# jirsat/wavenets

Measured on AMD Instinct MI355X. Metric: audio samples/sec (training step, 16 kHz mu-law), higher is better.
Workload: dtype f32 (fp16 hi|lo split operands, fp32 accumulate)

## Files before the change

### wavenets_amd/csrc/wn_elem.hip

```cpp
#include <algorithm>

#include "wn_kernels.h"
#include "wn_sample.h"

__global__ void wn_add_kernel(const float* a, const float* b, float* out, int64_t n) {
  for (int64_t i = (int64_t)blockIdx.x * blockDim.x + threadIdx.x; i < n;
       i += (int64_t)gridDim.x * blockDim.x)
    out[i] = a[i] + b[i];
}
int wn_launch_add(const float* a, const float* b, float* out, int64_t n, hipStream_t s) {
  if (n <= 0) return WN_OK;
  hipLaunchKernelGGL(wn_add_kernel, dim3(wn_blocks(n)), dim3(256), 0, s, a, b, out, n);
  WN_HIP_CHECK(hipGetLastError());
  return WN_OK;
}

__global__ void wn_fill_kernel(float* p, float v, int64_t n) {
  for (int64_t i = (int64_t)blockIdx.x * blockDim.x + threadIdx.x; i < n;
       i += (int64_t)gridDim.x * blockDim.x)
    p[i] = v;
}
int wn_launch_fill(float* p, float v, int64_t n, hipStream_t s) {
  if (n <= 0) return WN_OK;
  hipLaunchKernelGGL(wn_fill_kernel, dim3(wn_blocks(n)), dim3(256), 0, s, p, v, n);
  WN_HIP_CHECK(hipGetLastError());
  return WN_OK;
}

#define WN_CS_CHUNKS 128
__global__ void wn_colsum_stage1(const float* g, int T, int C, float* part) {
  __shared__ float sm[256];
  const int b = blockIdx.x, chunk = blockIdx.y;
  const int c = blockIdx.z * 64 + (threadIdx.x & 63);
  const int p = threadIdx.x >> 6;
  const int len = (T + WN_CS_CHUNKS - 1) / WN_CS_CHUNKS;
  const int t0 = chunk * len, t1 = min(T, t0 + len);
  float acc = 0.f;
  if (c < C)
    for (int t = t0 + p; t < t1; t += 4) acc += g[((int64_t)b * T + t) * C + c];
  sm[threadIdx.x] = acc;
  __syncthreads();
  if (p == 0 && c < C)
    part[((int64_t)b * WN_CS_CHUNKS + chunk) * C + c] = sm[threadIdx.x] + sm[threadIdx.x + 64] + sm[threadIdx.x + 128] + sm[threadIdx.x + 192];
}
__global__ void wn_colsum_stage2(const float* part, int C, float* out, int64_t total) {
  const int64_t i = (int64_t)blockIdx.x * blockDim.x + threadIdx.x;
  if (i >= total) return;
  const int64_t b = i / C;
  const int c = (int)(i % C);
  double acc = 0.0;
  for (int k = 0; k < WN_CS_CHUNKS; ++k) acc += (double)part[(b * WN_CS_CHUNKS + k) * C + c];
  out[i] = (float)acc;
}
int64_t wn_colsum_scratch_floats(int B, int C) { return (int64_t)B * WN_CS_CHUNKS * C; }
int wn_launch_colsum_per_batch(const float* g, int B, int T, int C, float* out, float* scratch, hipStream_t s) {
  hipLaunchKernelGGL(wn_colsum_stage1, dim3(B, WN_CS_CHUNKS, (C + 63) / 64), dim3(256), 0, s, g, T, C, scratch);
  const int64_t total = (int64_t)B * C;
  hipLaunchKernelGGL(wn_colsum_stage2, dim3((unsigned)((total + 255) / 256)), dim3(256), 0, s, scratch, C, out, total);
  WN_HIP_CHECK(hipGetLastError());
  return WN_OK;
}

__device__ __forceinline__ int wn_quantize_one(float x, int bits) {
  const int nmax = (1 << bits) - 1;
  const double step = ldexp(1.0, 1 - bits);
  double f = floor(((double)x + 1.0) / step);
  int idx = f < 0.0 ? 0 : (f > (double)nmax ? nmax : (int)f);
  while (idx > 0 && (float)(-1.0 + idx * step) > x) --idx;
  while (idx < nmax && (float)(-1.0 + (idx + 1) * step) <= x) ++idx;
  return idx;
}
__global__ void wn_quantize_kernel(const float* x, int32_t* idx, int64_t n, int bits) {
  for (int64_t i = (int64_t)blockIdx.x * blockDim.x + threadIdx.x; i < n;
       i += (int64_t)gridDim.x * blockDim.x)
    idx[i] = wn_quantize_one(x[i], bits);
}
int wn_launch_quantize(const float* x, int32_t* idx, int64_t n, int bits, hipStream_t s) {
  if (n <= 0) return WN_OK;
  if (bits < 1 || bits > 16) { wn_set_error("quantize: bits %d unsupported", bits); return WN_E_UNSUPPORTED; }
  hipLaunchKernelGGL(wn_quantize_kernel, dim3(wn_blocks(n)), dim3(256), 0, s, x, idx, n, bits);
  WN_HIP_CHECK(hipGetLastError());
  return WN_OK;
}

__global__ void wn_dequantize_kernel(const int32_t* idx, float* x, int64_t n, float inv) {
  for (int64_t i = (int64_t)blockIdx.x * blockDim.x + threadIdx.x; i < n;
       i += (int64_t)gridDim.x * blockDim.x)
    x[i] = (float)idx[i] * inv - 1.0f;
}
int wn_launch_dequantize(const int32_t* idx, float* x, int64_t n, int bits, hipStream_t s) {
  if (n <= 0) return WN_OK;
  hipLaunchKernelGGL(wn_dequantize_kernel, dim3(wn_blocks(n)), dim3(256), 0, s, idx, x, n,
                     1.0f / (float)(1 << (bits - 1)));
  WN_HIP_CHECK(hipGetLastError());
  return WN_OK;
}

__global__ void wn_mulaw_kernel(const float* x, float* y, int64_t n) {
  const float inv = 1.0f / logf(256.0f);
  for (int64_t i = (int64_t)blockIdx.x * blockDim.x + threadIdx.x; i < n;
       i += (int64_t)gridDim.x * blockDim.x) {
    const float v = x[i];
    const float sgn = v > 0.f ? 1.f : (v < 0.f ? -1.f : 0.f);
    y[i] = sgn * (logf(1.0f + 255.0f * fabsf(v)) * inv);
  }
}
int wn_launch_mulaw(const float* x, float* y, int64_t n, hipStream_t s) {
  if (n <= 0) return WN_OK;
  hipLaunchKernelGGL(wn_mulaw_kernel, dim3(wn_blocks(n)), dim3(256), 0, s, x, y, n);
  WN_HIP_CHECK(hipGetLastError());
  return WN_OK;
}

__global__ void wn_inv_mulaw_kernel(const float* y, float* x, int64_t n) {
  for (int64_t i = (int64_t)blockIdx.x * blockDim.x + threadIdx.x; i < n;
       i += (int64_t)gridDim.x * blockDim.x) {
    const float v = y[i];
    const float sgn = v > 0.f ? 1.f : (v < 0.f ? -1.f : 0.f);
    x[i] = sgn * (powf(256.0f, fabsf(v)) - 1.0f) / 255.0f;
  }
}
int wn_launch_inv_mulaw(const float* y, float* x, int64_t n, hipStream_t s) {
  if (n <= 0) return WN_OK;
  hipLaunchKernelGGL(wn_inv_mulaw_kernel, dim3(wn_blocks(n)), dim3(256), 0, s, y, x, n);
  WN_HIP_CHECK(hipGetLastError());
  return WN_OK;
}

__global__ void wn_sumsq_kernel(const float* g, const WnTensorDesc* table, float* norms2) {
  __shared__ double sm[256];
  const WnTensorDesc d = table[blockIdx.x];
  const float* p = g + d.off;
  double a0 = 0.0, a1 = 0.0, a2 = 0.0, a3 = 0.0;
  int64_t i = threadIdx.x;
  for (; i + 3 * 256 < d.len; i += 4 * 256) {
    const float v0 = p[i], v1 = p[i + 256], v2 = p[i + 512], v3 = p[i + 768];
    a0 += (double)v0 * (double)v0; a1 += (double)v1 * (double)v1;
    a2 += (double)v2 * (double)v2; a3 += (double)v3 * (double)v3;
  }
  for (; i < d.len; i += 256) a0 += (double)p[i] * (double)p[i];
  const double acc = (a0 + a1) + (a2 + a3);
  sm[threadIdx.x] = acc;
  __syncthreads();
  for (int o = 128; o > 0; o >>= 1) {
    if (threadIdx.x < o) sm[threadIdx.x] += sm[threadIdx.x + o];
    __syncthreads();
  }
  if (threadIdx.x == 0) norms2[blockIdx.x] = (float)sm[0];
}
int wn_launch_sumsq(const float* g, const WnTensorDesc* d_table, int n, float* norms2, hipStream_t s) {
  if (n <= 0) return WN_OK;
  hipLaunchKernelGGL(wn_sumsq_kernel, dim3(n), dim3(256), 0, s, g, d_table, norms2);
  WN_HIP_CHECK(hipGetLastError());
  return WN_OK;
}

#define WN_CLIP_THREADS 1024
__global__ void __launch_bounds__(WN_CLIP_THREADS)
wn_clip_kernel(float* g, const WnTensorDesc* table, float clipnorm, float* norms2) {
  __shared__ double sm[WN_CLIP_THREADS / 64];
  __shared__ float sm_scale;
  const WnTensorDesc d = table[blockIdx.x];
  float* p = g + d.off;
  const int tid = threadIdx.x;
  int64_t head = (int64_t)((16u - (unsigned)((uintptr_t)p & 15u)) & 15u) >> 2;
  if (head > d.len) head = d.len;
  const int64_t nvec = (d.len - head) >> 2;
  const int64_t tail = head + 4 * nvec;
  float4* pv = reinterpret_cast<float4*>(p + head);
  double a0 = 0.0, a1 = 0.0, a2 = 0.0, a3 = 0.0;
  int64_t i = tid;
  for (; i + WN_CLIP_THREADS < nvec; i += 2 * WN_CLIP_THREADS) {
    const float4 x = pv[i], y = pv[i + WN_CLIP_THREADS];
    a0 += (double)x.x * (double)x.x; a1 += (double)x.y * (double)x.y;
    a2 += (double)x.z * (double)x.z; a3 += (double)x.w * (double)x.w;
    a0 += (double)y.x * (double)y.x; a1 += (double)y.y * (double)y.y;
    a2 += (double)y.z * (double)y.z; a3 += (double)y.w * (double)y.w;
  }
  for (; i < nvec; i += WN_CLIP_THREADS) {
    const float4 x = pv[i];
    a0 += (double)x.x * (double)x.x; a1 += (double)x.y * (double)x.y;
    a2 += (double)x.z * (double)x.z; a3 += (double)x.w * (double)x.w;
  }
  if (tid < head) a0 += (double)p[tid] * (double)p[tid];
  if (tail + tid < d.len) a1 += (double)p[tail + tid] * (double)p[tail + tid];
  double acc = (a0 + a1) + (a2 + a3);
  for (int o = 32; o > 0; o >>= 1) acc += __shfl_down(acc, o, 64);
  if ((tid & 63) == 0) sm[tid >> 6] = acc;
  __syncthreads();
  if (tid == 0) {
    double n2 = 0.0;
    for (int w = 0; w < WN_CLIP_THREADS / 64; ++w) n2 += sm[w];
    const float n2f = (float)n2;
    norms2[blockIdx.x] = n2f;
    sm_scale = clipnorm / fmaxf(sqrtf(n2f), clipnorm);
  }
  __syncthreads();
  const float scale = sm_scale;
  if (scale == 1.0f) return;
  for (i = tid; i < nvec; i += WN_CLIP_THREADS) {
    float4 x = pv[i];
    x.x *= scale; x.y *= scale; x.z *= scale; x.w *= scale;
    pv[i] = x;
  }
  if (tid < head) p[tid] *= scale;
  if (tail + tid < d.len) p[tail + tid] *= scale;
}
int wn_launch_clip(float* g, const WnTensorDesc* d_table, int n, float clipnorm, float* norms2, hipStream_t s) {
  if (n <= 0) return WN_OK;
  hipLaunchKernelGGL(wn_clip_kernel, dim3(n), dim3(WN_CLIP_THREADS), 0, s, g, d_table, clipnorm, norms2);
  WN_HIP_CHECK(hipGetLastError());
  return WN_OK;
}

__global__ void wn_adam_kernel(float* p, const float* g, float* m, float* v, const WnTensorDesc* table,
                               const float* norms2, float clipnorm, float alpha, float beta1,
                               float beta2, float eps, const float* skip_flag) {
  if (skip_flag && *skip_flag != 0.f) return;
  const WnTensorDesc d = table[blockIdx.y];
  float scale = 1.0f;
  if (clipnorm > 0.f) {
    const float nrm = sqrtf(norms2[blockIdx.y]);
    scale = clipnorm / fmaxf(nrm, clipnorm);
  }
  for (int64_t i = (int64_t)blockIdx.x * blockDim.x + threadIdx.x; i < d.len;
       i += (int64_t)gridDim.x * blockDim.x) {
    const int64_t k = d.off + i;
    const float gi = g[k] * scale;
    const float mi = m[k] + (gi - m[k]) * (1.0f - beta1);
    const float vi = v[k] + (gi * gi - v[k]) * (1.0f - beta2);
    m[k] = mi;
    v[k] = vi;
    p[k] = p[k] - alpha * mi / (sqrtf(vi) + eps);
  }
}
int wn_launch_adam(float* p, const float* g, float* m, float* v, const WnTensorDesc* d_table, int n,
                   const float* norms2, float clipnorm, float alpha, float beta1, float beta2,
                   float eps, const float* skip_flag, hipStream_t s) {
  if (n <= 0) return WN_OK;
  hipLaunchKernelGGL(wn_adam_kernel, dim3(32, n), dim3(256), 0, s, p, g, m, v, d_table, norms2,
                     clipnorm, alpha, beta1, beta2, eps, skip_flag);
  WN_HIP_CHECK(hipGetLastError());
  return WN_OK;
}

__global__ void wn_adam_ema_kernel(float* p, const float* g, float* m, float* v, float* a, const WnTensorDesc* table,
                                   const float* norms2, float clipnorm, float alpha, float beta1,
                                   float beta2, float eps, float momentum, int first, int overwrite,
                                   const float* skip_flag) {
  if (skip_flag && *skip_flag != 0.f) return;
  const WnTensorDesc d = table[blockIdx.y];
  float scale = 1.0f;
  if (clipnorm > 0.f) {
    const float nrm = sqrtf(norms2[blockIdx.y]);
    scale = clipnorm / fmaxf(nrm, clipnorm);
  }
  for (int64_t i = (int64_t)blockIdx.x * blockDim.x + threadIdx.x; i < d.len;
       i += (int64_t)gridDim.x * blockDim.x) {
    const int64_t k = d.off + i;
    const float gi = g[k] * scale;
    const float mi = m[k] + (gi - m[k]) * (1.0f - beta1);
    const float vi = v[k] + (gi * gi - v[k]) * (1.0f - beta2);
    m[k] = mi;
    v[k] = vi;
    const float pi = p[k] - alpha * mi / (sqrtf(vi) + eps);
    const float ai = first ? pi : a[k] + (pi - a[k]) * (1.0f - momentum);
    a[k] = ai;
    p[k] = overwrite ? ai : pi;
  }
}
int wn_launch_adam_ema(float* p, const float* g, float* m, float* v, float* a, const WnTensorDesc* d_table, int n,
                       const float* norms2, float clipnorm, float alpha, float beta1, float beta2,
                       float eps, float momentum, int first, int overwrite, const float* skip_flag, hipStream_t s) {
  if (n <= 0) return WN_OK;
  hipLaunchKernelGGL(wn_adam_ema_kernel, dim3(32, n), dim3(256), 0, s, p, g, m, v, a, d_table, norms2,
                     clipnorm, alpha, beta1, beta2, eps, momentum, first, overwrite, skip_flag);
  WN_HIP_CHECK(hipGetLastError());
  return WN_OK;
}

__global__ void wn_gate_kernel(const float* u, int64_t rows, int D, float* ag, float* z, int ldz) {
  const int64_t total = rows * D;
  for (int64_t i = (int64_t)blockIdx.x * blockDim.x + threadIdx.x; i < total;
       i += (int64_t)gridDim.x * blockDim.x) {
    const int64_t r = i / D;
    const int c = (int)(i % D);
    const float a = wn_tanh_fast(u[r * 2 * D + c]);
    const float g = wn_sigmoid_fast(u[r * 2 * D + D + c]);
    if (ag) ag[r * D + c] = g;
    if (z) z[r * ldz + c] = a * g;
  }
}
int wn_launch_gate(const float* u, int64_t rows, int D, float* ag, float* z, int ldz, hipStream_t s) {
  if (rows <= 0) return WN_OK;
  hipLaunchKernelGGL(wn_gate_kernel, dim3(wn_blocks(rows * D)), dim3(256), 0, s, u, rows, D, ag, z, ldz);
  WN_HIP_CHECK(hipGetLastError());
  return WN_OK;
}

__global__ void wn_batch_reduce_kernel(const float* slab, int splits, int N, float* out, int64_t total) {
  const int64_t i = (int64_t)blockIdx.x * blockDim.x + threadIdx.x;
  if (i >= total) return;
  const int64_t b = i / N;
  const int n = (int)(i % N);
  float acc = 0.f;
  for (int s = 0; s < splits; ++s) acc += slab[(b * splits + s) * N + n];
  out[i] = acc;
}
int wn_launch_batch_reduce(const float* slab, int B, int splits, int N, float* out, hipStream_t s) {
  const int64_t total = (int64_t)B * N;
  if (total <= 0) return WN_OK;
  hipLaunchKernelGGL(wn_batch_reduce_kernel, dim3((unsigned)((total + 255) / 256)), dim3(256), 0, s,
                     slab, splits, N, out, total);
  WN_HIP_CHECK(hipGetLastError());
  return WN_OK;
}

__global__ void wn_axpy_table_kernel(float* y, const float* x, const WnTensorDesc* table, float coef) {
  const WnTensorDesc d = table[blockIdx.y];
  for (int64_t i = (int64_t)blockIdx.x * blockDim.x + threadIdx.x; i < d.len;
       i += (int64_t)gridDim.x * blockDim.x)
    y[d.off + i] += coef * x[d.off + i];
}
int wn_launch_axpy_table(float* y, const float* x, const WnTensorDesc* d_table, int n, float coef,
                         hipStream_t s) {
  if (n <= 0) return WN_OK;
  hipLaunchKernelGGL(wn_axpy_table_kernel, dim3(16, n), dim3(256), 0, s, y, x, d_table, coef);
  WN_HIP_CHECK(hipGetLastError());
  return WN_OK;
}

__global__ void wn_dact_mul_kernel(const float* g, const float* y, float* out, int64_t n, int act) {
  for (int64_t i = (int64_t)blockIdx.x * blockDim.x + threadIdx.x; i < n;
       i += (int64_t)gridDim.x * blockDim.x)
    out[i] = g[i] * wn_dact_from_y(y[i], act);
}
int wn_launch_dact_mul(const float* g, const float* y, float* out, int64_t n, int act, hipStream_t s) {
  if (n <= 0) return WN_OK;
  hipLaunchKernelGGL(wn_dact_mul_kernel, dim3(wn_blocks(n)), dim3(256), 0, s, g, y, out, n, act);
  WN_HIP_CHECK(hipGetLastError());
  return WN_OK;
}

__device__ __forceinline__ uint32_t wn_hash32(uint32_t x) {
  x ^= x >> 16; x *= 0x7feb352dU; x ^= x >> 15; x *= 0x846ca68bU; x ^= x >> 16;
  return x;
}
__device__ __forceinline__ bool wn_drop_keep(int64_t idx, uint32_t key, float rate) {
  const uint32_t lo = (uint32_t)idx, hi = (uint32_t)((uint64_t)idx >> 32);
  const uint32_t hsh = wn_hash32(lo ^ wn_hash32(hi + key));
  return (float)(hsh >> 8) * (1.0f / 16777216.0f) >= rate;
}
__global__ void wn_dropout_kernel(const float* x, const float* g_res, float* out, int64_t n, float rate, float scale,
                                  uint32_t key, float* absmax_out) {
  float m = 0.f;
  for (int64_t i = (int64_t)blockIdx.x * blockDim.x + threadIdx.x; i < n; i += (int64_t)gridDim.x * blockDim.x) {
    float v = wn_drop_keep(i, key, rate) ? x[i] * scale : 0.f;
    if (g_res) v += g_res[i];
    out[i] = v;
    m = fmaxf(m, fabsf(v));
  }
  if (absmax_out) {
    m = wn_wave_max(m);
    if ((threadIdx.x & 63) == 0) wn_absmax_publish(absmax_out, m);
  }
}
uint32_t wn_dropout_key(uint64_t seed, int block, uint64_t step) {
  uint32_t k = (uint32_t)seed * 0x9E3779B9U + (uint32_t)(seed >> 32);
  k ^= (uint32_t)block * 0x85EBCA6BU + 0x1234567U;
  k ^= (uint32_t)step * 0xC2B2AE35U + (uint32_t)(step >> 32) * 0x27D4EB2FU;
  return k;
}
int wn_launch_dropout(const float* x, const float* g_res, float* out, int64_t n, float rate, uint32_t key,
                      float* absmax_out, hipStream_t s) {
  if (n <= 0) return WN_OK;
  hipLaunchKernelGGL(wn_dropout_kernel, dim3(wn_blocks(n)), dim3(256), 0, s, x, g_res, out, n, rate, 1.0f / (1.0f - rate),
                     key, absmax_out);
  WN_HIP_CHECK(hipGetLastError());
  return WN_OK;
}

__global__ void wn_cond_scatter_kernel(const float* tmp, const float* params, int64_t b_off0, int64_t b_stride, int B,
                                       int N, int D2, float* cb) {
  const int64_t total = (int64_t)N * B * D2;
  for (int64_t i = (int64_t)blockIdx.x * blockDim.x + threadIdx.x; i < total; i += (int64_t)gridDim.x * blockDim.x) {
    const int n = (int)(i % D2);
    const int u = (int)((i / D2) % B);
    const int b = (int)(i / ((int64_t)D2 * B));
    cb[i] = tmp[((int64_t)u * N + b) * D2 + n] + params[b_off0 + (int64_t)b * b_stride + n];
  }
}
__global__ void wn_cond_gather_kernel(const float* slab, int64_t P, int spb, int64_t bd_off0, int64_t bd_stride, int B,
                                      int N, int D2, float* dcb) {
  const int64_t total = (int64_t)B * N * D2;
  for (int64_t i = (int64_t)blockIdx.x * blockDim.x + threadIdx.x; i < total; i += (int64_t)gridDim.x * blockDim.x) {
    const int n = (int)(i % D2);
    const int b = (int)((i / D2) % N);
    const int u = (int)(i / ((int64_t)D2 * N));
    float acc = 0.f;
    for (int sp = 0; sp < spb; ++sp) acc += slab[(int64_t)(u * spb + sp) * P + bd_off0 + (int64_t)b * bd_stride + n];
    dcb[i] = acc;
  }
}
__global__ void wn_cond_wgrad_kernel(const float* m, const float* dcb, int B, int Cc, int N, int D2, float* grads,
                                     int64_t w_off0, int64_t w_stride, int64_t b_off0, int64_t b_stride) {
  const int64_t total = (int64_t)N * (Cc + 1) * D2;
  for (int64_t i = (int64_t)blockIdx.x * blockDim.x + threadIdx.x; i < total; i += (int64_t)gridDim.x * blockDim.x) {
    const int n = (int)(i % D2);
    const int c = (int)((i / D2) % (Cc + 1));
    const int b = (int)(i / ((int64_t)D2 * (Cc + 1)));
    float acc = 0.f;
    for (int u = 0; u < B; ++u) {
      const float g = dcb[((int64_t)u * N + b) * D2 + n];
      acc += c < Cc ? m[(int64_t)u * Cc + c] * g : g;
    }
    if (c < Cc) grads[w_off0 + (int64_t)b * w_stride + (int64_t)c * D2 + n] = acc;
    else grads[b_off0 + (int64_t)b * b_stride + n] = acc;
  }
}
int wn_launch_cond_scatter(const float* tmp, const float* params, int64_t b_off0, int64_t b_stride, int B, int N, int D2,
                           float* cb, hipStream_t s) {
  const int64_t total = (int64_t)N * B * D2;
  hipLaunchKernelGGL(wn_cond_scatter_kernel, dim3((unsigned)std::min<int64_t>((total + 255) / 256, 1024)), dim3(256), 0, s, tmp,
                     params, b_off0, b_stride, B, N, D2, cb);
  WN_HIP_CHECK(hipGetLastError());
  return WN_OK;
}
int wn_launch_cond_gather(const float* slab, int64_t P, int spb, int64_t bd_off0, int64_t bd_stride, int B, int N, int D2,
                          float* dcb, hipStream_t s) {
  const int64_t total = (int64_t)B * N * D2;
  hipLaunchKernelGGL(wn_cond_gather_kernel, dim3((unsigned)std::min<int64_t>((total + 255) / 256, 1024)), dim3(256), 0, s, slab, P,
                     spb, bd_off0, bd_stride, B, N, D2, dcb);
  WN_HIP_CHECK(hipGetLastError());
  return WN_OK;
}
int wn_launch_cond_wgrad(const float* m, const float* dcb, int B, int Cc, int N, int D2, float* grads, int64_t w_off0,
                         int64_t w_stride, int64_t b_off0, int64_t b_stride, hipStream_t s) {
  const int64_t total = (int64_t)N * (Cc + 1) * D2;
  hipLaunchKernelGGL(wn_cond_wgrad_kernel, dim3((unsigned)std::min<int64_t>((total + 255) / 256, 1024)), dim3(256), 0, s, m, dcb, B,
                     Cc, N, D2, grads, w_off0, w_stride, b_off0, b_stride);
  WN_HIP_CHECK(hipGetLastError());
  return WN_OK;
}

__global__ __launch_bounds__(256) void wn_inconv_fwd_kernel(const float* x, const float* w, const float* bias, int B, int T,
                                                            int R, int KS, float* y, float* absmax_out) {
  const int q = R / 4;
  const int64_t total = (int64_t)B * T * q;
  float wmax = 0.f;
  for (int64_t i = (int64_t)blockIdx.x * blockDim.x + threadIdx.x; i < total; i += (int64_t)gridDim.x * blockDim.x) {
    const int c = (int)(i % q) * 4;
    const int64_t row = i / q;
    const int t = (int)(row % T);
    float a0 = 0.f, a1 = 0.f, a2 = 0.f, a3 = 0.f;
    for (int tap = 0; tap < KS; ++tap) {
      const int ts = t - (KS - 1 - tap);
      const float xv = ts >= 0 ? x[row - (KS - 1 - tap)] : 0.f;
      const f32x4 wv = *reinterpret_cast<const f32x4*>(w + (int64_t)tap * R + c);
      a0 = fmaf(wv.x, xv, a0); a1 = fmaf(wv.y, xv, a1); a2 = fmaf(wv.z, xv, a2); a3 = fmaf(wv.w, xv, a3);
    }
    const f32x4 bv = *reinterpret_cast<const f32x4*>(bias + c);
    const f32x4 o = f32x4{a0 + bv.x, a1 + bv.y, a2 + bv.z, a3 + bv.w};
    *reinterpret_cast<f32x4*>(y + row * R + c) = o;
    wmax = fmaxf(wmax, fmaxf(fmaxf(fabsf(o.x), fabsf(o.y)), fmaxf(fabsf(o.z), fabsf(o.w))));
  }
  if (absmax_out) {
    __shared__ float wm[4];
    if (!(wmax < 3.0e38f)) wmax = 3.0e38f;
    wmax = wn_wave_max(wmax);
    if ((threadIdx.x & 63) == 0) wm[threadIdx.x >> 6] = wmax;
    __syncthreads();
    if (threadIdx.x == 0) wn_absmax_publish_any(absmax_out, fmaxf(fmaxf(wm[0], wm[1]), fmaxf(wm[2], wm[3])));
  }
}
int wn_launch_inconv_fwd(const float* x, const float* w, const float* bias, int B, int T, int R, int KS, float* y,
                         float* absmax_out, hipStream_t s) {
  const int64_t total = (int64_t)B * T * (R / 4);
  if (total <= 0) return WN_OK;
  hipLaunchKernelGGL(wn_inconv_fwd_kernel, dim3((unsigned)std::min<int64_t>((total + 255) / 256, 1024)), dim3(256), 0, s, x, w, bias,
                     B, T, R, KS, y, absmax_out);
  WN_HIP_CHECK(hipGetLastError());
  return WN_OK;
}

__global__ __launch_bounds__(256) void wn_sgemm_small32_kernel(const float* A, int64_t sai, int64_t sak, const float* B, int64_t sbk,
                                                               int64_t sbj, float* C, int ldc, int M, int N, int K,
                                                               int64_t za, int64_t zb, int64_t zc, const float* bias, int act,
                                                               int zk) {
  constexpr int KC = 128;
  __shared__ float As[KC][32 + 1], Bs[KC][32 + 1];
  A += (int64_t)blockIdx.z * za; B += (int64_t)blockIdx.z * zb; C += (int64_t)blockIdx.z * zc;
  if (zk > 0) K = max(0, min(K - (int)blockIdx.z * zk, zk));
  const int i0 = blockIdx.y * 32, j0 = blockIdx.x * 32;
  const int tx = threadIdx.x & 31, ty = threadIdx.x >> 5;
  float acc[4] = {0.f, 0.f, 0.f, 0.f};
  for (int k0 = 0; k0 < K; k0 += KC) {
    float ra[16], rb[16];
#pragma unroll
    for (int q = 0; q < 16; ++q) {
      const int e = threadIdx.x + 256 * q;
      const int ka = sak == 1 ? e % KC : e / 32, ia = sak == 1 ? e / KC : e % 32;
      ra[q] = (i0 + ia < M && k0 + ka < K) ? A[(int64_t)(i0 + ia) * sai + (int64_t)(k0 + ka) * sak] : 0.f;
      const int kb = sbk == 1 ? e % KC : e / 32, jb = sbk == 1 ? e / KC : e % 32;
      rb[q] = (j0 + jb < N && k0 + kb < K) ? B[(int64_t)(k0 + kb) * sbk + (int64_t)(j0 + jb) * sbj] : 0.f;
    }
    if (k0 > 0) __syncthreads();
#pragma unroll
    for (int q = 0; q < 16; ++q) {
      const int e = threadIdx.x + 256 * q;
      const int ka = sak == 1 ? e % KC : e / 32, ia = sak == 1 ? e / KC : e % 32;
      As[ka][ia] = ra[q];
      const int kb = sbk == 1 ? e % KC : e / 32, jb = sbk == 1 ? e / KC : e % 32;
      Bs[kb][jb] = rb[q];
    }
    __syncthreads();
#pragma unroll 8
    for (int k = 0; k < KC; ++k) {
      const float bv = Bs[k][tx];
#pragma unroll
      for (int a = 0; a < 4; ++a) acc[a] = fmaf(As[k][ty + 8 * a], bv, acc[a]);
    }
  }
#pragma unroll
  for (int a = 0; a < 4; ++a) {
    const int i = i0 + ty + 8 * a, j = j0 + tx;
    if (i < M && j < N) {
      float v = acc[a];
      if (bias) v = wn_act(v + bias[j], act);
      C[(int64_t)i * ldc + j] = v;
    }
  }
}
int wn_launch_sgemm_small(const float* A, int64_t sai, int64_t sak, const float* B, int64_t sbk, int64_t sbj, float* C, int ldc,
                          int M, int N, int K, hipStream_t s) {
  if (M <= 0 || N <= 0) return WN_OK;
  hipLaunchKernelGGL(wn_sgemm_small32_kernel, dim3((N + 31) / 32, (M + 31) / 32), dim3(256), 0, s, A, sai, sak, B, sbk, sbj, C,
                     ldc, M, N, K, (int64_t)0, (int64_t)0, (int64_t)0, (const float*)nullptr, 0, 0);
  WN_HIP_CHECK(hipGetLastError());
  return WN_OK;
}

int wn_launch_sgemm_small_batched(const float* A, int64_t sai, int64_t sak, int64_t za, const float* B, int64_t sbk, int64_t sbj,
                                  int64_t zb, float* C, int ldc, int64_t zc, int M, int N, int K, int nz, const float* bias,
                                  int act, hipStream_t s, int zk) {
  if (M <= 0 || N <= 0 || nz <= 0) return WN_OK;
  if (nz > 65535) { wn_set_error("sgemm_small_batched: too many products"); return WN_E_UNSUPPORTED; }
  hipLaunchKernelGGL(wn_sgemm_small32_kernel, dim3((N + 31) / 32, (M + 31) / 32, nz), dim3(256), 0, s, A, sai, sak, B, sbk, sbj, C,
                     ldc, M, N, K, za, zb, zc, bias, act, zk);
  WN_HIP_CHECK(hipGetLastError());
  return WN_OK;
}

__global__ void wn_skip_gather_kernel(const float* params, int64_t ws_off0, int64_t ws_stride, const float* bsum, int N, int D,
                                      int S, float* wsall) {
  for (int64_t i = (int64_t)blockIdx.x * blockDim.x + threadIdx.x; i < (int64_t)(N * D + 1) * S; i += (int64_t)gridDim.x * blockDim.x) {
    const int k = (int)(i / S), sidx = (int)(i % S);
    wsall[i] = k < N * D ? params[ws_off0 + (int64_t)(k / D) * ws_stride + (int64_t)(k % D) * S + sidx] : bsum[sidx];
  }
}
__global__ void wn_vec_add_kernel(const float* a, const float* b, int n, float* out) {
  const int i = blockIdx.x * blockDim.x + threadIdx.x;
  if (i < n) out[i] = a[i] + b[i];
}
int wn_launch_skip_fold(const float* params, int64_t ws_off0, int64_t ws_stride, int64_t wf0_off, int64_t bf0_off,
                        const float* bsum, int N, int D, int S, int F0, float* V, float* bfold, float* wsall, hipStream_t s) {
  const int64_t total = (int64_t)(N * D + 1) * S;
  hipLaunchKernelGGL(wn_skip_gather_kernel, dim3((unsigned)std::min<int64_t>((total + 255) / 256, 2048)), dim3(256), 0, s, params,
                     ws_off0, ws_stride, bsum, N, D, S, wsall);
  WN_HIP_CHECK(hipGetLastError());
  int rc = wn_launch_sgemm_small(wsall, S, 1, params + wf0_off, F0, 1, V, F0, N * D + 1, F0, S, s);
  if (rc) return rc;
  hipLaunchKernelGGL(wn_vec_add_kernel, dim3((F0 + 255) / 256), dim3(256), 0, s, V + (int64_t)N * D * F0, params + bf0_off, F0, bfold);
  WN_HIP_CHECK(hipGetLastError());
  return WN_OK;
}

__global__ void wn_skip_scatter_kernel(const float* Y, const float* colsum, int64_t ws_off0, int64_t ws_stride, int64_t bs_off0,
                                       int64_t bs_stride, int64_t bf0_off, int N, int D, int S, int F0, float* grads) {
  const int64_t n_ws = (int64_t)N * D * S, n_bs = (int64_t)N * S;
  const int64_t total = n_ws + n_bs + F0;
  for (int64_t i = (int64_t)blockIdx.x * blockDim.x + threadIdx.x; i < total; i += (int64_t)gridDim.x * blockDim.x) {
    if (i < n_ws) {
      const int k = (int)(i / S), sidx = (int)(i % S);
      grads[ws_off0 + (int64_t)(k / D) * ws_stride + (int64_t)(k % D) * S + sidx] = Y[i];
    } else if (i < n_ws + n_bs) {
      const int64_t j = i - n_ws;
      grads[bs_off0 + (j / S) * bs_stride + (j % S)] = Y[n_ws + (j % S)];
    } else {
      grads[bf0_off + (i - n_ws - n_bs)] = colsum[i - n_ws - n_bs];
    }
  }
}
int wn_launch_skip_scatter(const float* Y, const float* colsum, int64_t ws_off0, int64_t ws_stride, int64_t bs_off0,
                           int64_t bs_stride, int64_t bf0_off, int N, int D, int S, int F0, float* grads, hipStream_t s) {
  const int64_t total = (int64_t)N * D * S + (int64_t)N * S + F0;
  hipLaunchKernelGGL(wn_skip_scatter_kernel, dim3((unsigned)std::min<int64_t>((total + 255) / 256, 4096)), dim3(256), 0, s, Y, colsum,
                     ws_off0, ws_stride, bs_off0, bs_stride, bf0_off, N, D, S, F0, grads);
  WN_HIP_CHECK(hipGetLastError());
  return WN_OK;
}

__global__ void wn_guard_flag_kernel(const float* absmax, float limit, int enabled, float* out) {
  const float m = absmax ? *absmax : 0.f;
  out[0] = (enabled && !(m < limit)) ? 1.0f : 0.0f;
}
__global__ void wn_guard_accumulate_kernel(const float* src, float* dst) {
  const unsigned a = __float_as_uint(src[0]) & 0x7fffffffu, b = __float_as_uint(dst[0]) & 0x7fffffffu;
  dst[0] = __uint_as_float(a > b ? a : b);
}
int wn_launch_guard_accumulate(const float* src, float* dst, hipStream_t s) {
  hipLaunchKernelGGL(wn_guard_accumulate_kernel, dim3(1), dim3(1), 0, s, src, dst);
  WN_HIP_CHECK(hipGetLastError());
  return WN_OK;
}
int wn_launch_guard_flag(const float* absmax, float limit, int enabled, float* out, hipStream_t s) {
  hipLaunchKernelGGL(wn_guard_flag_kernel, dim3(1), dim3(1), 0, s, absmax, limit, enabled, out);
  WN_HIP_CHECK(hipGetLastError());
  return WN_OK;
}

template <int KS>
__global__ __launch_bounds__(256) void wn_inconv_wgrad_kernel(const float* x, const float* g, int T, int R, int spb,
                                                              float* slab, int64_t P, int64_t w_off, int64_t b_off) {
  __shared__ float red[256 * (KS + 1) * 4];
  const int split = blockIdx.x, ub = split / spb, sp = split % spb;
  int len = (T + spb - 1) / spb;
  const int r0 = sp * len, r1 = min(T, r0 + len);
// ... 49 lines not shown
```

### wavenets_amd/csrc/wn_forward.hip

```cpp
#include "wn_plan_internal.h"

namespace {

__global__ void wn_ring_capture_kernel(const float* src, int B, int T, int C, int nslots, float* ring) {
  const int64_t n = (int64_t)nslots * B * C;
  for (int64_t i = (int64_t)blockIdx.x * blockDim.x + threadIdx.x; i < n; i += (int64_t)gridDim.x * blockDim.x) {
    const int c = (int)(i % C);
    const int b = (int)((i / C) % B);
    const int k = (int)(i / ((int64_t)C * B));
    const int t = T - nslots + k;
    if (t >= 0) ring[((int64_t)(t % nslots) * B + b) * C + c] = src[((int64_t)b * T + t) * C + c];
  }
}

__global__ void wn_shift_split_kernel(const float* x_full, int B, int T, float* inputs, float* y_true) {
  const int64_t n = (int64_t)B * T;
  for (int64_t i = (int64_t)blockIdx.x * blockDim.x + threadIdx.x; i < n; i += (int64_t)gridDim.x * blockDim.x) {
    const int64_t b = i / T, t = i % T;
    inputs[i] = x_full[b * (T + 1) + t];
    y_true[i] = x_full[b * (T + 1) + t + 1];
  }
}

}

namespace wnp {

BlockPtrs block_ptrs(const wn_plan* p, int b, const float* params, const float* fragbase, int B, int T) {
  BlockPtrs k;
  memset(&k, 0, sizeof(k));
  const BlockInfo& bi = p->blocks[b];
  k.B = B; k.T = T; k.KS = p->KS; k.R = p->R; k.D = p->D; k.S = p->S; k.Cin = p->R; k.depth = p->LPB;
  k.act = p->c.activation; k.residual = p->c.use_residual;
  for (int i = 0; i < p->LPB; ++i) {
    const ConvInfo& c = bi.dil[i];
    k.dil[i] = c.dil;
    k.Wd[i] = params + p->tensors[c.kernel_t].off;
    k.bd[i] = params + p->tensors[c.bias_t].off;
    k.Fd[i] = fragbase + c.fragF; k.Fd_stride[i] = c.fragF_stride;
    k.Bd[i] = fragbase + c.fragB; k.Bd_stride[i] = c.fragB_stride;
  }
  k.br = params + p->tensors[bi.conv1.bias_t].off;
  k.Fr = fragbase + bi.conv1.fragF; k.Br_ = fragbase + bi.conv1.fragB;
  if (bi.has_skip) { k.bs = params + p->tensors[bi.conv_skip.bias_t].off; k.Bs = fragbase + bi.conv_skip.fragB; }
  k.Cc = 0; k.cond = nullptr; k.cb = nullptr;
  k.fused = p->fused_ok;
  if (p->fused16_ok && p->LPB == 1) { k.F16d = fragbase + bi.dil.back().frag16; k.F16r = fragbase + bi.conv1.frag16; }
  if (bi.f16gate >= 0) { k.F16g = fragbase + bi.f16gate; k.F16r = fragbase + bi.conv1.frag16; }
  if (bi.f16nat >= 0) k.F16n = fragbase + bi.f16nat;
  if (bi.g16u >= 0 && p->LPB == 1) k.G16u = fragbase + bi.g16u;
  if (bi.g16uf >= 0) k.G16uf = fragbase + bi.g16uf;
  if (p->LPB == 1 && bi.dil[0].frag16B >= 0) k.G16x = fragbase + bi.dil[0].frag16B;
  return k;
}

void deep16_ptrs(const wn_plan* p, int b, const float* fragbase, BlockPtrs& k) {
  if (!deep16(p)) return;
  const BlockInfo& bi = p->blocks[b];
  k.F16d = fragbase + bi.dil.back().frag16; k.F16r = fragbase + bi.conv1.frag16;
  for (int i = 0; i < p->LPB; ++i) {
    const ConvInfo& c = bi.dil[i];
    if (bi.d16F[i] >= 0) { k.F16i[i] = fragbase + bi.d16F[i]; k.JTi[i] = std::max(2, ceil32(c.cout)); }
    if (bi.d16B[i] >= 0) { k.G16i[i] = fragbase + bi.d16B[i]; k.JTb[i] = std::max(2, ceil32(c.cin)); }
  }
  if (bi.g16u >= 0) { k.G16u = fragbase + bi.g16u; k.JTu = std::max(2, ceil32(p->D)); }
}

int ring_capture(const float* src, int B, int T, int C, int nslots, float* ring, hipStream_t s) {
  const int64_t n = (int64_t)nslots * B * C;
  hipLaunchKernelGGL(wn_ring_capture_kernel, dim3((unsigned)std::min<int64_t>((n + 255) / 256, 4096)), dim3(256), 0, s,
                     src, B, T, C, nslots, ring);
  WN_HIP_CHECK(hipGetLastError());
  return WN_OK;
}

int forward_core(wn_plan* p, const float* params, const float* x, bool prep, const float* cond, int B,
                 int T, bool training, float* ws, const WsLayout& L, hipStream_t s, const GenRings* rings, LossFuse* lf) {
  int rc = ensure_device_tables(p);
  if (rc) return rc;
  const int64_t rows = (int64_t)B * T;
  float* fragbase = ws + L.frag;
  if (prep) {
    rc = wn_launch_prep_table(p->d_prep, (int)p->prep.size(), params, fragbase, s);
    if (rc) return rc;
  }
  wn_exec& exs = wnp::ex(p);
  const bool fold = fold_ok(p);
  const bool fork_prep = prep && fold && p->c.use_skip && wn_debug_get(9) == 0;
  bool prep_forked = false;
  auto fold_prep = [&](hipStream_t sp) -> int {
    const bool fp_prof = prep && fold && exs.foldprep_used + 2 <= (int)exs.foldprep_ev.size();
    if (fp_prof) (void)hipEventRecord(exs.foldprep_ev[exs.foldprep_used], sp);
    if (prep && p->c.use_skip) {
      const ConvInfo& c0 = p->blocks[0].has_skip ? p->blocks[0].conv_skip : p->blocks[0].conv1;
      WnVecSumArgs v;
      v.base = params; v.off0 = p->tensors[c0.bias_t].off;
      v.stride = p->N > 1 ? (p->tensors[(p->blocks[1].has_skip ? p->blocks[1].conv_skip : p->blocks[1].conv1).bias_t].off - v.off0) : 0;
      v.count = p->N; v.len = p->Sh; v.out = ws + L.bias_sum;
      const int r = wn_launch_vecsum(v, sp);
      if (r) return r;
    }
    if (fold && prep) {
      const BlockInfo& b0 = p->blocks[0];
      const int64_t wst = p->N > 1 ? p->tensors[p->blocks[1].conv_skip.kernel_t].off - p->tensors[b0.conv_skip.kernel_t].off : 0;
      int r = wn_launch_skip_fold(params, p->tensors[b0.conv_skip.kernel_t].off, wst, p->tensors[p->finals[0].kernel_t].off,
                                  p->tensors[p->finals[0].bias_t].off, ws + L.bias_sum, p->N, p->D, p->S, p->fold_F0, ws + L.vfold,
                                  ws + L.bfold, ws + L.wsall, sp);
      if (r) return r;
      r = wn_launch_prep_table(p->d_prep2, (int)p->prep2.size(), ws, fragbase, sp, 64);
      if (r) return r;
    }
    if (fp_prof) { (void)hipEventRecord(exs.foldprep_ev[exs.foldprep_used + 1], sp); exs.foldprep_used += 2; }
    return WN_OK;
  };
  if (!fork_prep) {
    rc = fold_prep(s);
    if (rc) return rc;
  }
  const float* m = cond;
  if (p->c.cond_inputs > 0) {
    if (!cond) { wn_set_error("Conditioning must be provided."); return WN_E_INVALID; }
    int mc = p->c.cond_inputs;
    for (size_t j = 0; j < p->mapping.size(); ++j) {
      const ConvInfo& c = p->mapping[j];
      if (cond_small(p))
        rc = wn_launch_sgemm_small_batched(m, mc, 1, 0, params + p->tensors[c.kernel_t].off, c.cout, 1, 0, ws + L.M[j], c.cout, 0,
                                           B, c.cout, mc, 1, params + p->tensors[c.bias_t].off, p->c.mapping_activation, s);
      else
      rc = Gemm(1, B, c.cout, ceil32(c.cout)).seg(m, mc, mc, 0, fragbase + c.fragF)
               .bias(params + p->tensors[c.bias_t].off).act(p->c.mapping_activation).run(ws + L.M[j], c.cout, s);
      if (rc) return rc;
      m = ws + L.M[j]; mc = c.cout;
    }
    if (p->frag_condF >= 0) {
      const int D2 = 2 * p->D;
      const ConvInfo& c0 = p->blocks[0].conv_cond;
      const int64_t bst = p->N > 1 ? p->tensors[p->blocks[1].conv_cond.bias_t].off - p->tensors[c0.bias_t].off : 0;
      if (cond_small(p)) {
        const int64_t wst = p->N > 1 ? p->tensors[p->blocks[1].conv_cond.kernel_t].off - p->tensors[c0.kernel_t].off : 0;
        rc = wn_launch_sgemm_small_batched(m, p->Cc, 1, 0, params + p->tensors[c0.kernel_t].off, D2, 1, wst, ws + L.cbt, p->N * D2, D2,
                                           B, D2, p->Cc, p->N, nullptr, 0, s);
      } else
      rc = Gemm(1, B, p->N * D2, ceil32(p->N * D2)).seg(m, p->Cc, p->Cc, 0, fragbase + p->frag_condF).run(ws + L.cbt, p->N * D2, s);
      if (rc) return rc;
      rc = wn_launch_cond_scatter(ws + L.cbt, params, p->tensors[c0.bias_t].off, bst, B, p->N, D2, ws + L.cb, s);
      if (rc) return rc;
    } else {
    for (int b = 0; b < p->N; ++b) {
      const ConvInfo& c = p->blocks[b].conv_cond;
      rc = Gemm(1, B, 2 * p->D, ceil32(2 * p->D)).seg(m, p->Cc, p->Cc, 0, fragbase + c.fragF)
               .bias(params + p->tensors[c.bias_t].off).run(ws + L.cb + (int64_t)b * B * 2 * p->D, 2 * p->D, s);
      if (rc) return rc;
    }
    }
  }
  float* const fam = ws + L.fwd_absmax;
  WN_HIP_CHECK(hipMemsetAsync(fam, 0, sizeof(float), s));
  {
    if (p->R % 4 == 0 && wn_debug_get(1) != 1) {
      rc = wn_launch_inconv_fwd(x, params + p->tensors[p->causal.kernel_t].off, params + p->tensors[p->causal.bias_t].off, B, T,
                                p->R, p->KS, ws + L.H[0], fam, s);
    } else {
      Gemm g(B, T, p->R, ceil32(p->R));
      for (int t = 0; t < p->KS; ++t)
        g.seg(x, 1, 1, (p->KS - 1 - t), fragbase + p->causal.fragF + t * p->causal.fragF_stride);
      rc = g.bias(params + p->tensors[p->causal.bias_t].off).run(ws + L.H[0], p->R, s);
    }
    if (rc) return rc;
    if (rings) {
      rc = ring_capture(x, B, T, 1, p->KS, rings->xin, s);
      if (!rc) rc = ring_capture(ws + L.H[0], B, T, p->R, rings->nslots[0], rings->h[0], s);
      if (rc) return rc;
    }
  }
  if (p->Dp != p->D) {
    rc = wn_launch_fill(ws + L.Z, 0.f, rows * p->N * p->Dp, s);
    if (rc) return rc;
  }
  const bool prof_chain = wnp::ex(p).prof_on && !rings && p->LPB == 1 && p->c.cond_inputs == 0 && p->R == p->D &&
                          !(training && wnp::ex(p).drop_rate > 0.f) && block_ptrs(p, 0, params, fragbase, B, T).fused;
  const bool stack_prof = !rings && wnp::ex(p).stack_used + 2 <= (int)wnp::ex(p).stack_ev.size();
  if (stack_prof) (void)hipEventRecord(wnp::ex(p).stack_ev[wnp::ex(p).stack_used], s);
  if (fork_prep) {
    if (!exs.side) {
      WN_HIP_CHECK(hipStreamCreateWithFlags(&exs.side, hipStreamNonBlocking));
      WN_HIP_CHECK(hipEventCreateWithFlags(&exs.ev_fork, hipEventDisableTiming));
      WN_HIP_CHECK(hipEventCreateWithFlags(&exs.ev_join, hipEventDisableTiming));
    }
    if (!exs.ev_ffork) {
      WN_HIP_CHECK(hipEventCreateWithFlags(&exs.ev_ffork, hipEventDisableTiming));
      WN_HIP_CHECK(hipEventCreateWithFlags(&exs.ev_fjoin, hipEventDisableTiming));
    }
    WN_HIP_CHECK(hipEventRecord(exs.ev_ffork, s));
    WN_HIP_CHECK(hipStreamWaitEvent(exs.side, exs.ev_ffork, 0));
    rc = fold_prep(exs.side);
    if (rc) return rc;
    WN_HIP_CHECK(hipEventRecord(exs.ev_fjoin, exs.side));
    prep_forked = true;
  }
  for (int b = 0; b < p->N; ++b) {
    BlockPtrs k = block_ptrs(p, b, params, fragbase, B, T);
    if (training && !rings) deep16_ptrs(p, b, fragbase, k);
    if (p->c.cond_inputs > 0) k.cb = ws + L.cb + (int64_t)b * B * 2 * p->D;
    BlockBufs f;
    memset(&f, 0, sizeof(f));
    const int hi = training ? b : (b & 1), ho = training ? b + 1 : ((b + 1) & 1);
    f.x = ws + L.H[hi];
    if (training && wnp::ex(p).drop_rate > 0.f) {
      rc = wn_launch_dropout(ws + L.H[hi], nullptr, ws + L.XD[b], rows * p->R, wnp::ex(p).drop_rate,
                             wn_dropout_key(wnp::ex(p).drop_seed, b, wnp::ex(p).drop_step), nullptr, s);
      if (rc) return rc;
      f.x = ws + L.XD[b];
      f.res = ws + L.H[hi];
    }
    for (int i = 0; i + 1 < p->LPB; ++i) f.P[i] = ws + L.P[b][i];
    f.U = ws + L.U;
    f.AG = training ? ws + L.AG[b] : nullptr;
    f.Z = ws + L.Z + (int64_t)b * rows * p->Dp; f.ldz = p->Dp;
    f.O = nullptr;
    f.x_out = ws + L.H[ho];
    f.fwd_absmax = fam;
    const bool prof = wnp::ex(p).prof_on && wnp::ex(p).prof_used + 2 <= (int)wnp::ex(p).prof_ev.size();
    const bool ev0 = prof && (!prof_chain || b == 0), ev1 = prof && (!prof_chain || b == p->N - 1);
    if (ev0) (void)hipEventRecord(wnp::ex(p).prof_ev[wnp::ex(p).prof_used], s);
    rc = block_forward(k, f, s);
    if (rc) return rc;
    if (ev1) {
      (void)hipEventRecord(wnp::ex(p).prof_ev[wnp::ex(p).prof_used + 1], s);
      wnp::ex(p).prof_cnt[wnp::ex(p).prof_used / 2] = prof_chain ? p->N : 1;
      wnp::ex(p).prof_used += 2;
    }
    if (rings && b + 1 < p->N) {
      rc = ring_capture(f.x_out, B, T, p->R, rings->nslots[b + 1], rings->h[b + 1], s);
      if (rc) return rc;
    }
    if (rings)
      for (int i = 0; i + 1 < p->LPB; ++i) {
        rc = ring_capture(f.P[i], B, T, p->D, rings->nslots_p[b][i], rings->hp[b][i], s);
        if (rc) return rc;
      }
  }
  if (prep_forked) WN_HIP_CHECK(hipStreamWaitEvent(s, exs.ev_fjoin, 0));
  const float* hin;
  size_t first_final = 0;
  if (fold) {
    const ConvInfo& c0 = p->finals[0];
    if (p->Dp == p->D && wn_gemm_planes16s_supported(c0.cout, p->D, p->N, p->Dp, c0.cout) &&
        (int64_t)rows * p->Dp * 4 < ((int64_t)1 << 32) && (int64_t)rows * c0.cout * 4 < ((int64_t)1 << 32)) {
      WnGemmPlanesArgs ga;
      memset(&ga, 0, sizeof(ga));
      ga.z = ws + L.Z; ga.plane_stride = rows * p->Dp; ga.ld = p->Dp; ga.plane_k = p->D; ga.nplanes = p->N;
      ga.w16 = fragbase + p->frag16_foldF; ga.bias = ws + L.bfold; ga.act = p->c.activation;
      ga.y = ws + L.HA[0]; ga.ldy = c0.cout; ga.N = c0.cout; ga.B = B; ga.T = T; ga.absmax_out = fam;
      rc = wn_launch_gemm_planes16s(ga, s);
    } else
    rc = Gemm(B, T, c0.cout, ceil32(c0.cout)).seg_planes(ws + L.Z, p->Dp, rows * p->Dp, p->N * p->Dp, nullptr)
             .w16(fragbase + p->frag16_foldF).bias(ws + L.bfold).act(p->c.activation).absmax_fwd(fam)
             .run(ws + L.HA[0], c0.cout, s);
    if (rc) return rc;
    hin = ws + L.HA[0];
    first_final = 1;
  } else if (p->c.use_skip) {
    rc = Gemm(B, T, p->Sh, ceil32(p->Sh)).seg_planes(ws + L.Z, p->Dp, rows * p->Dp, p->N * p->Dp, fragbase + p->frag_skipF)
             .w16(p->frag16_skipF >= 0 ? fragbase + p->frag16_skipF : nullptr)
             .bias(ws + L.bias_sum).absmax_fwd(fam).run(ws + L.skipsum, p->Sh, s);
    if (rc) return rc;
    hin = ws + L.skipsum;
  } else {
    hin = ws + L.H[training ? p->N : (p->N & 1)];
  }
  if (stack_prof) { (void)hipEventRecord(wnp::ex(p).stack_ev[wnp::ex(p).stack_used + 1], s); wnp::ex(p).stack_used += 2; }
  int hc = fold ? p->finals[0].cout : p->Hin;
  for (size_t i = first_final; i < p->finals.size(); ++i) {
    const ConvInfo& c = p->finals[i];
    const bool last = (i + 1 == p->finals.size());
    float* dst = last ? ws + L.logits : ws + L.HA[i];
    if (last && lf && loss_fusable(p, rows) && wn_gemm_planes16s_supported(c.cout, hc, 1, hc, c.cout) &&
        (int64_t)rows * hc * 4 < ((int64_t)1 << 32)) {
      WnGemmPlanesArgs ga;
      memset(&ga, 0, sizeof(ga));
      ga.z = hin; ga.plane_stride = 0; ga.ld = hc; ga.plane_k = hc; ga.nplanes = 1;
      ga.w16 = fragbase + c.frag16; ga.bias = params + p->tensors[c.bias_t].off; ga.act = WN_ACT_LINEAR;
      ga.y = lf->g_logits; ga.ldy = c.cout; ga.N = c.cout; ga.B = B; ga.T = T; ga.absmax_out = lf->absmax_out;
      ga.cat_loss = 1; ga.target = lf->target; ga.gscale = lf->gscale; ga.loss_rows = lf->loss_rows;
      ga.sample_out = lf->sample_out; ga.inv_lv = lf->inv_lv; ga.seed = lf->seed; ga.offset = lf->offset;
      rc = wn_launch_gemm_planes16s(ga, s);
      if (rc) return rc;
      lf->done = true;
      break;
    }
    if (c.frag16 >= 0 && wn_debug_get(1) != 1 && wn_gemm_planes16s_supported(c.cout, hc, 1, hc, c.cout) &&
        (int64_t)rows * hc * 4 < ((int64_t)1 << 32)) {
      WnGemmPlanesArgs ga;
      memset(&ga, 0, sizeof(ga));
      ga.z = hin; ga.plane_stride = 0; ga.ld = hc; ga.plane_k = hc; ga.nplanes = 1;
      ga.w16 = fragbase + c.frag16; ga.bias = params + p->tensors[c.bias_t].off; ga.act = last ? WN_ACT_LINEAR : p->c.activation;
      ga.y = dst; ga.ldy = c.cout; ga.N = c.cout; ga.B = B; ga.T = T; ga.absmax_out = last ? nullptr : fam;
      rc = wn_launch_gemm_planes16s(ga, s);
      if (rc) return rc;
      hin = dst; hc = c.cout;
      continue;
    }
    rc = Gemm(B, T, c.cout, ceil32(c.cout)).seg(hin, hc, hc, 0, fragbase + c.fragF)
             .w16(c.frag16 >= 0 ? fragbase + c.frag16 : nullptr)
             .bias(params + p->tensors[c.bias_t].off).act(last ? WN_ACT_LINEAR : p->c.activation)
             .absmax_fwd(last ? nullptr : fam).run(dst, c.cout, s);
    if (rc) return rc;
    hin = dst; hc = c.cout;
  }
  return WN_OK;
}

int shift_split(const float* x_full, int B, int T, float* inputs, float* y_true, hipStream_t s) {
  const int64_t rows = (int64_t)B * T;
  hipLaunchKernelGGL(wn_shift_split_kernel, dim3((unsigned)std::min<int64_t>((rows + 255) / 256, 4096)), dim3(256), 0, s,
                     x_full, B, T, inputs, y_true);
  WN_HIP_CHECK(hipGetLastError());
  return WN_OK;
}

bool loss_fusable(const wn_plan* p, int64_t rows) {
  if (p->c.head != WN_HEAD_CATEGORICAL || p->Cout != 256 || wn_debug_get(1) == 1 || p->finals.empty()) return false;
  const ConvInfo& c = p->finals.back();
  return c.frag16 >= 0 && c.cout == 256 && rows > 0;
}

int loss_stage(wn_plan* p, int B, int T, int global_batch, bool want_grad, float* ws, const WsLayout& L,
               float* loss_out, float* absmax_out, hipStream_t s, bool fused_done) {
  const int64_t rows = (int64_t)B * T;
  const float gscale = 1.0f / (float)global_batch;
  int rc;
  if (fused_done) return wn_launch_sum(ws + L.loss_rows, rows, gscale, loss_out, ws + L.sum_scratch, s);
  float* g_logits = want_grad ? ws + L.GF.back() : nullptr;
  if (p->c.head == WN_HEAD_CATEGORICAL) {
    rc = wn_launch_quantize(ws + L.yt, reinterpret_cast<int32_t*>(ws + L.target), rows, p->c.bits, s);
    if (rc) return rc;
    float* so = nullptr;
    if (want_grad && wnp::ex(p).step_sample && !wnp::ex(p).step_sample_det && p->Cout <= 256) { so = wnp::ex(p).step_sample; wnp::ex(p).step_sample = nullptr; }
    rc = wn_launch_cat_loss(ws + L.logits, reinterpret_cast<const int32_t*>(ws + L.target), rows, p->Cout,
                            gscale, ws + L.loss_rows, g_logits, absmax_out, s, so, p->c.bits, wnp::ex(p).step_sample_seed,
                            wnp::ex(p).step_sample_off);
  } else {
    rc = wn_launch_mix_loss(ws + L.logits, ws + L.yt, rows, p->c.num_mixtures, p->c.bits,
                            p->c.head == WN_HEAD_LOGISTIC ? 1 : 2, gscale, ws + L.loss_rows, g_logits, absmax_out, s);
  }
  if (rc) return rc;
  return wn_launch_sum(ws + L.loss_rows, rows, gscale, loss_out, ws + L.sum_scratch, s);
}

}

using namespace wnp;

extern "C" int wn_forward(wn_plan* p, const float* params, const float* x, const float* cond, int32_t B,
                          int32_t T, float* out, float* logits_out, float* workspace, int64_t ws_floats,
                          void* stream) {
  if (!p || !params || !x || !workspace || B < 1 || T < 1) { wn_set_error("forward: bad arguments"); return WN_E_INVALID; }
  hipStream_t s = (hipStream_t)stream;
  const WsLayout L = make_layout(p, B, T, false);
  if (ws_floats < L.total) { wn_set_error("forward: workspace too small (%lld < %lld floats)", (long long)ws_floats, (long long)L.total); return WN_E_INVALID; }
  int rc = forward_core(p, params, x, true, cond, B, T, false, workspace, L, s);
  if (rc) return rc;
  const int64_t rows = (int64_t)B * T;
  if (logits_out) WN_HIP_CHECK(hipMemcpyAsync(logits_out, workspace + L.logits, rows * p->Cout * sizeof(float), hipMemcpyDeviceToDevice, s));
  if (out) {
    if (p->c.head == WN_HEAD_CATEGORICAL) return wn_launch_softmax(workspace + L.logits, out, rows, p->Cout, s);
    WN_HIP_CHECK(hipMemcpyAsync(out, workspace + L.logits, rows * p->Cout * sizeof(float), hipMemcpyDeviceToDevice, s));
  }
  return WN_OK;
}

extern "C" int wn_forward_training(wn_plan* p, const float* params, const float* x, const float* cond, int32_t B,
                                   int32_t T, float* out, float* logits_out, float* workspace, int64_t ws_floats,
                                   void* stream) {
  if (!p || !params || !x || !workspace || B < 1 || T < 1) { wn_set_error("forward_training: bad arguments"); return WN_E_INVALID; }
  hipStream_t s = (hipStream_t)stream;
  const WsLayout L = make_layout(p, B, T, true);
  if (ws_floats < L.total) { wn_set_error("forward_training: workspace too small (%lld < %lld floats)", (long long)ws_floats, (long long)L.total); return WN_E_INVALID; }
  int rc = forward_core(p, params, x, true, cond, B, T, true, workspace, L, s);
  if (rc) return rc;
  const int64_t rows = (int64_t)B * T;
  if (logits_out) WN_HIP_CHECK(hipMemcpyAsync(logits_out, workspace + L.logits, rows * p->Cout * sizeof(float), hipMemcpyDeviceToDevice, s));
  if (out) {
    if (p->c.head == WN_HEAD_CATEGORICAL) return wn_launch_softmax(workspace + L.logits, out, rows, p->Cout, s);
    WN_HIP_CHECK(hipMemcpyAsync(out, workspace + L.logits, rows * p->Cout * sizeof(float), hipMemcpyDeviceToDevice, s));
  }
  return WN_OK;
}

extern "C" int wn_eval_loss(wn_plan* p, const float* params, const float* x_full, const float* cond,
                            int32_t B, int32_t T, int32_t global_batch, float* loss_out, float* pred_out,
                            float* workspace, int64_t ws_floats, void* stream) {
  if (!p || !params || !x_full || !workspace || !loss_out || B < 1 || T < 1) { wn_set_error("eval_loss: bad arguments"); return WN_E_INVALID; }
  hipStream_t s = (hipStream_t)stream;
  const WsLayout L = make_layout(p, B, T, false);
  if (ws_floats < L.total) { wn_set_error("eval_loss: workspace too small"); return WN_E_INVALID; }
  const int64_t rows = (int64_t)B * T;
  float* inputs = workspace + L.probs;
  { const int rcs = shift_split(x_full, B, T, inputs, workspace + L.yt, s); if (rcs) return rcs; }
  int rc = forward_core(p, params, inputs, true, cond, B, T, false, workspace, L, s);
  if (rc) return rc;
  rc = loss_stage(p, B, T, global_batch > 0 ? global_batch : B, false, workspace, L, loss_out, nullptr, s);
  if (rc) return rc;
  rc = wn_launch_guard_flag(workspace + L.fwd_absmax, WN_RANGE_LIMIT, wn_debug_get(1) != 1, loss_out + 2, s);
  if (rc) return rc;
  if (pred_out) {
    if (p->c.head == WN_HEAD_CATEGORICAL) return wn_launch_softmax(workspace + L.logits, pred_out, rows, p->Cout, s);
    WN_HIP_CHECK(hipMemcpyAsync(pred_out, workspace + L.logits, rows * p->Cout * sizeof(float), hipMemcpyDeviceToDevice, s));
  }
  return WN_OK;
}
```

### wavenets_amd/csrc/wn_gemm.hip

```cpp
#include "wn_split16.h"

using namespace wn_split16;

__device__ __forceinline__ void wn_prep16_body(const WnPrepDesc& d, const float* params, float* ws,
                                               int64_t start, int64_t stride) {
  const int JI = (d.I + 31) / 32;
  const int nks = (d.KK + 15) / 16;
  const int64_t total = (int64_t)nks * JI * 64 * 8;
  const float* src = params + d.src_off;
  __half* dst = reinterpret_cast<__half*>(ws + d.dst_off);
  for (int64_t idx = start; idx < total; idx += stride) {
    const int jj = idx & 7;
    const int lane = (idx >> 3) & 63;
    const int64_t blk = idx >> 9;
    const int j = blk % JI;
    const int ks = blk / JI;
    const int i = 32 * j + (lane & 31);
    const int kk = 16 * ks + 8 * (jj >> 2) + 4 * (lane >> 5) + (jj & 3);
    float v = 0.f;
    if (i < d.I && kk < d.KK) v = d.transpose ? src[(int64_t)kk * d.ld + i] : src[(int64_t)i * d.ld + kk];
    const __half hi = __float2half_rn(v);
    const __half lo = __float2half_rn(v - __half2float(hi));
    const int64_t base = (((int64_t)(ks + d.q_off) * d.JT + (j + d.j_off)) * 2) * 512 + lane * 8 + jj;
    dst[base] = hi;
    dst[base + 512] = lo;
  }
}

__device__ __forceinline__ void wn_prep_body(const WnPrepDesc& d, const float* params, float* ws,
                                             int64_t start, int64_t stride) {
  if (d.kind == 1) { wn_prep16_body(d, params, ws, start, stride); return; }
  const int JI = (d.I + 31) / 32;
  const int nq = (d.KK + 7) / 8;
  const int64_t total = (int64_t)nq * JI * 256;
  const float* src = params + d.src_off;
  float* dst = ws + d.dst_off;
  for (int64_t idx = start; idx < total; idx += stride) {
    int e = idx & 3;
    int lane = (idx >> 2) & 63;
    int64_t blk = idx >> 8;
    int j = blk % JI;
    int q = blk / JI;
    int i = 32 * j + (lane & 31);
    int kk = 8 * q + 4 * (lane >> 5) + e;
    float v = 0.f;
    if (i < d.I && kk < d.KK) v = d.transpose ? src[(int64_t)kk * d.ld + i] : src[(int64_t)i * d.ld + kk];
    dst[(((int64_t)(q + d.q_off) * d.JT + (j + d.j_off)) * 64 + lane) * 4 + e] = v;
  }
}

__global__ void wn_prep_table_kernel(const WnPrepDesc* table, const float* params, float* ws) {
  WnPrepDesc d = table[blockIdx.y];
  wn_prep_body(d, params, ws, (int64_t)blockIdx.x * blockDim.x + threadIdx.x,
               (int64_t)gridDim.x * blockDim.x);
}

__global__ void wn_prep_one_kernel(WnPrepDesc d, const float* params, float* ws) {
  wn_prep_body(d, params, ws, (int64_t)blockIdx.x * blockDim.x + threadIdx.x,
               (int64_t)gridDim.x * blockDim.x);
}

int wn_launch_prep_table(const WnPrepDesc* d_table, int n, const float* params, float* ws,
                         hipStream_t s, int gx) {
  if (n <= 0) return WN_OK;
  dim3 grid(gx > 0 ? gx : 16, n);
  hipLaunchKernelGGL(wn_prep_table_kernel, grid, dim3(256), 0, s, d_table, params, ws);
  WN_HIP_CHECK(hipGetLastError());
  return WN_OK;
}

int wn_launch_prep_one(WnPrepDesc d, const float* params, float* ws, hipStream_t s) {
  hipLaunchKernelGGL(wn_prep_one_kernel, dim3(16), dim3(256), 0, s, d, params, ws);
  WN_HIP_CHECK(hipGetLastError());
  return WN_OK;
}

__global__ void wn_vecsum_kernel(WnVecSumArgs a) {
  int i = blockIdx.x * blockDim.x + threadIdx.x;
  if (i >= a.len) return;
  float acc = 0.f;
  for (int j = 0; j < a.count; ++j) acc += a.base[a.off0 + (int64_t)j * a.stride + i];
  a.out[i] = acc;
}

int wn_launch_vecsum(WnVecSumArgs a, hipStream_t s) {
  hipLaunchKernelGGL(wn_vecsum_kernel, dim3((a.len + 255) / 256), dim3(256), 0, s, a);
  WN_HIP_CHECK(hipGetLastError());
  return WN_OK;
}

template <int JT>
__global__ __launch_bounds__(256, (JT >= 8 ? 2 : (JT >= 4 ? 3 : 4))) void wn_gemm_rows_kernel(WnGemmArgs a) {
  const int lane = threadIdx.x & 63;
  const int wave = threadIdx.x >> 6;
  const int tiles_per_b = (a.T + 31) >> 5;
  const int64_t tile = (int64_t)blockIdx.x * 4 + wave;
  if (tile >= (int64_t)a.B * tiles_per_b) return;
  const int b = (int)(tile / tiles_per_b);
  const int t0 = (int)(tile % tiles_per_b) * 32;
  const int tl = lane & 31, h = lane >> 5;
  const int t = t0 + tl;
  const int jb = blockIdx.y * JT;

  f32x16 acc[JT];
#pragma unroll
  for (int j = 0; j < JT; ++j)
#pragma unroll
    for (int r = 0; r < 16; ++r) acc[j][r] = 0.f;

#pragma unroll
  for (int s = 0; s < WN_MAXSEG; ++s) {
    if (s >= a.nseg) break;
    const float* sx = a.seg[s].x;
    const float* sfrag = a.seg[s].frag;
    const int sldx = a.seg[s].ldx, sK = a.seg[s].K, sshift = a.seg[s].shift, svec = a.seg[s].vec;
    const int splk = a.seg[s].plane_k;
    const int64_t splst = a.seg[s].plane_stride;
    const int ts = t - sshift;
    const bool valid = (t < a.T) && (ts >= 0) && (ts < a.T);
    const float* xrow = sx + ((int64_t)b * a.T + (valid ? ts : 0)) * sldx;
    const int nq = (sK + 7) >> 3;
    const f32x4* fr = reinterpret_cast<const f32x4*>(sfrag) + (int64_t)jb * 64 + lane;

    auto load_x = [&](int q) -> f32x4 {
      const int k = 8 * q + 4 * h;
      f32x4 xv = {0.f, 0.f, 0.f, 0.f};
      if (valid) {
        const float* xp = splk > 0 ? xrow + (int64_t)(k / splk) * splst + (k % splk) : xrow + k;
        if (svec && k + 3 < sK) {
          xv = *reinterpret_cast<const f32x4*>(xp);
        } else {
          if (k + 0 < sK) xv.x = xp[0];
          if (k + 1 < sK) xv.y = xp[1];
          if (k + 2 < sK) xv.z = xp[2];
          if (k + 3 < sK) xv.w = xp[3];
        }
      }
      return xv;
    };
    auto load_a = [&](int q, f32x4 (&av)[JT]) {
      wn_static_for<JT>([&](auto jc) {
        constexpr int j = decltype(jc)::value;
        if (jb + j < a.JTtot) av[j] = fr[((int64_t)q * a.JTtot + j) * 64];
      });
    };
    auto compute = [&](const f32x4& xv, const f32x4 (&av)[JT]) {
      wn_static_for<JT>([&](auto jc) {
        constexpr int j = decltype(jc)::value;
        if (jb + j < a.JTtot) {
          acc[j] = wn_mfma(av[j].x, xv.x, acc[j]);
          acc[j] = wn_mfma(av[j].y, xv.y, acc[j]);
          acc[j] = wn_mfma(av[j].z, xv.z, acc[j]);
          acc[j] = wn_mfma(av[j].w, xv.w, acc[j]);
        }
      });
    };
    constexpr int PF = 8;
    if (JT == 1 && svec && splk == 0 && (sK & 7) == 0 && (nq % PF) == 0 && jb < a.JTtot) {
      const f32x4* xp = reinterpret_cast<const f32x4*>(xrow + 4 * h);
      const f32x4* ap = fr;
      const int64_t astep = (int64_t)a.JTtot * 64;
      f32x4 xr[PF], ar[PF];
#pragma unroll
      for (int i = 0; i < PF; ++i) { xr[i] = xp[2 * i]; ar[i] = ap[i * astep]; }
      __builtin_amdgcn_sched_barrier(0);
      for (int q0 = 0; q0 < nq; q0 += PF) {
#pragma unroll
        for (int i = 0; i < PF; ++i) {
          f32x4 xv = xr[i];
          if (!valid) xv = f32x4{0.f, 0.f, 0.f, 0.f};
          const f32x4 av = ar[i];
          acc[0] = wn_mfma(av.x, xv.x, acc[0]);
          acc[0] = wn_mfma(av.y, xv.y, acc[0]);
          acc[0] = wn_mfma(av.z, xv.z, acc[0]);
          acc[0] = wn_mfma(av.w, xv.w, acc[0]);
          const int qn = min(q0 + i + PF, nq - 1);
          xr[i] = xp[2 * qn];
          ar[i] = ap[qn * astep];
          __builtin_amdgcn_sched_barrier(0);
        }
      }
    } else {
    f32x4 x0, x1, a0[JT], a1[JT];
    x0 = load_x(0);
    load_a(0, a0);
    int q = 0;
    for (; q + 2 <= nq; q += 2) {
      x1 = load_x(q + 1);
      load_a(q + 1, a1);
      compute(x0, a0);
      if (q + 2 < nq) {
        x0 = load_x(q + 2);
        load_a(q + 2, a0);
      }
      compute(x1, a1);
    }
    if (q < nq) compute(x0, a0);
    }
  }

  if (t >= a.T) return;
  const int64_t row = (int64_t)b * a.T + t;
  wn_static_for<JT * 4>([&](auto jc) {
    constexpr int j = decltype(jc)::value / 4;
    constexpr int rq = decltype(jc)::value % 4;
    {
      const int n0 = 32 * (jb + j) + 8 * rq + 4 * h;
      if (n0 >= a.N) return;
      float v[4];
      v[0] = acc[j][4 * rq + 0]; v[1] = acc[j][4 * rq + 1];
      v[2] = acc[j][4 * rq + 2]; v[3] = acc[j][4 * rq + 3];
      const bool full = a.vec_out && (n0 + 3 < a.N);
      if (full) {
        if (a.bias) {
          const f32x4 bv = *reinterpret_cast<const f32x4*>(a.bias + n0);
          v[0] += bv.x; v[1] += bv.y; v[2] += bv.z; v[3] += bv.w;
        }
        if (a.rowbias) {
          const float* rb = a.rowbias + (int64_t)b * a.ld_rowbias + n0;
// ... 258 lines not shown
      compute_chunk(av0, bv0);
      if (tt + 16 < r1) {
        if (tt + 32 < r1) load_chunk(tt + 32, av0, bv0);
        compute_chunk(av1, bv1);
      }
    }
  }

#pragma unroll
  for (int i = 0; i < WG_TM; ++i)
#pragma unroll
    for (int j = 0; j < WG_TN; ++j) {
      const int n = n0 + 32 * j + tl;
#pragma unroll
      for (int r = 0; r < 16; ++r) {
        const int k = k0 + 32 * i + wn_drow(r, h);
        if (k < a.K && n < a.N) a.out[(int64_t)k * a.out_ld + n] = acc[i][j][r] * inv_gsc;
      }
    }
  if (a.bias) {
#pragma unroll
    for (int j = 0; j < WG_TN; ++j) {
      const float tot = bsum[j] + __shfl_xor(bsum[j], 32);
      const int n = n0 + 32 * j + tl;
      if (h == 0 && n < a.N) a.bias[n] = tot;
    }
  }
}

__global__ __launch_bounds__(256, 2) void wn_wgrad_kernel(WnWgradArgs a, int nkb, int nnb) {
  const int wave = threadIdx.x >> 6;
  const int nsplit = a.B * a.splits_per_b;
  const int split = blockIdx.x * 4 + wave;
  if (split >= nsplit) return;
  const int kb = blockIdx.y / nnb, nb = blockIdx.y % nnb;
  const int sp = split % a.splits_per_b;
  int len = (a.T + a.splits_per_b - 1) / a.splits_per_b;
  len = (len + 1) & ~1;
  WnWgUnit u;
  u.x = a.x; u.ldx = a.ldx; u.K = a.K; u.shift = a.shift; u.g = a.g; u.ldg = a.ldg; u.N = a.N;
  u.T = a.T; u.b = split / a.splits_per_b; u.r0 = sp * len; u.r1 = min(a.T, u.r0 + len);
  u.k0 = kb * 32 * WG_TM; u.n0 = nb * 32 * WG_TN;
  u.out = a.slab + (int64_t)split * a.K * a.N; u.out_ld = a.N;
  u.bias = (a.slab_bias && kb == 0) ? a.slab_bias + (int64_t)split * a.N : nullptr;
  wn_wgrad_body(u);
}

template <bool F16>
__global__ __launch_bounds__(256, 2) void wn_wgrad_batched_kernel(const WnWgJob* jobs, float* ws, float* slab,
                                                                  int64_t P, int B, int T, int splits_per_b) {
  const int wave = threadIdx.x >> 6;
  const int nsplit = B * splits_per_b;
  const int split = blockIdx.x * 4 + wave;
  if (split >= nsplit) return;
  const WnWgJob j = jobs[blockIdx.y];
  const int sp = split % splits_per_b;
  int len = (T + splits_per_b - 1) / splits_per_b;
  len = (len + 1) & ~1;
  WnWgUnit u;
  u.x = ws + j.x_off; u.ldx = j.ldx; u.K = j.K; u.shift = j.shift; u.g = ws + j.g_off; u.ldg = j.ldg; u.N = j.N;
  u.T = T; u.b = split / splits_per_b; u.r0 = sp * len; u.r1 = min(T, u.r0 + len);
  u.k0 = j.k0; u.n0 = j.n0;
  float* row = slab + (int64_t)split * P;
  u.out = row + j.out_off; u.out_ld = j.N;
  u.bias = j.bias_off >= 0 ? row + j.bias_off : nullptr;
  if constexpr (F16) {
    float gsc = 1.0f, inv = 1.0f;
    if (j.gmax_off >= 0) pow2_scale(ws[j.gmax_off], gsc, inv);
    wn_wgrad_body16(u, gsc, inv);
  } else {
    wn_wgrad_body(u);
  }
}

int wn_launch_wgrad_batched(const WnWgJob* d_jobs, int njobs, float* ws, float* slab, int64_t P, int B, int T,
                            int splits_per_b, hipStream_t s, bool exact_fp32) {
  if (njobs <= 0) return WN_OK;
  const int nsplit = B * splits_per_b;
  if (exact_fp32 || wn_debug_get(1) == 1 || wn_debug_get(3) == 1)
    hipLaunchKernelGGL(wn_wgrad_batched_kernel<false>, dim3((nsplit + 3) / 4, njobs), dim3(256), 0, s, d_jobs, ws, slab, P,
                       B, T, splits_per_b);
  else
    hipLaunchKernelGGL(wn_wgrad_batched_kernel<true>, dim3((nsplit + 3) / 4, njobs), dim3(256), 0, s, d_jobs, ws, slab, P,
                       B, T, splits_per_b);
  WN_HIP_CHECK(hipGetLastError());
  return WN_OK;
}

__global__ void wn_reduce_table_kernel(const float* slab, int nsplit, int64_t P, float* out,
                                       const WnTensorDesc* table) {
  const WnTensorDesc d = table[blockIdx.y];
  for (int64_t i = (int64_t)blockIdx.x * blockDim.x + threadIdx.x; i < d.len;
       i += (int64_t)gridDim.x * blockDim.x) {
    float acc = 0.f;
    const float* col = slab + d.off + i;
    int s = 0;
    for (; s + 8 <= nsplit; s += 8) {
      float v[8];
#pragma unroll
      for (int e = 0; e < 8; ++e) v[e] = col[(int64_t)(s + e) * P];
#pragma unroll
      for (int e = 0; e < 8; ++e) acc += v[e];
    }
    for (; s < nsplit; ++s) acc += col[(int64_t)s * P];
    out[d.off + i] = acc;
  }
}

struct WnBlkFirst { int v[257]; };
__global__ __launch_bounds__(256) void wn_reduce_flat_kernel(const float* slab, int nsplit, int64_t P, float* out,
                                                             const WnTensorDesc* table, WnBlkFirst bf, int n) {
  int lo = 0, hi = n;
  while (hi - lo > 1) {
    const int mid = (lo + hi) >> 1;
    if (bf.v[mid] <= (int)blockIdx.x) lo = mid; else hi = mid;
  }
  const WnTensorDesc d = table[lo];
  const int64_t i = (int64_t)((int)blockIdx.x - bf.v[lo]) * 256 + threadIdx.x;
  if (i >= d.len) return;
  float acc = 0.f;
  const float* col = slab + d.off + i;
  int s = 0;
  for (; s + 16 <= nsplit; s += 16) {
    float v[16];
#pragma unroll
    for (int e = 0; e < 16; ++e) v[e] = col[(int64_t)(s + e) * P];
#pragma unroll
    for (int e = 0; e < 16; ++e) acc += v[e];
  }
  for (; s < nsplit; ++s) acc += col[(int64_t)s * P];
  out[d.off + i] = acc;
}

int wn_launch_reduce_table(const float* slab, int nsplit, int64_t P, float* out, const WnTensorDesc* d_table,
                           int n, hipStream_t s, const WnTensorDesc* h_table) {
  if (n <= 0) return WN_OK;
  if (h_table && n <= 256) {
    WnBlkFirst bf;
    int64_t nblk = 0;
    for (int t = 0; t < n; ++t) { bf.v[t] = (int)nblk; nblk += (h_table[t].len + 255) / 256; }
    for (int t = n; t <= 256; ++t) bf.v[t] = (int)nblk;
    if (nblk <= 0) return WN_OK;
    if (nblk < (int64_t)1 << 30) {
      hipLaunchKernelGGL(wn_reduce_flat_kernel, dim3((unsigned)nblk), dim3(256), 0, s, slab, nsplit, P, out, d_table, bf, n);
      WN_HIP_CHECK(hipGetLastError());
      return WN_OK;
    }
  }
  hipLaunchKernelGGL(wn_reduce_table_kernel, dim3(64, n), dim3(256), 0, s, slab, nsplit, P, out, d_table);
  WN_HIP_CHECK(hipGetLastError());
  return WN_OK;
}

int wn_wgrad_tile_k() { return 32 * WG_TM; }
int wn_wgrad_tile_n() { return 32 * WG_TN; }

int wn_wgrad_choose_splits(int B, int T, int K, int N) {
  const int jobs = ((K + 32 * WG_TM - 1) / (32 * WG_TM)) * ((N + 32 * WG_TN - 1) / (32 * WG_TN));
  int want = (1024 + jobs - 1) / jobs;
  int per_b = (want + B - 1) / B;
  const int max_per_b = (T + 255) / 256;
  if (per_b > max_per_b) per_b = max_per_b;
  if (per_b < 1) per_b = 1;
  return per_b;
}

int wn_launch_wgrad(const WnWgradArgs& a, hipStream_t s) {
  if (a.K <= 0 || a.N <= 0 || a.B <= 0 || a.T <= 0) return WN_OK;
  const int nkb = (a.K + 32 * WG_TM - 1) / (32 * WG_TM);
  const int nnb = (a.N + 32 * WG_TN - 1) / (32 * WG_TN);
  const int nsplit = a.B * a.splits_per_b;
  dim3 grid((nsplit + 3) / 4, nkb * nnb);
  hipLaunchKernelGGL(wn_wgrad_kernel, grid, dim3(256), 0, s, a, nkb, nnb);
  WN_HIP_CHECK(hipGetLastError());
  return WN_OK;
}

#define WN_RED_GROUP 16
__global__ void wn_reduce_stageA_kernel(float* slab, int nsplit, int64_t total) {
  const int g = blockIdx.y;
  const int s0 = g * WN_RED_GROUP;
  const int s1 = min(nsplit, s0 + WN_RED_GROUP);
  for (int64_t i = (int64_t)blockIdx.x * blockDim.x + threadIdx.x; i < total;
       i += (int64_t)gridDim.x * blockDim.x) {
    float acc = 0.f;
    for (int s = s0; s < s1; ++s) acc += slab[(int64_t)s * total + i];
    slab[(int64_t)s0 * total + i] = acc;
  }
}

__global__ void wn_reduce_kernel(WnReduceArgs a, int stride) {
  const int64_t total = (int64_t)a.K * a.N;
  for (int64_t i = (int64_t)blockIdx.x * blockDim.x + threadIdx.x; i < total;
       i += (int64_t)gridDim.x * blockDim.x) {
    float acc = 0.f;
    for (int s = 0; s < a.nsplit; s += stride) acc += a.slab[(int64_t)s * total + i];
    const int k = (int)(i / a.N), n = (int)(i % a.N);
    float* dst = a.out + (int64_t)(k / a.seg_len) * a.seg_stride + (int64_t)(k % a.seg_len) * a.N + n;
    for (int r = 0; r < a.replicate; ++r) {
      float* d = dst + (int64_t)r * a.rep_stride;
      *d = a.accumulate ? (*d + acc) : acc;
    }
  }
}

int wn_launch_reduce(const WnReduceArgs& a, hipStream_t s) {
  const int64_t total = (int64_t)a.K * a.N;
  if (total <= 0) return WN_OK;
  int blocks = (int)((total + 255) / 256);
  if (blocks > 2048) blocks = 2048;
  int stride = 1;
  if (a.nsplit > 2 * WN_RED_GROUP) {
    const int groups = (a.nsplit + WN_RED_GROUP - 1) / WN_RED_GROUP;
    hipLaunchKernelGGL(wn_reduce_stageA_kernel, dim3(blocks, groups), dim3(256), 0, s,
                       const_cast<float*>(a.slab), a.nsplit, total);
    stride = WN_RED_GROUP;
  }
  hipLaunchKernelGGL(wn_reduce_kernel, dim3(blocks), dim3(256), 0, s, a, stride);
  WN_HIP_CHECK(hipGetLastError());
  return WN_OK;
}
```

### wavenets_amd/csrc/wn_kernels.h

```cpp
#pragma once
#include "wn_common.h"

struct WnTensorDesc { int64_t off; int64_t len; };

struct WnPrepDesc {
  int64_t src_off;
  int64_t dst_off;
  int32_t I;
  int32_t KK;
  int32_t ld;
  int32_t transpose;
  int32_t q_off;
  int32_t j_off;
  int32_t JT;
  int32_t kind;
};
int wn_launch_prep_table(const WnPrepDesc* d_table, int n, const float* params, float* ws,
                         hipStream_t s, int gx = 16);
int wn_launch_prep_one(WnPrepDesc d, const float* params, float* ws, hipStream_t s);
struct WnVecSumArgs { const float* base; int64_t off0; int64_t stride; int32_t count; int32_t len; float* out; };
int wn_launch_vecsum(WnVecSumArgs a, hipStream_t s);

#define WN_MAXSEG 4
struct WnSeg {
  const float* x;
  const float* frag;
  int32_t ldx;
  int32_t K;
  int32_t shift;
  int32_t vec;
  int32_t plane_k;
  int64_t plane_stride;
};
struct WnGemmArgs {
  WnSeg seg[WN_MAXSEG];
  int32_t nseg;
  int32_t B, T;
  int32_t N;
  int32_t JTtot;
  const float* bias;
  const float* rowbias;
  int32_t ld_rowbias;
  const float* addc;
  int32_t ld_addc;
  int32_t act;
  int32_t epi;
  const float* aux;
  int32_t ld_aux;
  const float* aux2;
  int32_t ld_aux2;
  float* y;
  int32_t ldy;
  int32_t vec_out;
  float* y2;
  int32_t ld_y2;
  int32_t absmax_any;
};
int wn_launch_gemm_rows(const WnGemmArgs& a, hipStream_t s);
int wn_gemm_rows16_ok(const WnGemmArgs& a);
int wn_launch_gemm_rows16(const WnGemmArgs& a, const float* w16, const float* absmax_in0,
                          const float* absmax_in1, float* absmax_out, hipStream_t s);

struct WnGemmPlanesArgs {
  const float* z;
  int64_t plane_stride;
  int32_t ld, plane_k, nplanes;
  const float* w16;
  const float* bias;
  int32_t act;
  float* y; int32_t ldy;
  int32_t N;
  int32_t B, T;
  float* absmax_out;
  int32_t bwd;
  const float* absmax_in;
  const float* aux; int32_t ld_aux;
  int32_t nshift; int32_t shift[4];
  int32_t cat_loss;
  const int32_t* target;
  float gscale;
  float* loss_rows;
  float* sample_out;
  float inv_lv;
  uint64_t seed, offset;
};
int wn_gemm_planes16s_supported(int N, int plane_k, int nplanes, int ld, int ldy);
int wn_gemm_taps16s_supported(int N, int plane_k, int ntaps, int ld, int ldy);
int wn_launch_gemm_planes16s(const WnGemmPlanesArgs& a, hipStream_t s);

struct WnWgradArgs {
  const float* x; int32_t ldx; int32_t K; int32_t shift;
  const float* g; int32_t ldg; int32_t N;
  int32_t B, T;
  int32_t splits_per_b;
  float* slab;
  float* slab_bias;
};
int wn_wgrad_choose_splits(int B, int T, int K, int N);
int wn_launch_wgrad(const WnWgradArgs& a, hipStream_t s);
struct WnWgJob {
  int64_t x_off, g_off, out_off, bias_off;
  int64_t gmax_off;
  int32_t ldx, ldg, K, N, shift, k0, n0, pad_;
};
struct WnWgLayer {
  int64_t x_off, du_off, z_off, go_off;
  int64_t dwd_off, dbd_off, dwr_off, dbr_off;
  int64_t gmax_u_off, gmax_h_off;
  int32_t dilation, ldz;
};
int wn_wgrad_layer_supported(int R, int D, int KS);
int wn_launch_wgrad_layers(const WnWgLayer* d_layers, int nlayers, int R, float* ws, float* slab, int64_t P, int B,
                           int T, int splits_per_b, hipStream_t s, int inner = 0);
struct WnWgPair {
  int64_t x_off, g_off;
  int64_t w_off, b_off;
  int64_t gmax_off;
  int32_t shift;
  union { int32_t pad_; int32_t nseg; };
  union { int64_t g2_off; int64_t seg_stride; };
  int64_t w2_off, b2_off, gmax2_off;
};
int wn_wgrad_pair_kind(int K, int N);
int wn_launch_wgrad_pairs(int kind, const WnWgPair* d_jobs, int njobs, float* ws, float* slab, int64_t P, int B, int T,
                          int splits_per_b, hipStream_t s);
int wn_wgrad_tr_kind(int K, int N, int taps);
int wn_launch_wgrad_tr(int kind, const WnWgPair* d_jobs, int njobs, float* ws, float* slab, int64_t P, int B, int T,
                       int splits_per_b, hipStream_t s, float* slab2 = nullptr, int64_t P2 = 0);
struct WnBwdPairArgs {
  const float* gu_in;
  const float* gx_res;
  const float* gf;
  const float* ag;
  const float* z; int32_t ldz;
  float* gx_out;
  float* gu_out;
  const float* wx16;
  const float* wu16;
  const float* am_gu_in; const float* am_gf;
  float* am_gx; float* am_gu;
  int32_t B, T, dil;
};
int wn_bwd_pair_supported(int R, int D, int KS, int F0);
int wn_launch_bwd_pair(const WnBwdPairArgs& a, hipStream_t s);
int wn_bwd_s128_supported(int R, int D, int KS, int F0);
int wn_launch_bwd_s128(const WnBwdPairArgs& a, hipStream_t s);
int wn_wgrad_skip_supported(int D, int S, int KZ);
int wn_launch_wgrad_skip(const float* z, int ldz, const float* g, int ldg, int64_t rows, int KZ, int S, int D,
                         int nsplit, float* slab, int64_t P, int64_t w_off0, int64_t w_stride, int64_t b_off0,
                         int64_t b_stride, int nblocks, const float* gmax, hipStream_t s);
int wn_wgrad_tile_k();
int wn_wgrad_tile_n();
int wn_launch_wgrad_batched(const WnWgJob* d_jobs, int njobs, float* ws, float* slab, int64_t P, int B, int T,
                            int splits_per_b, hipStream_t s, bool exact_fp32 = false);
int wn_launch_reduce_table(const float* slab, int nsplit, int64_t P, float* out, const WnTensorDesc* d_table,
                           int n, hipStream_t s, const WnTensorDesc* h_table = nullptr);
struct WnReduceArgs {
  const float* slab; int32_t nsplit; int32_t K; int32_t N;
  float* out; int32_t seg_len; int64_t seg_stride; int32_t accumulate;
  int32_t replicate; int64_t rep_stride;
};
int wn_launch_reduce(const WnReduceArgs& a, hipStream_t s);

struct WnLayerFwdArgs {
  const float* x;
  const float* frag_d;
  const float* frag_r;
  const float* bias_d;
  const float* bias_r;
  const float* cb;
  float* x_out;
  float* o_out;
  float* z_out; int32_t ldz;
  float* ag_out;
  const float* res;
  const float* xt[3];
  int32_t B, T, R, D, KS, dilation, residual;
  float* absmax_out;
};
int wn_layer_fwd_supported(int R, int D, int KS);
int wn_layer_fwd_f16_supported(int R, int D, int KS);
int wn_launch_layer_fwd_f16(const WnLayerFwdArgs& a, hipStream_t s);
size_t wn_frag16_floats(int I, int KK);
int wn_layer_fwd_s128_supported(int R, int D, int KS);
int wn_launch_layer_fwd_s128(const WnLayerFwdArgs& a, hipStream_t s);
int wn_launch_layer_fwd(const WnLayerFwdArgs& a, hipStream_t s);
int wn_gen_block128_supported(int R, int D, int KS);
int wn_launch_gen_block128(const WnLayerFwdArgs& a, hipStream_t s);

struct WnGenBlock {
  int64_t ring_off;
  int64_t w16d_off;
  int64_t w16r_off;
  int64_t bias_d_off;
  int64_t bias_r_off;
  int64_t cb_off;
  int32_t nslots, dilation;
};
struct WnGenStepArgs {
  const float* params;
  float* ws;
  const WnGenBlock* blocks;
  const float* xin;
  const float* causal_w;
  const float* causal_b;
  int64_t zrow_off;
  int64_t hrow_off;
  int64_t skip_w16_off;
  int64_t skip_bias_off;
  int64_t skiprow_off;
  int32_t skip_tiles, skip_ld;
  int32_t skip_act, pad1_;
  int64_t u0_off;
  int64_t tau;
  int32_t B, nblocks, residual;
  int32_t ntiles;
  unsigned long long* ts;
  int64_t bias_r_off0, bias_r_stride;
  WnGenBlock blk0[3];
  float* guard;
};
struct WnGen128Args {
  const float* params;
  float* ws;
  const WnGenBlock* blocks;
  int64_t zrow_off;
  int64_t hrow_off;
  int64_t tau;
  int32_t B, nblocks, residual;
  float* guard;
  int64_t skip_w16_off, skip_bias_off, skiprow_off;
  int32_t skip_act;
  const float* xin; const float* causal_w; const float* causal_b;
  int32_t ntiles; uint32_t epoch; int64_t relay_off; unsigned* tmo;
  unsigned long long* ts;
  int32_t mute_block;
};
int wn_launch_gen_chain128(const WnGen128Args& a, hipStream_t s);
int wn_launch_gen_relay128(const WnGen128Args& a, hipStream_t s);
int64_t wn_gen_relay128_floats(int B, int nblocks);
struct WnEmit { float* out; int length; int step; float* xin_slot; };
#define WN_EMIT_NONE (WnEmit{nullptr, 0, 0, nullptr})
struct WnSampleCtl {
  float T, inv_T;
  int32_t top_k;
  float top_p;
  __host__ __device__ bool on() const { return T != 1.0f || top_k > 0 || top_p > 0.f; }
};
#define WN_SAMPLE_CTL_OFF (WnSampleCtl{1.0f, 1.0f, 0, 0.f})
#define WN_GEN_HEAD_MAX 4
struct WnGenHeadArgs {
  const float* params;
  float* ws;
  int64_t in_off;
  int64_t out_off;
  int64_t w16_off[WN_GEN_HEAD_MAX];
  int64_t bias_off[WN_GEN_HEAD_MAX];
  int32_t K[WN_GEN_HEAD_MAX], N[WN_GEN_HEAD_MAX], act[WN_GEN_HEAD_MAX];
  int32_t in_ld, nlayers, B;
  int64_t f32_w_off, f32_bias_off;
  int32_t f32_K, f32_N;
  int32_t tail, mix_M, mix_kind;
  float inv_lv;
  uint64_t seed, offset;
  float* samp;
  WnEmit em;
  float* guard;
  WnSampleCtl ctl;
};
int wn_launch_gen_head(const WnGenHeadArgs& a, hipStream_t s);
int wn_gen_blocks_supported(int R, int D, int KS);
int wn_gen_chain_max_blocks();
int64_t wn_gen_u0_floats(int B, int nblocks, int D);
int wn_gen_skip_fusable(int S);
int wn_launch_gen_blocks(const WnGenStepArgs& a, int R, int KS, int what, hipStream_t s);
int wn_launch_gen_head_pre(const WnGenHeadArgs& a, const WnGenStepArgs& g, int R, int KS, hipStream_t s);

int wn_launch_add(const float* a, const float* b, float* out, int64_t n, hipStream_t s);
int wn_launch_fill(float* p, float v, int64_t n, hipStream_t s);
int wn_launch_dact_mul(const float* g, const float* y, float* out, int64_t n, int act, hipStream_t s);
uint32_t wn_dropout_key(uint64_t seed, int block, uint64_t step);
int wn_launch_dropout(const float* x, const float* g_res, float* out, int64_t n, float rate, uint32_t key,
                      float* absmax_out, hipStream_t s);
int wn_launch_gate(const float* u, int64_t rows, int D, float* ag, float* z, int ldz, hipStream_t s);
int wn_launch_cond_scatter(const float* tmp, const float* params, int64_t b_off0, int64_t b_stride, int B, int N, int D2,
                           float* cb, hipStream_t s);
int wn_launch_cond_gather(const float* slab, int64_t P, int spb, int64_t bd_off0, int64_t bd_stride, int B, int N, int D2,
                          float* dcb, hipStream_t s);
int wn_launch_cond_wgrad(const float* m, const float* dcb, int B, int Cc, int N, int D2, float* grads, int64_t w_off0,
                         int64_t w_stride, int64_t b_off0, int64_t b_stride, hipStream_t s);
int wn_launch_skip_fold(const float* params, int64_t ws_off0, int64_t ws_stride, int64_t wf0_off, int64_t bf0_off,
                        const float* bsum, int N, int D, int S, int F0, float* V, float* bfold, float* wsall, hipStream_t s);
int wn_launch_sgemm_small(const float* A, int64_t sai, int64_t sak, const float* B, int64_t sbk, int64_t sbj, float* C, int ldc,
                          int M, int N, int K, hipStream_t s);
int wn_launch_sgemm_small_batched(const float* A, int64_t sai, int64_t sak, int64_t za, const float* B, int64_t sbk, int64_t sbj,
                                  int64_t zb, float* C, int ldc, int64_t zc, int M, int N, int K, int nz, const float* bias,
                                  int act, hipStream_t s, int zk = 0);
int wn_launch_skip_scatter(const float* Y, const float* colsum, int64_t ws_off0, int64_t ws_stride, int64_t bs_off0,
                           int64_t bs_stride, int64_t bf0_off, int N, int D, int S, int F0, float* grads, hipStream_t s);
int wn_inconv_wgrad_supported(int R, int KS);
int wn_launch_inconv_wgrad(const float* x, const float* g, int B, int T, int R, int KS, int splits_per_b, float* slab,
                           int64_t P, int64_t w_off, int64_t b_off, hipStream_t s);
int wn_launch_inconv_fwd(const float* x, const float* w, const float* bias, int B, int T, int R, int KS, float* y,
                         float* absmax_out, hipStream_t s);
int wn_launch_guard_flag(const float* absmax, float limit, int enabled, float* out, hipStream_t s);
int wn_launch_guard_accumulate(const float* src, float* dst, hipStream_t s);
int wn_launch_batch_reduce(const float* slab, int B, int splits, int N, float* out, hipStream_t s);
int64_t wn_colsum_scratch_floats(int B, int C);
int wn_launch_colsum_per_batch(const float* g, int B, int T, int C, float* out, float* scratch, hipStream_t s);
int wn_launch_quantize(const float* x, int32_t* idx, int64_t n, int bits, hipStream_t s);
int wn_launch_dequantize(const int32_t* idx, float* x, int64_t n, int bits, hipStream_t s);
int wn_launch_mulaw(const float* x, float* y, int64_t n, hipStream_t s);
int wn_launch_inv_mulaw(const float* y, float* x, int64_t n, hipStream_t s);

int wn_launch_softmax(const float* logits, float* probs, int64_t rows, int C, hipStream_t s);
int wn_launch_cat_loss(const float* logits, const int32_t* target, int64_t rows, int C,
                       float gscale, float* loss_rows, float* g_logits, float* absmax_out, hipStream_t s,
                       float* sample_out = nullptr, int bits = 8, uint64_t seed = 0, uint64_t offset = 0);
int wn_launch_cat_loss_probs(const float* probs, const int32_t* target, int64_t rows, int C,
                             float* loss_rows, hipStream_t s);
int wn_launch_mix_loss(const float* pred, const float* y, int64_t rows, int M, int bits, int kind,
                       float gscale, float* loss_rows, float* g_pred, float* absmax_out, hipStream_t s);
int wn_launch_sum(const float* v, int64_t n, float scale, float* out, float* scratch, hipStream_t s);
int wn_launch_sqdiff_sum(const float* a, const float* b, int64_t n, float scale, float* out, float* scratch, hipStream_t s);

int wn_launch_sample_det(const float* pred, int64_t rows, int C, int M, int bits, float* out, hipStream_t s,
                         WnEmit em = WN_EMIT_NONE);
int wn_launch_sample_rand(const float* pred, int64_t rows, int C, int M, int bits, int kind, uint64_t seed, uint64_t offset,
                          float* out, hipStream_t s, WnSampleCtl ctl = WN_SAMPLE_CTL_OFF, WnEmit em = WN_EMIT_NONE);
int wn_sample_from_logits_supported(int C);
int wn_launch_sample_rand_cat_logits(const float* logits, int64_t rows, int C, int bits, uint64_t seed, uint64_t offset,
                                     float* out, hipStream_t s, WnSampleCtl ctl = WN_SAMPLE_CTL_OFF, WnEmit em = WN_EMIT_NONE);
int wn_sample_top_k_max_classes();

int wn_launch_sumsq(const float* g, const WnTensorDesc* d_table, int n, float* norms2, hipStream_t s);
int wn_launch_clip(float* g, const WnTensorDesc* d_table, int n, float clipnorm, float* norms2, hipStream_t s);
int wn_launch_axpy_table(float* y, const float* x, const WnTensorDesc* d_table, int n, float coef,
                         hipStream_t s);
int wn_launch_adam(float* p, const float* g, float* m, float* v, const WnTensorDesc* d_table, int n,
                   const float* norms2, float clipnorm, float alpha, float beta1, float beta2,
                   float eps, const float* skip_flag, hipStream_t s);
int wn_launch_adam_ema(float* p, const float* g, float* m, float* v, float* a, const WnTensorDesc* d_table, int n,
                       const float* norms2, float clipnorm, float alpha, float beta1, float beta2,
                       float eps, float momentum, int first, int overwrite, const float* skip_flag, hipStream_t s);
```

### wavenets_amd/csrc/wn_loss.hip

```cpp
#include <algorithm>

#include "wn_kernels.h"
#include "wn_sample.h"

__global__ __launch_bounds__(256) void wn_softmax_kernel(const float* logits, float* probs,
                                                         int64_t rows, int C) {
  const int lane = threadIdx.x & 63;
  const int64_t row = (int64_t)blockIdx.x * 4 + (threadIdx.x >> 6);
  if (row >= rows) return;
  WnSoftmaxLoop(logits + row * C, C, lane).each([&](int j, float q) { probs[row * C + j] = q; });
}
int wn_launch_softmax(const float* logits, float* probs, int64_t rows, int C, hipStream_t s) {
  if (rows <= 0) return WN_OK;
  hipLaunchKernelGGL(wn_softmax_kernel, dim3((unsigned)((rows + 3) / 4)), dim3(256), 0, s, logits,
                     probs, rows, C);
  WN_HIP_CHECK(hipGetLastError());
  return WN_OK;
}

__global__ __launch_bounds__(256) void wn_cat_loss256_kernel(const float* logits, const int32_t* target,
                                                             int64_t rows, int C, float gscale,
                                                             float* loss_rows, float* g_logits, float* absmax_out,
                                                             float* sample_out, float inv_lv, uint64_t seed, uint64_t offset) {
  __shared__ float qs[4][256];
// ... 52 lines not shown
  if (sample_out && C > 256) { wn_set_error("cat_loss: the in-kernel sample draw needs <= 256 classes"); return WN_E_UNSUPPORTED; }
  const float inv_lv = sample_out ? 1.0f / (float)(1 << (bits - 1)) : 0.f;
  if (C <= 256) {
    const int64_t wgs = std::min<int64_t>((rows + 3) / 4, 256 * 8);
    hipLaunchKernelGGL(wn_cat_loss256_kernel, dim3((unsigned)wgs), dim3(256), 0, s, logits, target, rows, C, gscale,
                       loss_rows, g_logits, absmax_out, sample_out, inv_lv, seed, offset);
  } else {
    hipLaunchKernelGGL(wn_cat_loss_kernel, dim3((unsigned)((rows + 3) / 4)), dim3(256), 0, s, logits,
                       target, rows, C, gscale, loss_rows, g_logits, absmax_out);
  }
  WN_HIP_CHECK(hipGetLastError());
  return WN_OK;
}

__global__ __launch_bounds__(256) void wn_cat_loss_probs_kernel(const float* probs,
                                                                const int32_t* target, int64_t rows,
                                                                int C, float* loss_rows) {
  const int lane = threadIdx.x & 63;
  const int64_t row = (int64_t)blockIdx.x * 4 + (threadIdx.x >> 6);
  if (row >= rows) return;
  const float* q = probs + row * C;
  float S = 0.f;
  for (int j = lane; j < C; j += 64) S += wn_ce_clip(q[j]);
  S = wn_wave_sum(S);
  const float pt = wn_ce_clip(q[wn_ce_target(target[row], C)]);
  if (lane == 0) loss_rows[row] = wn_ce_loss(pt, S);
}
int wn_launch_cat_loss_probs(const float* probs, const int32_t* target, int64_t rows, int C,
                             float* loss_rows, hipStream_t s) {
  if (rows <= 0) return WN_OK;
  hipLaunchKernelGGL(wn_cat_loss_probs_kernel, dim3((unsigned)((rows + 3) / 4)), dim3(256), 0, s,
                     probs, target, rows, C, loss_rows);
  WN_HIP_CHECK(hipGetLastError());
  return WN_OK;
}

#define WN_MAXMIX 32
__device__ __forceinline__ double wn_sigmoid_d(double x) { return 1.0 / (1.0 + exp(-x)); }
__device__ __forceinline__ double wn_dsigmoid_d(double x) { return wn_sigmoid_d(x) * wn_sigmoid_d(-x); }
__device__ __forceinline__ bool wn_logistic_bin(double a, double b, double& hi, double& lo) {
  const bool up = a + b > 0.0;
  hi = up ? -b : a;
  lo = up ? -a : b;
  return up;
}
__global__ void wn_mix_loss_kernel(const float* pred, const float* y, int64_t rows, int M, int bits,
                                   int kind, float gscale, float* loss_rows, float* g_pred, float* absmax_out) {
  const int64_t row = (int64_t)blockIdx.x * blockDim.x + threadIdx.x;
  if (row >= rows) return;
  const float* p = pred + row * 3 * M;
  const double yy = (double)y[row];
  double w[WN_MAXMIX], comp[WN_MAXMIX];
  double wm = -INFINITY;
  for (int k = 0; k < M; ++k) wm = fmax(wm, (double)p[k]);
  double wz = 0.0;
  for (int k = 0; k < M; ++k) { w[k] = exp((double)p[k] - wm); wz += w[k]; }
  const double winv = 1.0 / wz;
  const double halfbit = 0.5 / (double)(1 << bits);
  const double sqrt2pi = sqrt(2.0 * 3.14159265359);
  double lik = 0.0;
  for (int k = 0; k < M; ++k) {
    w[k] *= winv;
    const double mu = (double)p[M + k];
    const double ls = fmax((double)p[2 * M + k], -7.0);
    if (kind == 1) {
      const double inv = exp(-ls);
      double hi, lo;
      wn_logistic_bin((yy - mu + halfbit) * inv, (yy - mu - halfbit) * inv, hi, lo);
      comp[k] = wn_sigmoid_d(hi) - wn_sigmoid_d(lo);
    } else {
      const double sc = exp(ls);
      const double xx = fmin((yy - mu) / sc, 1e8);
      comp[k] = exp(-0.5 * xx * xx) / (sc * sqrt2pi);
    }
    lik += w[k] * comp[k];
  }
  loss_rows[row] = (float)(-log(lik));
  if (!g_pred) return;
  float* g = g_pred + row * 3 * M;
  const double dl = -(double)gscale / lik;
  for (int k = 0; k < M; ++k) {
    const double mu = (double)p[M + k];
    const double lsr = (double)p[2 * M + k];
    const double ls = fmax(lsr, -7.0);
    const double lsmask = lsr >= -7.0 ? 1.0 : 0.0;
    g[k] = (float)(dl * (w[k] * comp[k] - w[k] * lik));
    if (kind == 1) {
      const double inv = exp(-ls);
      double hi, lo;
      const bool up = wn_logistic_bin((yy - mu + halfbit) * inv, (yy - mu - halfbit) * inv, hi, lo);
      const double dhi = wn_dsigmoid_d(hi), dlo = wn_dsigmoid_d(lo);
      g[M + k] = (float)(dl * (-w[k] * inv * (up ? dlo - dhi : dhi - dlo)));
      g[2 * M + k] = (float)(dl * lsmask * (-w[k] * (hi * dhi - lo * dlo)));
    } else {
      const double sc = exp(ls);
      const double xr = (yy - mu) / sc;
      const double xx = fmin(xr, 1e8);
      const double xmask = xr <= 1e8 ? 1.0 : 0.0;
      const double pdf = comp[k];
      g[M + k] = (float)(dl * w[k] * pdf * xx / sc * xmask);
      g[2 * M + k] = (float)(dl * lsmask * w[k] * pdf * (xx * xx * xmask - 1.0));
    }
  }
  if (absmax_out) {
    float gmax = 0.f;
    for (int k = 0; k < 3 * M; ++k) gmax = fmaxf(gmax, fabsf(g[k]));
    wn_absmax_publish(absmax_out, gmax);
  }
}
int wn_launch_mix_loss(const float* pred, const float* y, int64_t rows, int M, int bits, int kind,
                       float gscale, float* loss_rows, float* g_pred, float* absmax_out, hipStream_t s) {
  if (rows <= 0) return WN_OK;
  if (M < 1 || M > WN_MAXMIX) { wn_set_error("mix_loss: num_mixtures %d unsupported (max %d)", M, WN_MAXMIX); return WN_E_UNSUPPORTED; }
  hipLaunchKernelGGL(wn_mix_loss_kernel, dim3((unsigned)((rows + 255) / 256)), dim3(256), 0, s, pred,
                     y, rows, M, bits, kind, gscale, loss_rows, g_pred, absmax_out);
  WN_HIP_CHECK(hipGetLastError());
  return WN_OK;
}

__global__ void wn_sum_stage1(const float* v, int64_t n, double* scratch) {
  __shared__ double sm[256];
  double acc = 0.0;
  for (int64_t i = (int64_t)blockIdx.x * blockDim.x + threadIdx.x; i < n;
       i += (int64_t)gridDim.x * blockDim.x)
    acc += (double)v[i];
  sm[threadIdx.x] = acc;
  __syncthreads();
  for (int o = 128; o > 0; o >>= 1) {
    if (threadIdx.x < o) sm[threadIdx.x] += sm[threadIdx.x + o];
    __syncthreads();
  }
  if (threadIdx.x == 0) scratch[blockIdx.x] = sm[0];
}
__global__ void wn_sum_stage2(const double* scratch, int nb, float scale, float* out) {
  __shared__ double sm[256];
  double acc = 0.0;
  for (int i = threadIdx.x; i < nb; i += blockDim.x) acc += scratch[i];
  sm[threadIdx.x] = acc;
  __syncthreads();
  for (int o = 128; o > 0; o >>= 1) {
    if (threadIdx.x < o) sm[threadIdx.x] += sm[threadIdx.x + o];
    __syncthreads();
  }
  if (threadIdx.x == 0) out[0] = (float)(sm[0] * (double)scale);
}
int wn_launch_sum(const float* v, int64_t n, float scale, float* out, float* scratch, hipStream_t s) {
  int nb = wn_blocks(n, 256, 1024);
  hipLaunchKernelGGL(wn_sum_stage1, dim3(nb), dim3(256), 0, s, v, n, reinterpret_cast<double*>(scratch));
  hipLaunchKernelGGL(wn_sum_stage2, dim3(1), dim3(256), 0, s, reinterpret_cast<const double*>(scratch), nb, scale, out);
  WN_HIP_CHECK(hipGetLastError());
  return WN_OK;
}

__global__ void wn_sqdiff_stage1(const float* a, const float* b, int64_t n, double* scratch) {
  __shared__ double sm[256];
  double acc = 0.0;
  for (int64_t i = (int64_t)blockIdx.x * blockDim.x + threadIdx.x; i < n;
       i += (int64_t)gridDim.x * blockDim.x) {
    const float d = a[i] - b[i];
    acc += (double)(d * d);
  }
  sm[threadIdx.x] = acc;
  __syncthreads();
  for (int o = 128; o > 0; o >>= 1) {
    if (threadIdx.x < o) sm[threadIdx.x] += sm[threadIdx.x + o];
    __syncthreads();
  }
  if (threadIdx.x == 0) scratch[blockIdx.x] = sm[0];
}
int wn_launch_sqdiff_sum(const float* a, const float* b, int64_t n, float scale, float* out, float* scratch, hipStream_t s) {
  int nb = wn_blocks(n, 256, 1024);
  hipLaunchKernelGGL(wn_sqdiff_stage1, dim3(nb), dim3(256), 0, s, a, b, n, reinterpret_cast<double*>(scratch));
  hipLaunchKernelGGL(wn_sum_stage2, dim3(1), dim3(256), 0, s, reinterpret_cast<const double*>(scratch), nb, scale, out);
  WN_HIP_CHECK(hipGetLastError());
  return WN_OK;
}
```

### wavenets_amd/csrc/wn_plan_internal.h

```cpp
#pragma once
#include <math.h>
#include <stdlib.h>
#include <string.h>

#include <algorithm>
#include <mutex>
#include <vector>

#include "../../include/wn_hip.h"
#include "wn_kernels.h"

namespace wnp {

inline int64_t align64(int64_t v) { return (v + 63) & ~(int64_t)63; }
inline int ceil32(int v) { return (v + 31) / 32; }
inline int ceil8(int v) { return (v + 7) / 8 * 8; }

struct TensorInfo {
  int64_t off, len;
  int ndim;
  int64_t shape[3];
  int is_kernel;
};

struct ConvInfo {
  int kernel_t = -1, bias_t = -1;
  int taps = 1, cin = 0, cout = 0, dil = 1;
  int64_t fragF = -1;
  int64_t fragB = -1;
  int64_t fragF_stride = 0, fragB_stride = 0;
  int64_t frag16 = -1;
  int64_t frag16B = -1;
};

struct BlockInfo {
  std::vector<ConvInfo> dil;
  ConvInfo conv1, conv_skip, conv_cond;
  bool has_skip = false, has_cond = false;
  int64_t g16u = -1;
  int64_t f16gate = -1;
  int64_t f16nat = -1;
  int64_t g16uf = -1;
  int64_t d16F[16], d16B[16];
  BlockInfo() { for (int i = 0; i < 16; ++i) d16F[i] = d16B[i] = -1; }
};

struct AbsmaxSlots {
  int nf, N, LPB;
  int gf(int i) const { return i; }
  int gskip() const { return nf; }
  int gu(int b) const { return nf + 1 + b; }
  int gh(int b) const { return nf + 1 + N + b; }
  int gp(int b, int i) const { return nf + 1 + N + (N + 1) + b * (LPB - 1) + i; }
  int count() const { return gp(N, 0); }
};

enum WgFamily { WG_LAYER, WG_LAYER_INNER, WG_TR_PAIRS, WG_GENERIC, WG_GENERIC_FP32 };
enum BwdFamily { BWD_BLOCKS, BWD_PAIR, BWD_S128 };
struct TrainPaths {
  WgFamily wg = WG_GENERIC;
  BwdFamily bwd = BWD_BLOCKS;
  int mtr = 0;
  bool mfused = false;
  bool skipk = false, fold = false, deep16 = false, head_pairs = false;
  bool drop = false, head_split = false, in_split = false, rows32 = true;
  bool layerk() const { return wg == WG_LAYER || wg == WG_LAYER_INNER; }
  bool pairk() const { return wg == WG_TR_PAIRS; }
  bool headpairs() const { return head_pairs && head_split; }
  bool bwd_pairs() const { return bwd != BWD_BLOCKS && !drop && (bwd != BWD_S128 || rows32); }
  bool operator==(const TrainPaths& o) const {
    return wg == o.wg && bwd == o.bwd && mtr == o.mtr && mfused == o.mfused && skipk == o.skipk && fold == o.fold &&
           deep16 == o.deep16 && head_pairs == o.head_pairs && drop == o.drop && head_split == o.head_split &&
           in_split == o.in_split && rows32 == o.rows32;
  }
};

template <class T> struct DevTable {
  T* d = nullptr;
  void release() { if (d) (void)hipFree(d); d = nullptr; }
  int upload(const std::vector<T>& v, size_t min_count = 0) {
    release();
    const size_t n = std::max(v.size(), min_count);
    if (n == 0) return WN_OK;
    WN_HIP_CHECK(hipMalloc((void**)&d, n * sizeof(T)));
    if (!v.empty()) WN_HIP_CHECK(hipMemcpy(d, v.data(), v.size() * sizeof(T), hipMemcpyHostToDevice));
    return WN_OK;
  }
};

struct WgSpan {
  enum Op : uint8_t { INCONV, JOBS, PAIRS, TR, LAYERS, SKIP } op;
  enum Slab : uint8_t { BATCH, HEAD, MFOLD } slab;
  int kind;
  int first, count;
};

struct WgSchedule {
  bool valid = false;
  int B = 0, T = 0, bsplits = 0;
  TrainPaths paths;
  DevTable<WnWgJob> jobs;
  DevTable<WnWgLayer> layers, inner;
  DevTable<WnWgPair> pairs;
  DevTable<WnTensorDesc> cov;
  std::vector<WnTensorDesc> h_cov;
  std::vector<WgSpan> spans;
  int n_side = 0;
  bool overlap = false;
  int cov_head = 0;
  void release() { valid = false; jobs.release(); layers.release(); inner.release(); pairs.release(); cov.release(); }
};

}

struct wn_exec {
  const struct wn_plan* plan = nullptr;
  float drop_rate = 0.f;
  uint64_t drop_seed = 0, drop_step = 0;
  float* step_sample = nullptr; int step_sample_det = 0; uint64_t step_sample_seed = 0, step_sample_off = 0;
  wnp::WgSchedule wg;
  hipStream_t side = nullptr;
  hipEvent_t ev_fork = nullptr, ev_join = nullptr;
  hipEvent_t ev_ffork = nullptr, ev_fjoin = nullptr;
  WnGenBlock* d_gen = nullptr;
  WnGenBlock gen_blk0[3]{};
  int64_t gen_bias_stride = 0;
  int train_phases = 3;
  int gen_B = 0;
  bool gen_chain128 = false;
  std::vector<hipEvent_t> prof_ev;
  std::vector<int> prof_cnt;
  hipEvent_t phase_ev[5] = {nullptr, nullptr, nullptr, nullptr, nullptr};
  bool phase_on = false;
  int prof_used = 0;
  bool prof_on = false;
  std::vector<hipEvent_t> stack_ev;
  std::vector<hipEvent_t> foldprep_ev;
  int foldprep_used = 0;
  int stack_used = 0;
};

struct wn_plan {
  wn_config c;
  int KS, R, D, S, N, LPB, Cout, Sh, Hin, Cc, Dp;
  std::vector<int> dilations;
  std::vector<wnp::TensorInfo> tensors;
  int64_t nparams = 0;
  wnp::ConvInfo causal;
  std::vector<wnp::BlockInfo> blocks;
  std::vector<wnp::ConvInfo> finals, mapping;
  int64_t frag_skipF = -1;
  int64_t frag_condF = -1, frag_condB = -1;
  int64_t frag16_skipF = -1;
  int64_t frag_floats = 0;
  int fold_F0 = 0;
  int64_t frag16_foldF = -1;
  std::vector<WnPrepDesc> prep2;
  WnPrepDesc* d_prep2 = nullptr;
  WnTensorDesc* d_cov_fold = nullptr;
  WnTensorDesc h_cov_fold = {0, 0};
  std::vector<WnPrepDesc> prep;
  std::vector<WnTensorDesc> tdesc, kdesc;
  WnPrepDesc* d_prep = nullptr;
  WnTensorDesc* d_tdesc = nullptr;
  WnTensorDesc* d_kdesc = nullptr;
  bool fused_ok = false, fused16_ok = false;
  bool deep16_ok = false;
  std::mutex tables_mu;
  bool tables_ready = false;
  struct wn_exec* own = nullptr;
};

namespace wnp {
wn_exec& ex(const wn_plan* p);
void exec_release(wn_exec* e);


struct Carver {
  int64_t pos = 0;
  int64_t take(int64_t n) { int64_t o = pos; pos = align64(pos + (n > 0 ? n : 0)); return o; }
};

struct WsLayout {
  int64_t frag, bias_sum;
  std::vector<int64_t> H;
  std::vector<std::vector<int64_t>> P;
  int64_t Z;
  std::vector<int64_t> AG;
  std::vector<std::vector<int64_t>> GP;
  int64_t U;
  int64_t O;
  int64_t skipsum;
  std::vector<int64_t> HA;
  int64_t logits, probs;
  int64_t target, loss_rows, yt;
  int64_t g_skipsum;
  int64_t slab, slab_floats;
  std::vector<int64_t> GU, GH, GO, GF;
  int64_t bslab; int bsplits;
  int64_t hslab; int hsplits; int64_t head_base, head_span;
  int64_t islab; int isplits;
  int64_t vfold, bfold, wsall, mslab, mtot, ytmp;
  std::vector<int64_t> XD;
  int64_t gxd;
  int64_t absmax; int n_absmax;
  int64_t fwd_absmax;
  int64_t sum_scratch;
  std::vector<int64_t> M;
  int64_t cb;
  int64_t dcb, g_m0, g_m1;
  int64_t cbt;
  int64_t total;
};

inline bool al16(const void* p) { return (((uintptr_t)p) & 15) == 0; }

struct Gemm {
  WnGemmArgs a;
  const float* w16_ = nullptr;
  const float* am0_ = nullptr;
  const float* am1_ = nullptr;
  float* amo_ = nullptr;
  Gemm& w16(const float* img) { w16_ = img; return *this; }
  Gemm& absmax(const float* in0, const float* in1, float* out) { am0_ = in0; am1_ = in1; amo_ = out; return *this; }
  Gemm& absmax_fwd(float* out) { amo_ = out; a.absmax_any = out ? 1 : 0; return *this; }
  Gemm(int B, int T, int N, int JTtot) {
    memset(&a, 0, sizeof(a));
    a.B = B; a.T = T; a.N = N; a.JTtot = JTtot; a.act = WN_ACT_LINEAR; a.epi = WN_EPI_PLAIN;
  }
  Gemm& seg(const float* x, int ldx, int K, int shift, const float* frag) {
    WnSeg& s = a.seg[a.nseg++];
    s.x = x; s.ldx = ldx; s.K = K; s.shift = shift; s.frag = frag;
    s.vec = (ldx % 4 == 0 && K % 4 == 0 && al16(x)) ? 1 : 0;
    s.plane_k = 0; s.plane_stride = 0;
    return *this;
  }
  Gemm& seg_planes(const float* x, int plane_k, int64_t plane_stride, int K, const float* frag) {
    seg(x, plane_k, K, 0, frag);
    WnSeg& s = a.seg[a.nseg - 1];
    s.plane_k = plane_k; s.plane_stride = plane_stride;
    s.vec = (plane_k % 4 == 0 && plane_stride % 4 == 0 && al16(x)) ? 1 : 0;
    return *this;
  }
  Gemm& bias(const float* b) { a.bias = b; return *this; }
  Gemm& rowbias(const float* b, int ld) { a.rowbias = b; a.ld_rowbias = ld; return *this; }
  Gemm& addc(const float* c, int ld) { a.addc = c; a.ld_addc = ld; return *this; }
  Gemm& act(int act) { a.act = act; return *this; }
  Gemm& dact(const float* ysaved, int ld, int act) { a.epi = WN_EPI_DACT; a.aux = ysaved; a.ld_aux = ld; a.act = act; return *this; }
  Gemm& gate_bwd(const float* g, int ldg, const float* z, int ldz) {
    a.epi = WN_EPI_GATE_BWD; a.aux = g; a.ld_aux = ldg; a.aux2 = z; a.ld_aux2 = ldz;
    return *this;
  }
  Gemm& gate_fwd(float* sig, int ld) { a.epi = WN_EPI_GATE_FWD; a.y2 = sig; a.ld_y2 = ld; return *this; }
  int run(float* y, int ldy, hipStream_t s) {
    a.y = y; a.ldy = ldy;
    bool v = (a.N % 4 == 0) && (ldy % 4 == 0) && al16(y);
    if (a.bias) v = v && al16(a.bias);
    if (a.addc) v = v && (a.ld_addc % 4 == 0) && al16(a.addc);
    if (a.aux) v = v && (a.ld_aux % 4 == 0) && al16(a.aux);
    if (a.aux2) v = v && (a.ld_aux2 % 4 == 0) && al16(a.aux2);
    if (a.y2) v = v && (a.ld_y2 % 4 == 0) && al16(a.y2);
    a.vec_out = v ? 1 : 0;
    if (w16_ && wn_debug_get(1) != 1 && wn_gemm_rows16_ok(a)) return wn_launch_gemm_rows16(a, w16_, am0_, am1_, amo_, s);
    if (a.epi == WN_EPI_GATE_FWD) { wn_set_error("gate-forward contraction needs the split-precision kernel (alignment / shape)"); return WN_E_UNSUPPORTED; }
    for (int i = 0; i < a.nseg; ++i)
      if (!a.seg[i].frag) { wn_set_error("contraction without an fp32 weight image needs the split-precision kernel"); return WN_E_UNSUPPORTED; }
    return wn_launch_gemm_rows(a, s);
  }
};

struct BlockPtrs {
  int B, T, KS, R, D, S, Cin, depth, act, residual;
  int dil[16];
  const float* Wd[16]; const float* bd[16];
  const float* br; const float* bs; const float* bc;
  const float* Fd[16]; const float* Bd[16]; int64_t Fd_stride[16], Bd_stride[16];
  const float* Fr; const float* Br_;
  const float* Fs; const float* Bs;
  const float* Fc; const float* Bc;
  int Cc;
  const float* cond;
  const float* cb;
  bool fused;
  const float* F16d; const float* F16r;
  const float* G16u; const float* G16x;
  const float* G16uf;
  const float* F16g;
  const float* F16n;
  const float* F16i[16]; const float* G16i[16];
  int JTi[16], JTb[16], JTu;
};

struct BlockBufs {
  const float* x;
  float* P[16];
  float* U;
  float* AG;
  float* Z; int ldz;
  float* O;
  float* x_out;
  const float* xt[3];
  const float* res;
  bool pre_done;
  float* fwd_absmax;
};

struct BlockGrads {
  const float* g_xout;
  const float* g_skip;
  float* g_o_tmp;
  float* g_u;
  float* g_p;
  float* g_pi[16];
  float* g_x;
  float* g_cond;
  float* dWd[16]; float* dbd[16];
  float* dWr; float* dbr; float* dWs; float* dbs; float* dWc; float* dbc;
  float* dcb;
  float* slab;
  bool defer;
  const float* am_gxout; const float* am_gskip;
  float* am_gu; float* am_gx;
  float* am_gp[16];
  const float* g_fold; int fold_F0; const float* am_gfold;
  float drop_rate; uint32_t drop_key; float* g_xd;
};

struct GenRings {
  float* xin;
  std::vector<float*> h;
  std::vector<int> nslots;
  std::vector<std::vector<float*>> hp;
  std::vector<std::vector<int>> nslots_p;
};

inline bool m16(int v) { return v > 0 && v % 16 == 0; }
inline bool m32(int v) { return v >= 64 && v % 32 == 0; }

int ensure_device_tables(wn_plan* p);
WsLayout make_layout(const wn_plan* p, int B, int T, bool training);
bool deep16(const wn_plan* p);
bool cond_small(const wn_plan* p);
bool fold_ok(const wn_plan* p);
bool head_pairs_ok(const wn_plan* p);
TrainPaths train_paths(const wn_plan* p);
TrainPaths train_paths(const wn_plan* p, const wn_exec& e, const WsLayout& L, int64_t rows);
int64_t slab_need(int B, int T, int K, int N);
int wgrad(const float* x, int ldx, int K, int shift, const float* g, int ldg, int N, int B, int T,
          float* dW, float* db, float* per_batch, float* slab, hipStream_t s);
int block_forward(const BlockPtrs& k, const BlockBufs& f, hipStream_t s);
int block_backward(const BlockPtrs& k, const BlockBufs& f, const BlockGrads& g, hipStream_t s);
struct LossFuse {
  const int32_t* target; float gscale; float* loss_rows; float* g_logits; float* absmax_out;
  float* sample_out; float inv_lv; uint64_t seed, offset;
  bool done;
};
bool loss_fusable(const wn_plan* p, int64_t rows);
BlockPtrs block_ptrs(const wn_plan* p, int b, const float* params, const float* fragbase, int B, int T);
void deep16_ptrs(const wn_plan* p, int b, const float* fragbase, BlockPtrs& k);
int forward_core(wn_plan* p, const float* params, const float* x, bool prep, const float* cond, int B,
                 int T, bool training, float* ws, const WsLayout& L, hipStream_t s, const GenRings* rings = nullptr,
                 LossFuse* lf = nullptr);
int shift_split(const float* x_full, int B, int T, float* inputs, float* y_true, hipStream_t s);
int loss_stage(wn_plan* p, int B, int T, int global_batch, bool want_grad, float* ws, const WsLayout& L,
               float* loss_out, float* absmax_out, hipStream_t s, bool fused_done = false);

}

int wn_sampling_check(const char* who, const wn_sampling* sp, int head, int classes, WnSampleCtl* ctl);
```

### wavenets_amd/csrc/wn_train.hip

```cpp
#include "wn_plan_internal.h"

namespace {
using namespace wnp;

void add_jobs(std::vector<WnWgJob>& jobs, int64_t x_off, int ldx, int K, int shift, int64_t g_off, int ldg, int N,
              int64_t out_off, int64_t bias_off, int64_t gmax_off) {
  const int tk = wn_wgrad_tile_k(), tn = wn_wgrad_tile_n();
  for (int k0 = 0; k0 < K; k0 += tk)
    for (int n0 = 0; n0 < N; n0 += tn) {
      WnWgJob j;
      memset(&j, 0, sizeof(j));
      j.x_off = x_off; j.g_off = g_off; j.out_off = out_off; j.bias_off = (k0 == 0) ? bias_off : -1;
      j.gmax_off = gmax_off;
      j.ldx = ldx; j.ldg = ldg; j.K = K; j.N = N; j.shift = shift; j.k0 = k0; j.n0 = n0;
      jobs.push_back(j);
    }
}

int ensure_schedule(const wn_plan* p, wn_exec& e, const WsLayout& L, int B, int T, const TrainPaths& tp) {
  WgSchedule& g = e.wg;
  if (g.valid && g.B == B && g.T == T && g.bsplits == L.bsplits && g.paths == tp) return WN_OK;
  const bool layerk = tp.layerk(), pairk = tp.pairk(), fold = tp.fold;
  std::vector<WnWgLayer> wgl, wgli;
  std::vector<WnWgPair> pairs[3];
// ... 1 lines not shown
  std::vector<WnWgJob> jobs;
  std::vector<WnTensorDesc> cov;
  auto cover = [&](int t) { WnTensorDesc d; d.off = p->tensors[t].off; d.len = p->tensors[t].len; cov.push_back(d); };
  const AbsmaxSlots slot{(int)p->finals.size(), p->N, p->LPB};
  const int64_t am_skip = L.absmax + slot.gskip();
  auto am_GU = [&](int b) { return L.absmax + slot.gu(b); };
  auto am_GH = [&](int b) { return L.absmax + slot.gh(b); };
  auto am_GP = [&](int b, int i) { return tp.deep16 ? L.absmax + slot.gp(b, i) : (int64_t)-1; };
  if (!tp.in_split)
    for (int t = 0; t < p->KS; ++t)
      add_jobs(jobs, L.probs, 1, 1, p->KS - 1 - t, L.GH[0], p->R, p->R,
               p->tensors[p->causal.kernel_t].off + (int64_t)t * p->R,
               t == p->KS - 1 ? p->tensors[p->causal.bias_t].off : -1, am_GH(0));
  cover(p->causal.kernel_t); cover(p->causal.bias_t);
  for (int b = 0; b < p->N; ++b) {
    const BlockInfo& bi = p->blocks[b];
    const ConvInfo& c = bi.dil.back();
    const int64_t zoff = L.Z + (int64_t)b * B * T * p->Dp;
    if (layerk) {
      const int64_t xin0 = tp.drop ? L.XD[b] : L.H[b];
      for (int i = 0; i + 1 < p->LPB; ++i) {
        const ConvInfo& ci = bi.dil[i];
        WnWgLayer w;
        memset(&w, 0, sizeof(w));
        w.x_off = i == 0 ? xin0 : L.P[b][i - 1];
        w.du_off = L.GP[b][i];
        w.dwd_off = p->tensors[ci.kernel_t].off; w.dbd_off = p->tensors[ci.bias_t].off;
        w.dwr_off = w.dbr_off = -1; w.z_off = w.go_off = 0;
        w.gmax_u_off = am_GP(b, i); w.gmax_h_off = -1;
        w.dilation = ci.dil; w.ldz = p->Dp;
        wgli.push_back(w);
        cover(ci.kernel_t); cover(ci.bias_t);
      }
      WnWgLayer w;
      w.x_off = p->LPB > 1 ? L.P[b][p->LPB - 2] : xin0;
      w.du_off = L.GU[b]; w.z_off = zoff; w.ldz = p->Dp;
      w.go_off = p->S == 0 ? L.GO[b] : L.GH[b + 1];
      w.dwd_off = p->tensors[c.kernel_t].off; w.dbd_off = p->tensors[c.bias_t].off;
      w.dwr_off = p->tensors[bi.conv1.kernel_t].off; w.dbr_off = p->tensors[bi.conv1.bias_t].off;
      w.gmax_u_off = am_GU(b); w.gmax_h_off = p->S == 0 ? am_skip : am_GH(b + 1);
      w.dilation = c.dil;
      wgl.push_back(w);
    } else if (pairk) {
      const int64_t xoff = tp.drop ? L.XD[b] : L.H[b];
      {
        WnWgPair w;
        memset(&w, 0, sizeof(w));
        w.x_off = xoff; w.g_off = L.GU[b]; w.shift = c.dil;
        w.w_off = p->tensors[c.kernel_t].off;
        w.b_off = p->tensors[c.bias_t].off;
        w.gmax_off = am_GU(b);
        pairs[1].push_back(w);
      }
      WnWgPair w;
      memset(&w, 0, sizeof(w));
      w.x_off = zoff; w.g_off = p->S == 0 ? L.GO[b] : L.GH[b + 1]; w.shift = 0;
      w.w_off = p->tensors[bi.conv1.kernel_t].off; w.b_off = p->tensors[bi.conv1.bias_t].off;
      w.gmax_off = p->S == 0 ? am_skip : am_GH(b + 1);
      w.g2_off = w.w2_off = w.b2_off = w.gmax2_off = -1;
      if (tp.mfused) {
        w.g2_off = L.GF[0]; w.w2_off = (int64_t)b * p->D * p->fold_F0;
        w.b2_off = b == 0 ? (int64_t)p->N * p->D * p->fold_F0 : -1;
        w.gmax2_off = L.absmax + slot.gf(0);
      }
      pairs[2].push_back(w);
    } else {
    for (int i = 0; i < p->LPB; ++i) {
      const ConvInfo& ci = bi.dil[i];
      const bool lastc = i == p->LPB - 1;
      const int64_t xo = i == 0 ? (tp.drop ? L.XD[b] : L.H[b]) : L.P[b][i - 1];
      const int kc = i == 0 ? p->R : p->D, nc = lastc ? 2 * p->D : p->D;
      for (int t = 0; t < p->KS; ++t)
        add_jobs(jobs, xo, kc, kc, (p->KS - 1 - t) * ci.dil, lastc ? L.GU[b] : L.GP[b][i], nc, nc,
                 p->tensors[ci.kernel_t].off + (int64_t)t * kc * nc,
                 t == p->KS - 1 ? p->tensors[ci.bias_t].off : -1, lastc ? am_GU(b) : am_GP(b, i));
      if (!lastc) { cover(ci.kernel_t); cover(ci.bias_t); }
    }
    add_jobs(jobs, zoff, p->Dp, p->D, 0, p->S == 0 ? L.GO[b] : L.GH[b + 1], p->R, p->R,
             p->tensors[bi.conv1.kernel_t].off, p->tensors[bi.conv1.bias_t].off, p->S == 0 ? am_skip : am_GH(b + 1));
    }
    cover(bi.dil.back().kernel_t); cover(bi.dil.back().bias_t);
    cover(bi.conv1.kernel_t); cover(bi.conv1.bias_t);
    if (bi.has_skip && p->c.use_skip && !fold) {
      if (!tp.skipk)
        add_jobs(jobs, zoff, p->Dp, p->D, 0, L.g_skipsum, p->S, p->S,
                 p->tensors[bi.conv_skip.kernel_t].off, p->tensors[bi.conv_skip.bias_t].off, am_skip);
      cover(bi.conv_skip.kernel_t); cover(bi.conv_skip.bias_t);
    }
  }
  if (tp.mtr != 0) {
    const int per = 256 / p->D;
    for (int b0 = 0; b0 < p->N; b0 += per) {
      WnWgPair w;
      memset(&w, 0, sizeof(w));
      w.x_off = L.Z + (int64_t)b0 * B * T * p->Dp;
      w.seg_stride = (int64_t)B * T * p->Dp;
      w.nseg = std::min(per, p->N - b0);
      w.g_off = L.GF[0]; w.shift = 0;
      w.w_off = (int64_t)b0 * p->D * p->fold_F0;
      w.b_off = b0 == 0 ? (int64_t)p->N * p->D * p->fold_F0 : -1;
      w.gmax_off = L.absmax + slot.gf(0);
      w.w2_off = w.b2_off = w.gmax2_off = -1;
      pairs[0].push_back(w);
    }
  }
  const int head_first = (int)jobs.size(), cov_head = (int)cov.size();
  for (size_t i = fold ? 1 : 0; i < p->finals.size(); ++i) {
    const ConvInfo& c = p->finals[i];
    const int64_t xin = (i == 0) ? (p->c.use_skip ? L.skipsum : L.H[p->N]) : L.HA[i - 1];
    if (tp.headpairs() && wn_wgrad_pair_kind(c.cin, c.cout) != 0) {
      WnWgPair w;
      memset(&w, 0, sizeof(w));
      w.x_off = xin; w.g_off = L.GF[i]; w.shift = 0;
      w.w_off = p->tensors[c.kernel_t].off; w.b_off = p->tensors[c.bias_t].off;
      w.gmax_off = L.absmax + slot.gf((int)i);
      const int kind = wn_wgrad_pair_kind(c.cin, c.cout);
      hpairs[kind].push_back(w);
      if (kind == 5) {
        w.g_off += 128; w.w_off += 128; w.b_off += 128;
        hpairs[kind].push_back(w);
      }
    } else {
      add_jobs(jobs, xin, c.cin, c.cin, 0, L.GF[i], c.cout, c.cout, p->tensors[c.kernel_t].off,
               p->tensors[c.bias_t].off, L.absmax + slot.gf((int)i));
    }
    cover(c.kernel_t); cover(c.bias_t);
  }
  std::vector<WnWgPair> all;
  int pfirst[3], hfirst[6] = {0, 0, 0, 0, 0, 0};
  for (int kd = 0; kd <= 2; ++kd) { pfirst[kd] = (int)all.size(); all.insert(all.end(), pairs[kd].begin(), pairs[kd].end()); }
  for (int kd = 1; kd <= 5; ++kd) { hfirst[kd] = (int)all.size(); all.insert(all.end(), hpairs[kd].begin(), hpairs[kd].end()); }
  std::vector<WgSpan> spans;
  auto span = [&](WgSpan::Op op, WgSpan::Slab slab, int kind, int first, size_t count) {
    if (count > 0) spans.push_back(WgSpan{op, slab, kind, first, (int)count});
  };
  const int njobs = (int)jobs.size();
  const bool head_own = tp.head_split && (head_first < njobs || tp.headpairs());
  span(WgSpan::INCONV, WgSpan::BATCH, 0, 0, tp.in_split);
  span(WgSpan::JOBS, WgSpan::BATCH, tp.wg == WG_GENERIC_FP32, 0, head_own ? head_first : njobs);
  if (head_own) span(WgSpan::JOBS, WgSpan::HEAD, 0, head_first, njobs - head_first);
  for (int kd = 1; kd <= 5; ++kd) {
    const int trk = kd == 1 ? 3 : (kd == 3 ? 4 : (kd == 5 ? 5 : (kd == 2 ? 2 : 0)));
    if (trk != 0 && tp.pairk()) span(WgSpan::TR, WgSpan::HEAD, trk, hfirst[kd], hpairs[kd].size());
    else span(WgSpan::PAIRS, WgSpan::HEAD, kd, hfirst[kd], hpairs[kd].size());
  }
  const int n_side = (int)spans.size();
  span(WgSpan::TR, WgSpan::BATCH, 1, pfirst[1], pairs[1].size());
  span(WgSpan::TR, WgSpan::BATCH, tp.mfused ? 6 : 2, pfirst[2], pairs[2].size());
  span(WgSpan::LAYERS, WgSpan::BATCH, 0, 0, wgl.size());
  span(WgSpan::LAYERS, WgSpan::BATCH, 1, 0, wgli.size());
  if (tp.mtr != 0) span(WgSpan::TR, WgSpan::MFOLD, tp.mtr, pfirst[0], pairs[0].size());
  else if (tp.fold) span(WgSpan::SKIP, WgSpan::MFOLD, 0, 0, !tp.mfused);
  else span(WgSpan::SKIP, WgSpan::BATCH, 0, 0, tp.skipk);
  g.valid = false;
  int rc = g.jobs.upload(jobs, 1);
  if (!rc) rc = g.cov.upload(cov);
  if (!rc) rc = g.layers.upload(wgl);
  if (!rc) rc = g.inner.upload(wgli);
  if (!rc) rc = g.pairs.upload(all);
  if (rc) return rc;
  g.h_cov.swap(cov); g.spans.swap(spans);
  g.n_side = n_side; g.overlap = layerk || pairk; g.cov_head = head_own ? cov_head : (int)g.h_cov.size();
  g.B = B; g.T = T; g.bsplits = L.bsplits; g.paths = tp;
  g.valid = true;
  return WN_OK;
}

struct TrainCall {
  wn_exec& e;
  wn_plan* p; const float* params; const float* x_full; const float* cond;
  int B, T, global_batch, n_replicas;
  float* grads; float* loss_out; float* pred_out; float* ws; hipStream_t s;
  WsLayout L;
  int64_t rows;
  float* inputs;
  const float* fragbase; float* slab;
  float* am; AbsmaxSlots slot;
  int nf; float* am_gskip;
  const float* mlast = nullptr;
  TrainPaths tp;
  bool cond_batched = false;
  int64_t pm = 0;
  float* am_GF(int i) const { return am + slot.gf(i); }
  float* am_GU(int b) const { return am + slot.gu(b); }
  float* am_GH(int b) const { return am + slot.gh(b); }
  float* am_GP(int b, int i) const { return am + slot.gp(b, i); }
  struct Strided { int64_t off, stride; };
  Strided strided(int t0, int t1) const { return {p->tensors[t0].off, p->N > 1 ? p->tensors[t1].off - p->tensors[t0].off : 0}; }
  Strided skip_w{0, 0}, skip_b{0, 0};

  int forward_and_loss() {
    int rc;
    { const int rcs = shift_split(x_full, B, T, inputs, ws + L.yt, s); if (rcs) return rcs; }
    if (e.phase_on) (void)hipEventRecord(e.phase_ev[0], s);
    WN_HIP_CHECK(hipMemsetAsync(am, 0, L.n_absmax * sizeof(float), s));
    LossFuse lf;
    memset(&lf, 0, sizeof(lf));
    const bool fuse = !pred_out && loss_fusable(p, rows);
    if (fuse) {
      rc = wn_launch_quantize(ws + L.yt, reinterpret_cast<int32_t*>(ws + L.target), rows, p->c.bits, s);
      if (rc) return rc;
      lf.target = reinterpret_cast<const int32_t*>(ws + L.target);
      lf.gscale = 1.0f / (float)global_batch;
      lf.loss_rows = ws + L.loss_rows; lf.g_logits = ws + L.GF.back(); lf.absmax_out = am_GF(nf - 1);
      if (e.step_sample && !e.step_sample_det) {
        lf.sample_out = e.step_sample; lf.inv_lv = 1.0f / (float)(1 << (p->c.bits - 1));
        lf.seed = e.step_sample_seed; lf.offset = e.step_sample_off;
      }
    }
    rc = forward_core(p, params, inputs, true, cond, B, T, true, ws, L, s, nullptr, fuse ? &lf : nullptr);
    if (rc) return rc;
    if (lf.done && lf.sample_out) e.step_sample = nullptr;
    if (e.phase_on) (void)hipEventRecord(e.phase_ev[1], s);
    rc = loss_stage(p, B, T, global_batch, true, ws, L, loss_out, am_GF(nf - 1), s, lf.done);
    if (rc) return rc;
    if (pred_out) {
      if (p->c.head == WN_HEAD_CATEGORICAL) rc = wn_launch_softmax(ws + L.logits, pred_out, rows, p->Cout, s);
      else rc = hipMemcpyAsync(pred_out, ws + L.logits, rows * p->Cout * sizeof(float), hipMemcpyDeviceToDevice, s) == hipSuccess ? WN_OK : WN_E_HIP;
      if (rc) return rc;
    }
    if (e.step_sample) {
      float* so = e.step_sample;
      e.step_sample = nullptr;
      if (p->c.head == WN_HEAD_CATEGORICAL) {
        if (e.step_sample_det) {
          wn_set_error("step sample: deterministic categorical draws go through wn_sample_waveform");
          return WN_E_UNSUPPORTED;
        }
        rc = wn_launch_sample_rand_cat_logits(ws + L.logits, rows, p->Cout, p->c.bits, e.step_sample_seed, e.step_sample_off, so, s);
      } else {
        if (e.step_sample_det) rc = wn_launch_sample_det(ws + L.logits, rows, p->Cout, p->c.num_mixtures, p->c.bits, so, s);
        else rc = wn_launch_sample_rand(ws + L.logits, rows, p->Cout, p->c.num_mixtures, p->c.bits, p->c.head, e.step_sample_seed, e.step_sample_off, so, s);
      }
      if (rc) return rc;
    }
    if (p->c.l2_reg_factor > 0.f) {
      float* norms = ws + L.loss_rows;
      rc = wn_launch_sumsq(params, p->d_kdesc, (int)p->kdesc.size(), norms, s);
      if (rc) return rc;
      rc = wn_launch_sum(norms, (int64_t)p->kdesc.size(), p->c.l2_reg_factor / (float)n_replicas, loss_out + 1, ws + L.sum_scratch, s);
      if (rc) return rc;
    } else {
      rc = wn_launch_fill(loss_out + 1, 0.f, 1, s);
      if (rc) return rc;
    }
    rc = wn_launch_guard_flag(ws + L.fwd_absmax, WN_RANGE_LIMIT * (e.drop_rate > 0.f ? 1.f - e.drop_rate : 1.f),
                              wn_debug_get(1) != 1, loss_out + 2, s);
    if (rc) return rc;
    if (e.phase_on) (void)hipEventRecord(e.phase_ev[2], s);
    return WN_OK;
  }

  int cond_block_bwd(const BlockInfo& bi) {
    const ConvInfo& c = bi.conv_cond;
    int r = wgrad(mlast, p->Cc, p->Cc, 0, ws + L.dcb, 2 * p->D, 2 * p->D, 1, B, grads + p->tensors[c.kernel_t].off,
                  grads + p->tensors[c.bias_t].off, nullptr, slab, s);
    if (r) return r;
    return Gemm(1, B, p->Cc, ceil32(p->Cc)).seg(ws + L.dcb, 2 * p->D, 2 * p->D, 0, fragbase + c.fragB)
        .addc(ws + L.g_m0, p->Cc).run(ws + L.g_m0, p->Cc, s);
  }

  int head_backward() {
    int rc;
    float* head_out = p->c.use_skip ? ws + L.g_skipsum : ws + L.GH[p->N];
    for (int i = (int)p->finals.size() - 1; i >= (tp.fold ? 1 : 0); --i) {
      const ConvInfo& c = p->finals[i];
      float* dst = (i == 0) ? head_out : ws + L.GF[i - 1];
      if (c.frag16B >= 0 && wn_debug_get(1) != 1 && wn_gemm_planes16s_supported(c.cin, c.cout, 1, c.cout, c.cin) &&
          (int64_t)rows * c.cout * 4 < ((int64_t)1 << 32)) {
        WnGemmPlanesArgs ga;
        memset(&ga, 0, sizeof(ga));
        ga.z = ws + L.GF[i]; ga.ld = c.cout; ga.plane_k = c.cout; ga.nplanes = 1;
        ga.w16 = fragbase + c.frag16B; ga.act = p->c.activation;
        ga.y = dst; ga.ldy = c.cin; ga.N = c.cin; ga.B = B; ga.T = T;
        ga.bwd = 1; ga.absmax_in = am_GF(i);
        ga.absmax_out = i > 0 ? am_GF(i - 1) : (p->c.use_skip ? am_gskip : am_GH(p->N));
        if (i > 0) { ga.aux = ws + L.HA[i - 1]; ga.ld_aux = c.cin; }
        rc = wn_launch_gemm_planes16s(ga, s);
        if (rc) return rc;
        continue;
      }
      Gemm gm(B, T, c.cin, ceil32(c.cin));
      gm.seg(ws + L.GF[i], c.cout, c.cout, 0, fragbase + c.fragB);
      if (i > 0) gm.dact(ws + L.HA[i - 1], c.cin, p->c.activation);
      if (c.frag16B >= 0)
        gm.w16(fragbase + c.frag16B).absmax(am_GF(i), nullptr, i > 0 ? am_GF(i - 1) : (p->c.use_skip ? am_gskip : am_GH(p->N)));
      rc = gm.run(dst, c.cin, s);
      if (rc) return rc;
    }
    return WN_OK;
  }

  int chain_backward() {
    int rc;
    const float* g_skip = (p->c.use_skip && !tp.fold) ? ws + L.g_skipsum : nullptr;
    if (p->c.use_skip) {
      rc = wn_launch_fill(ws + L.GH[p->N], 0.f, rows * p->R, s);
      if (rc) return rc;
    }
    const bool pairk = tp.bwd_pairs();
    for (int b = p->N - 1; b >= 0; --b) {
      BlockPtrs k = block_ptrs(p, b, params, fragbase, B, T);
      deep16_ptrs(p, b, fragbase, k);
      const BlockInfo& bi = p->blocks[b];
      if (pairk && b < p->N - 1) {
        const BlockPtrs k1 = block_ptrs(p, b + 1, params, fragbase, B, T);
        WnBwdPairArgs a;
        memset(&a, 0, sizeof(a));
        a.gu_in = ws + L.GU[b + 1]; a.gx_res = ws + L.GH[b + 2]; a.gf = ws + L.GF[0];
        a.ag = ws + L.AG[b]; a.z = ws + L.Z + (int64_t)b * rows * p->Dp; a.ldz = p->Dp;
        a.gx_out = ws + L.GH[b + 1]; a.gu_out = ws + L.GU[b];
        a.wx16 = k1.G16x; a.wu16 = k.G16uf;
        a.am_gu_in = am_GU(b + 1); a.am_gf = am_GF(0); a.am_gx = am_GH(b + 1); a.am_gu = am_GU(b);
        a.B = B; a.T = T; a.dil = k1.dil[0];
        if (!a.wx16 || !a.wu16) { wn_set_error("bwd_pair: weight images missing"); return WN_E_UNSUPPORTED; }
        rc = tp.bwd == BWD_S128 ? wn_launch_bwd_s128(a, s) : wn_launch_bwd_pair(a, s);
        if (rc) return rc;
        if (b == 0) {
          Gemm gm(B, T, p->R, ceil32(p->R));
          for (int t = 0; t < p->KS; ++t)
            gm.seg(ws + L.GU[0], 2 * p->D, 2 * p->D, -(p->KS - 1 - t) * k.dil[0], k.Bd[0] + t * k.Bd_stride[0]);
          if (p->c.use_residual) gm.addc(ws + L.GH[1], p->R);
          gm.w16(k.G16x).absmax(am_GU(0), nullptr, am_GH(0));
          rc = gm.run(ws + L.GH[0], p->R, s);
          if (rc) return rc;
        }
        continue;
      }
      BlockBufs f;
      memset(&f, 0, sizeof(f));
      f.x = tp.drop ? ws + L.XD[b] : ws + L.H[b];
      for (int i = 0; i + 1 < p->LPB; ++i) f.P[i] = ws + L.P[b][i];
      f.AG = ws + L.AG[b];
      f.Z = ws + L.Z + (int64_t)b * rows * p->Dp; f.ldz = p->Dp;
      BlockGrads bg;
      memset(&bg, 0, sizeof(bg));
      bg.defer = true;
      for (int i = 0; i + 1 < p->LPB; ++i) bg.g_pi[i] = ws + L.GP[b][i];
      if (tp.deep16)
        for (int i = 0; i + 1 < p->LPB; ++i) bg.am_gp[i] = am_GP(b, i);
      if (tp.drop) {
        bg.drop_rate = e.drop_rate; bg.drop_key = wn_dropout_key(e.drop_seed, b, e.drop_step); bg.g_xd = ws + L.gxd;
      }
      bg.g_xout = (p->c.use_skip && b == p->N - 1 && p->S == 0) ? nullptr : ws + L.GH[b + 1];
      bg.g_skip = g_skip;
      bg.g_o_tmp = p->S == 0 ? ws + L.GO[b] : nullptr;
      bg.g_u = ws + L.GU[b];
      bg.g_x = pairk ? nullptr : ws + L.GH[b];
      bg.dcb = (bi.has_cond && !cond_batched) ? ws + L.dcb : nullptr;
      bg.slab = slab;
      bg.am_gxout = bg.g_xout ? am_GH(b + 1) : nullptr;
      bg.am_gskip = g_skip ? am_gskip : nullptr;
      bg.am_gu = am_GU(b); bg.am_gx = am_GH(b);
      if (tp.fold) { bg.g_fold = ws + L.GF[0]; bg.fold_F0 = p->fold_F0; bg.am_gfold = am_GF(0); }
      rc = block_backward(k, f, bg, s);
      if (rc) return rc;
      if (p->S == 0 && bg.g_xout == nullptr && g_skip) {
        WN_HIP_CHECK(hipMemcpyAsync(ws + L.GO[b], g_skip, rows * p->R * sizeof(float), hipMemcpyDeviceToDevice, s));
      }
      if (bi.has_cond && !cond_batched) {
        rc = cond_block_bwd(bi);
        if (rc) return rc;
      }
    }
    return WN_OK;
  }

  int fold_weight_gradients() {
    const int F0 = p->fold_F0;
    int rc = wn_launch_reduce_table(ws + L.mslab, B * L.bsplits, pm, ws + L.mtot, p->d_cov_fold, 1, s, &p->h_cov_fold);
    if (rc) return rc;
    const ConvInfo& c0 = p->finals[0];
    const int nd1 = p->N * p->D + 1;
    const float* wf0 = params + p->tensors[c0.kernel_t].off;
    rc = wn_launch_sgemm_small(ws + L.mtot, F0, 1, wf0, 1, F0, ws + L.ytmp, p->S, nd1, p->S, F0, s);
    if (rc) return rc;
    const int nzk = (nd1 + 127) / 128;
    if ((int64_t)nzk * p->S * F0 <= L.slab_floats) {
      rc = wn_launch_sgemm_small_batched(ws + L.wsall, 1, p->S, (int64_t)128 * p->S, ws + L.mtot, F0, 1, (int64_t)128 * F0, slab, F0,
                                         (int64_t)p->S * F0, p->S, F0, nd1, nzk, nullptr, 0, s, 128);
      if (rc) return rc;
      WnVecSumArgs v;
      v.base = slab; v.off0 = 0; v.stride = (int64_t)p->S * F0; v.count = nzk; v.len = p->S * F0;
      v.out = grads + p->tensors[c0.kernel_t].off;
      rc = wn_launch_vecsum(v, s);
    } else
    rc = wgrad(ws + L.wsall, p->S, p->S, 0, ws + L.mtot, F0, F0, 1, nd1, grads + p->tensors[c0.kernel_t].off, nullptr, nullptr,
               slab, s);
    if (rc) return rc;
    return wn_launch_skip_scatter(ws + L.ytmp, ws + L.mtot + (int64_t)p->N * p->D * F0, skip_w.off, skip_w.stride, skip_b.off,
                                  skip_b.stride, p->tensors[c0.bias_t].off, p->N, p->D, p->S, F0, grads, s);
  }

  int cond_weight_gradients() {
    int rc;
    const int D2 = 2 * p->D;
    const BlockInfo& b0 = p->blocks[0]; const BlockInfo& b1 = p->blocks[p->N > 1 ? 1 : 0];
    const Strided db = strided(b0.dil.back().bias_t, b1.dil.back().bias_t);
    const Strided cw = strided(b0.conv_cond.kernel_t, b1.conv_cond.kernel_t), cbi = strided(b0.conv_cond.bias_t, b1.conv_cond.bias_t);
    rc = wn_launch_cond_gather(ws + L.bslab, p->nparams, L.bsplits, db.off, db.stride, B, p->N, D2, ws + L.cbt, s);
    if (rc) return rc;
    if (cond_small(p) && (int64_t)p->N * B * p->Cc <= L.slab_floats) {
      rc = wn_launch_sgemm_small_batched(ws + L.cbt, p->N * D2, 1, D2, params + cw.off, 1, D2, cw.stride,
                                         slab, p->Cc, (int64_t)B * p->Cc, B, p->Cc, D2, p->N, nullptr, 0, s);
      if (rc) return rc;
      WnVecSumArgs v;
      v.base = slab; v.off0 = 0; v.stride = (int64_t)B * p->Cc; v.count = p->N; v.len = B * p->Cc; v.out = ws + L.g_m0;
      rc = wn_launch_vecsum(v, s);
    } else
    rc = Gemm(1, B, p->Cc, ceil32(p->Cc)).seg(ws + L.cbt, p->N * D2, p->N * D2, 0, fragbase + p->frag_condB).run(ws + L.g_m0, p->Cc, s);
    if (rc) return rc;
    return wn_launch_cond_wgrad(mlast, ws + L.cbt, B, p->Cc, p->N, D2, grads, cw.off, cw.stride, cbi.off, cbi.stride, s);
  }

  int launch(const WgSpan& sp, hipStream_t st) {
    const WgSchedule& g = e.wg;
    float* out = ws + L.bslab; int64_t pitch = p->nparams; int splits = L.bsplits;
    if (sp.slab == WgSpan::HEAD) { out = ws + L.hslab - L.head_base; pitch = L.head_span; splits = L.hsplits; }
    if (sp.slab == WgSpan::MFOLD) { out = ws + L.mslab; pitch = pm; }
    switch (sp.op) {
      case WgSpan::INCONV:
        return wn_launch_inconv_wgrad(inputs, ws + L.GH[0], B, T, p->R, p->KS, L.isplits, ws + L.islab, (int64_t)(p->KS + 1) * p->R,
                                      0, (int64_t)p->KS * p->R, st);
      case WgSpan::JOBS: return wn_launch_wgrad_batched(g.jobs.d + sp.first, sp.count, ws, out, pitch, B, T, splits, st, sp.kind != 0);
      case WgSpan::PAIRS: return wn_launch_wgrad_pairs(sp.kind, g.pairs.d + sp.first, sp.count, ws, out, pitch, B, T, splits, st);
      case WgSpan::TR:
        return wn_launch_wgrad_tr(sp.kind, g.pairs.d + sp.first, sp.count, ws, out, pitch, B, T, splits, st,
                                  sp.kind == 6 ? ws + L.mslab : nullptr, sp.kind == 6 ? pm : 0);
      case WgSpan::LAYERS: return wn_launch_wgrad_layers(sp.kind ? g.inner.d : g.layers.d, sp.count, p->R, ws, out, pitch, B, T, splits, st, sp.kind);
      case WgSpan::SKIP:
        if (sp.slab == WgSpan::MFOLD)
          return wn_launch_wgrad_skip(ws + L.Z, p->Dp, ws + L.GF[0], p->fold_F0, rows, p->N * p->D, p->fold_F0, p->D, B * splits, out, pitch,
                                      0, (int64_t)p->D * p->fold_F0, (int64_t)p->N * p->D * p->fold_F0, 0, 1, am_GF(0), st);
        return wn_launch_wgrad_skip(ws + L.Z, p->Dp, ws + L.g_skipsum, p->S, rows, p->N * p->D, p->S, p->D, B * splits, out, pitch,
                                    skip_w.off, skip_w.stride, skip_b.off, skip_b.stride, p->N, am_gskip, st);
    }
    return WN_E_INVALID;
  }

  int weight_gradients() {
    int rc;
    const WgSchedule& g = e.wg;
    if (e.phase_on) (void)hipEventRecord(e.phase_ev[3], s);
    const bool fork = g.overlap && wn_debug_get(9) != 1;
    if (fork && !e.side) {
      WN_HIP_CHECK(hipStreamCreateWithFlags(&e.side, hipStreamNonBlocking));
      WN_HIP_CHECK(hipEventCreateWithFlags(&e.ev_fork, hipEventDisableTiming));
      WN_HIP_CHECK(hipEventCreateWithFlags(&e.ev_join, hipEventDisableTiming));
    }
    struct SideJoin {
      wn_exec& e; hipStream_t s; bool armed;
      ~SideJoin() {
        if (!armed) return;
        if (hipEventRecord(e.ev_join, e.side) != hipSuccess || hipStreamWaitEvent(s, e.ev_join, 0) != hipSuccess)
          (void)hipStreamSynchronize(e.side);
      }
    } side_join{e, s, false};
    if (fork) {
      WN_HIP_CHECK(hipEventRecord(e.ev_fork, s));
      WN_HIP_CHECK(hipStreamWaitEvent(e.side, e.ev_fork, 0));
      side_join.armed = true;
    }
    size_t i = 0;
    for (; i < (size_t)g.n_side; ++i)
      if ((rc = launch(g.spans[i], fork ? e.side : s))) return rc;
    if (fork) WN_HIP_CHECK(hipEventRecord(e.ev_join, e.side));
    for (; i < g.spans.size(); ++i)
      if ((rc = launch(g.spans[i], s))) return rc;
    if (tp.fold && (rc = fold_weight_gradients())) return rc;
    if (fork) { WN_HIP_CHECK(hipStreamWaitEvent(s, e.ev_join, 0)); side_join.armed = false; }
    if (cond_batched && (rc = cond_weight_gradients())) return rc;
    const int cov0 = tp.in_split ? 2 : 0, ncov = (int)g.h_cov.size(), cov1 = g.cov_head;
    rc = wn_launch_reduce_table(ws + L.bslab, B * L.bsplits, p->nparams, grads, g.cov.d + cov0, cov1 - cov0, s, g.h_cov.data() + cov0);
    if (rc) return rc;
    if (tp.in_split && (rc = wn_launch_reduce_table(ws + L.islab, B * L.isplits, (int64_t)(p->KS + 1) * p->R, grads, g.cov.d, 2, s, g.h_cov.data())))
      return rc;
    if (cov1 < ncov && (rc = wn_launch_reduce_table(ws + L.hslab - L.head_base, B * L.hsplits, L.head_span, grads, g.cov.d + cov1, ncov - cov1,
                                                    s, g.h_cov.data() + cov1)))
      return rc;
    if (!p->c.use_skip && p->S > 0) {
      for (const BlockInfo& bi : p->blocks) {
        rc = wn_launch_fill(grads + p->tensors[bi.conv_skip.kernel_t].off, 0.f, p->tensors[bi.conv_skip.kernel_t].len, s);
        if (!rc) rc = wn_launch_fill(grads + p->tensors[bi.conv_skip.bias_t].off, 0.f, p->tensors[bi.conv_skip.bias_t].len, s);
        if (rc) return rc;
      }
    }
    return WN_OK;
  }

  int mapping_backward() {
    int rc;
    if (p->c.cond_inputs > 0) {
      const float* gm_cur = ws + L.g_m0;
      float* gm_other = ws + L.g_m1;
      for (int j = (int)p->mapping.size() - 1; j >= 0; --j) {
        const ConvInfo& c = p->mapping[j];
        const float* yin = (j == 0) ? cond : ws + L.M[j - 1];
        rc = wn_launch_dact_mul(gm_cur, ws + L.M[j], gm_other, (int64_t)B * c.cout, p->c.mapping_activation, s);
        if (rc) return rc;
        if (cond_small(p)) {
          rc = wn_launch_sgemm_small_batched(yin, 1, c.cin, 0, gm_other, c.cout, 1, 0, grads + p->tensors[c.kernel_t].off, c.cout, 0,
                                             c.cin, c.cout, B, 1, nullptr, 0, s);
          if (rc) return rc;
          WnVecSumArgs v;
          v.base = gm_other; v.off0 = 0; v.stride = c.cout; v.count = B; v.len = c.cout; v.out = grads + p->tensors[c.bias_t].off;
          rc = wn_launch_vecsum(v, s);
          if (rc) return rc;
          if (j > 0) {
            float* dst = const_cast<float*>(gm_cur);
            rc = wn_launch_sgemm_small_batched(gm_other, c.cout, 1, 0, params + p->tensors[c.kernel_t].off, 1, c.cout, 0, dst, c.cin, 0,
                                               B, c.cin, c.cout, 1, nullptr, 0, s);
            if (rc) return rc;
          }
          continue;
        }
        rc = wgrad(yin, c.cin, c.cin, 0, gm_other, c.cout, c.cout, 1, B, grads + p->tensors[c.kernel_t].off,
                   grads + p->tensors[c.bias_t].off, nullptr, slab, s);
        if (rc) return rc;
        if (j > 0) {
          float* dst = const_cast<float*>(gm_cur);
          rc = Gemm(1, B, c.cin, ceil32(c.cin)).seg(gm_other, c.cout, c.cout, 0, fragbase + c.fragB).run(dst, c.cin, s);
          if (rc) return rc;
        }
      }
    }
    return WN_OK;
  }

  int backward() {
    int rc;
    fragbase = ws + L.frag;
    slab = ws + L.slab;
    if (p->c.cond_inputs > 0) {
      mlast = p->mapping.empty() ? cond : ws + L.M.back();
      rc = wn_launch_fill(ws + L.g_m0, 0.f, (int64_t)B * p->Cc, s);
      if (rc) return rc;
    }
    cond_batched = p->frag_condB >= 0;
    tp = train_paths(p, e, L, rows);
    pm = (int64_t)p->N * p->D * p->fold_F0 + p->fold_F0;
    if (p->blocks[0].has_skip) {
      const BlockInfo& b0 = p->blocks[0]; const BlockInfo& b1 = p->blocks[p->N > 1 ? 1 : 0];
      skip_w = strided(b0.conv_skip.kernel_t, b1.conv_skip.kernel_t); skip_b = strided(b0.conv_skip.bias_t, b1.conv_skip.bias_t);
    }
    rc = ensure_schedule(p, e, L, B, T, tp);
    if (rc) return rc;
    if ((rc = head_backward())) return rc;
    if ((rc = chain_backward())) return rc;
    if ((rc = weight_gradients())) return rc;
    if ((rc = mapping_backward())) return rc;
    if (p->c.l2_reg_factor > 0.f) {
      rc = wn_launch_axpy_table(grads, params, p->d_kdesc, (int)p->kdesc.size(), 2.0f * p->c.l2_reg_factor / (float)n_replicas, s);
      if (rc) return rc;
    }
    if (e.phase_on) {
      (void)hipEventRecord(e.phase_ev[4], s);
    }

    return WN_OK;
  }
};

}

extern "C" int wn_plan_set_train_phases(wn_plan* p, int32_t phases) {
  if (!p || phases < 1 || phases > 3) { wn_set_error("set_train_phases: 1 (forward + loss), 2 (backward), 3 (both)"); return WN_E_INVALID; }
  wnp::ex(p).train_phases = phases;
  return WN_OK;
}

extern "C" int wn_train_fwd_bwd(wn_plan* p, const float* params, const float* x_full, const float* cond,
                                int32_t B, int32_t T, int32_t global_batch, int32_t n_replicas, float* grads,
                                float* loss_out, float* pred_out, float* workspace, int64_t ws_floats,
                                void* stream) {
  if (!p || !params || !x_full || !workspace || !loss_out || !grads || B < 1 || T < 1) { wn_set_error("train_fwd_bwd: bad arguments"); return WN_E_INVALID; }
  TrainCall c{wnp::ex(p)};
  c.p = p; c.params = params; c.x_full = x_full; c.cond = cond; c.B = B; c.T = T;
  c.global_batch = global_batch > 0 ? global_batch : B;
  c.n_replicas = n_replicas > 0 ? n_replicas : 1;
  c.grads = grads; c.loss_out = loss_out; c.pred_out = pred_out; c.ws = workspace; c.s = (hipStream_t)stream;
  c.L = make_layout(p, B, T, true);
  if (ws_floats < c.L.total) { wn_set_error("train_fwd_bwd: workspace too small (%lld < %lld floats)", (long long)ws_floats, (long long)c.L.total); return WN_E_INVALID; }
  c.rows = (int64_t)B * T;
  c.inputs = workspace + c.L.probs;
  c.am = workspace + c.L.absmax;
  c.nf = (int)p->finals.size();
  c.slot = AbsmaxSlots{c.nf, p->N, p->LPB};
  c.am_gskip = c.am + c.slot.gskip();
  const int phases = c.e.train_phases;
  int rc = WN_OK;
  if (phases & 1) rc = c.forward_and_loss();
  if (!rc && (phases & 2)) rc = c.backward();
  return rc;
}

extern "C" int wn_adam_step_guarded(wn_plan* p, float* params, const float* grads, float* m, float* v, int64_t step,
                                    float lr, float beta1, float beta2, float eps, float clipnorm, float* scratch,
                                    const float* skip_flag, void* stream) {
  if (!p || !params || !grads || !m || !v || !scratch || step < 1) { wn_set_error("adam_step: bad arguments"); return WN_E_INVALID; }
  hipStream_t s = (hipStream_t)stream;
  int rc = ensure_device_tables(p);
  if (rc) return rc;
  const int n = (int)p->tdesc.size();
  if (clipnorm > 0.f) {
    rc = wn_launch_sumsq(grads, p->d_tdesc, n, scratch, s);
    if (rc) return rc;
  }
  const double alpha = (double)lr * sqrt(1.0 - pow((double)beta2, (double)step)) / (1.0 - pow((double)beta1, (double)step));
  return wn_launch_adam(params, grads, m, v, p->d_tdesc, n, scratch, clipnorm, (float)alpha, beta1, beta2, eps, skip_flag, s);
}

extern "C" int wn_adam_step_ema(wn_plan* p, float* params, const float* grads, float* m, float* v, float* ema, int64_t step,
                                float lr, float beta1, float beta2, float eps, float clipnorm, float ema_momentum,
                                int32_t ema_overwrite, float* scratch, const float* skip_flag, void* stream) {
  if (!p || !params || !grads || !m || !v || !ema || !scratch || step < 1) { wn_set_error("adam_step_ema: bad arguments"); return WN_E_INVALID; }
  if (!std::isfinite(ema_momentum) || ema_momentum < 0.f || ema_momentum > 1.f) {
    wn_set_error("adam_step_ema: ema_momentum must be finite and in [0, 1] (got %g)", (double)ema_momentum);
    return WN_E_INVALID;
  }
  if (ema_overwrite != 0 && ema_overwrite != 1) { wn_set_error("adam_step_ema: ema_overwrite must be 0 or 1 (got %d)", (int)ema_overwrite); return WN_E_INVALID; }
  hipStream_t s = (hipStream_t)stream;
  int rc = ensure_device_tables(p);
  if (rc) return rc;
  const int n = (int)p->tdesc.size();
  if (clipnorm > 0.f) {
    rc = wn_launch_sumsq(grads, p->d_tdesc, n, scratch, s);
    if (rc) return rc;
  }
  const double alpha = (double)lr * sqrt(1.0 - pow((double)beta2, (double)step)) / (1.0 - pow((double)beta1, (double)step));
  return wn_launch_adam_ema(params, grads, m, v, ema, p->d_tdesc, n, scratch, clipnorm, (float)alpha, beta1, beta2, eps,
                            ema_momentum, step == 1 ? 1 : 0, (int)ema_overwrite, skip_flag, s);
}
// ... 15 lines not shown
```

Measured before the change: 23.06 million.

## Fuse training prologue, loss tail, coverage reductions and vectorize optimizer kernels

Several launch-reducing changes land together. The shift/split, quantize and absmax memset are folded into the input-conv kernel and the prep kernel. Loss sum and guard flag become one tail kernel, and the three gradient-slab reductions become a single table-driven kernel. The skip-gradient zero-fill moves onto the side stream during forward, Adam/EMA use float4 accesses, and sumsq uses 1024 threads with unrolled loads. This trims launch count and memory latency in a small-kernel-dominated step, at the cost of more complex alignment and stream-ordering logic.

```diff
diff --git a/wavenets_amd/csrc/wn_elem.hip b/wavenets_amd/csrc/wn_elem.hip
--- a/wavenets_amd/csrc/wn_elem.hip
+++ b/wavenets_amd/csrc/wn_elem.hip
@@ -127,20 +127,36 @@
   return WN_OK;
 }
 
-__global__ void wn_sumsq_kernel(const float* g, const WnTensorDesc* table, float* norms2) {
-  __shared__ double sm[256];
+__device__ inline int64_t wn_sumsq_groups(int64_t len, int lane) {
+  return len > lane + 768 ? (len - lane - 768 + 1023) / 1024 : 0;
+}
+#define WN_SUMSQ_THREADS 1024
+__global__ void __launch_bounds__(WN_SUMSQ_THREADS)
+wn_sumsq_kernel(const float* g, const WnTensorDesc* table, float* norms2) {
+  __shared__ double sm[WN_SUMSQ_THREADS];
   const WnTensorDesc d = table[blockIdx.x];
   const float* p = g + d.off;
-  double a0 = 0.0, a1 = 0.0, a2 = 0.0, a3 = 0.0;
-  int64_t i = threadIdx.x;
-  for (; i + 3 * 256 < d.len; i += 4 * 256) {
-    const float v0 = p[i], v1 = p[i + 256], v2 = p[i + 512], v3 = p[i + 768];
-    a0 += (double)v0 * (double)v0; a1 += (double)v1 * (double)v1;
-    a2 += (double)v2 * (double)v2; a3 += (double)v3 * (double)v3;
-  }
-  for (; i < d.len; i += 256) a0 += (double)p[i] * (double)p[i];
-  const double acc = (a0 + a1) + (a2 + a3);
-  sm[threadIdx.x] = acc;
+  const int lane = threadIdx.x & 255, chain = threadIdx.x >> 8;
+  const int64_t ng = wn_sumsq_groups(d.len, lane);
+  const float* q = p + lane + 256 * chain;
+  double a = 0.0;
+  int64_t gi = 0;
+  for (; gi + 16 <= ng; gi += 16) {
+    float v[16];
+#pragma unroll
+    for (int e = 0; e < 16; ++e) v[e] = q[1024 * (gi + e)];
+#pragma unroll
+    for (int e = 0; e < 16; ++e) a += (double)v[e] * (double)v[e];
+  }
+  for (; gi < ng; ++gi) a += (double)q[1024 * gi] * (double)q[1024 * gi];
+  if (chain == 0)
+    for (int64_t i = lane + 1024 * ng; i < d.len; i += 256) a += (double)p[i] * (double)p[i];
+  sm[threadIdx.x] = a;
+  __syncthreads();
+  if (threadIdx.x < 256) {
+    const double acc = (sm[lane] + sm[lane + 256]) + (sm[lane + 512] + sm[lane + 768]);
+    sm[lane] = acc;
+  }
   __syncthreads();
   for (int o = 128; o > 0; o >>= 1) {
     if (threadIdx.x < o) sm[threadIdx.x] += sm[threadIdx.x + o];
@@ -150,7 +166,7 @@
 }
 int wn_launch_sumsq(const float* g, const WnTensorDesc* d_table, int n, float* norms2, hipStream_t s) {
   if (n <= 0) return WN_OK;
-  hipLaunchKernelGGL(wn_sumsq_kernel, dim3(n), dim3(256), 0, s, g, d_table, norms2);
+  hipLaunchKernelGGL(wn_sumsq_kernel, dim3(n), dim3(WN_SUMSQ_THREADS), 0, s, g, d_table, norms2);
   WN_HIP_CHECK(hipGetLastError());
   return WN_OK;
 }
@@ -213,6 +229,31 @@
   return WN_OK;
 }
 
+__device__ inline int64_t wn_vec_head(const void* p0, const void* p1, const void* p2, const void* p3, const void* p4,
+                                      int64_t off, int64_t len) {
+  const unsigned a = (unsigned)((uintptr_t)p0 & 15u);
+  if (((uintptr_t)p1 & 15u) != a || ((uintptr_t)p2 & 15u) != a || ((uintptr_t)p3 & 15u) != a || ((uintptr_t)p4 & 15u) != a ||
+      (a & 3u) != 0)
+    return len;
+  const int64_t head = (int64_t)((16u - (unsigned)(((uintptr_t)p0 + (uintptr_t)off * 4u) & 15u)) & 15u) >> 2;
+  return head < len ? head : len;
+}
+__device__ __forceinline__ void wn_adam_update(float gk, float scale, float& m, float& v, float& p, float alpha, float beta1,
+                                               float beta2, float eps) {
+  const float gi = gk * scale;
+  const float mi = m + (gi - m) * (1.0f - beta1);
+  const float vi = v + (gi * gi - v) * (1.0f - beta2);
+  m = mi;
+  v = vi;
+  p = p - alpha * mi / (sqrtf(vi) + eps);
+}
+__device__ __forceinline__ void wn_ema_update(float& p, float& a, float momentum, int first, int overwrite) {
+  const float pi = p;
+  const float ai = first ? pi : a + (pi - a) * (1.0f - momentum);
+  a = ai;
+  p = overwrite ? ai : pi;
+}
+
 __global__ void wn_adam_kernel(float* p, const float* g, float* m, float* v, const WnTensorDesc* table,
                                const float* norms2, float clipnorm, float alpha, float beta1,
                                float beta2, float eps, const float* skip_flag) {
@@ -223,15 +264,25 @@
     const float nrm = sqrtf(norms2[blockIdx.y]);
     scale = clipnorm / fmaxf(nrm, clipnorm);
   }
-  for (int64_t i = (int64_t)blockIdx.x * blockDim.x + threadIdx.x; i < d.len;
-       i += (int64_t)gridDim.x * blockDim.x) {
-    const int64_t k = d.off + i;
-    const float gi = g[k] * scale;
-    const float mi = m[k] + (gi - m[k]) * (1.0f - beta1);
-    const float vi = v[k] + (gi * gi - v[k]) * (1.0f - beta2);
-    m[k] = mi;
-    v[k] = vi;
-    p[k] = p[k] - alpha * mi / (sqrtf(vi) + eps);
+  const int64_t head = wn_vec_head(p, g, m, v, p, d.off, d.len);
+  const int64_t nvec = (d.len - head) >> 2, tail = head + 4 * nvec;
+  const int64_t tid = (int64_t)blockIdx.x * blockDim.x + threadIdx.x, nth = (int64_t)gridDim.x * blockDim.x;
+  const int64_t k0 = d.off + head;
+  for (int64_t i = tid; i < nvec; i += nth) {
+    const int64_t k = k0 + 4 * i;
+    const float4 g4 = *reinterpret_cast<const float4*>(g + k);
+    float4 m4 = *reinterpret_cast<float4*>(m + k), v4 = *reinterpret_cast<float4*>(v + k), p4 = *reinterpret_cast<float4*>(p + k);
+    wn_adam_update(g4.x, scale, m4.x, v4.x, p4.x, alpha, beta1, beta2, eps);
+    wn_adam_update(g4.y, scale, m4.y, v4.y, p4.y, alpha, beta1, beta2, eps);
+    wn_adam_update(g4.z, scale, m4.z, v4.z, p4.z, alpha, beta1, beta2, eps);
+    wn_adam_update(g4.w, scale, m4.w, v4.w, p4.w, alpha, beta1, beta2, eps);
+    *reinterpret_cast<float4*>(m + k) = m4;
+    *reinterpret_cast<float4*>(v + k) = v4;
+    *reinterpret_cast<float4*>(p + k) = p4;
+  }
+  for (int64_t i = tid; i < head + (d.len - tail); i += nth) {
+    const int64_t k = d.off + (i < head ? i : tail + (i - head));
+    wn_adam_update(g[k], scale, m[k], v[k], p[k], alpha, beta1, beta2, eps);
   }
 }
 int wn_launch_adam(float* p, const float* g, float* m, float* v, const WnTensorDesc* d_table, int n,
@@ -255,18 +306,32 @@
     const float nrm = sqrtf(norms2[blockIdx.y]);
     scale = clipnorm / fmaxf(nrm, clipnorm);
   }
-  for (int64_t i = (int64_t)blockIdx.x * blockDim.x + threadIdx.x; i < d.len;
-       i += (int64_t)gridDim.x * blockDim.x) {
-    const int64_t k = d.off + i;
-    const float gi = g[k] * scale;
-    const float mi = m[k] + (gi - m[k]) * (1.0f - beta1);
-    const float vi = v[k] + (gi * gi - v[k]) * (1.0f - beta2);
-    m[k] = mi;
-    v[k] = vi;
-    const float pi = p[k] - alpha * mi / (sqrtf(vi) + eps);
-    const float ai = first ? pi : a[k] + (pi - a[k]) * (1.0f - momentum);
-    a[k] = ai;
-    p[k] = overwrite ? ai : pi;
+  const int64_t head = wn_vec_head(p, g, m, v, a, d.off, d.len);
+  const int64_t nvec = (d.len - head) >> 2, tail = head + 4 * nvec;
+  const int64_t tid = (int64_t)blockIdx.x * blockDim.x + threadIdx.x, nth = (int64_t)gridDim.x * blockDim.x;
+  const int64_t k0 = d.off + head;
+  for (int64_t i = tid; i < nvec; i += nth) {
+    const int64_t k = k0 + 4 * i;
+    const float4 g4 = *reinterpret_cast<const float4*>(g + k);
+    float4 m4 = *reinterpret_cast<float4*>(m + k), v4 = *reinterpret_cast<float4*>(v + k), p4 = *reinterpret_cast<float4*>(p + k);
+    float4 a4 = *reinterpret_cast<float4*>(a + k);
+    wn_adam_update(g4.x, scale, m4.x, v4.x, p4.x, alpha, beta1, beta2, eps);
+    wn_adam_update(g4.y, scale, m4.y, v4.y, p4.y, alpha, beta1, beta2, eps);
+    wn_adam_update(g4.z, scale, m4.z, v4.z, p4.z, alpha, beta1, beta2, eps);
+    wn_adam_update(g4.w, scale, m4.w, v4.w, p4.w, alpha, beta1, beta2, eps);
+    wn_ema_update(p4.x, a4.x, momentum, first, overwrite);
+    wn_ema_update(p4.y, a4.y, momentum, first, overwrite);
+    wn_ema_update(p4.z, a4.z, momentum, first, overwrite);
+    wn_ema_update(p4.w, a4.w, momentum, first, overwrite);
+    *reinterpret_cast<float4*>(m + k) = m4;
+    *reinterpret_cast<float4*>(v + k) = v4;
+    *reinterpret_cast<float4*>(a + k) = a4;
+    *reinterpret_cast<float4*>(p + k) = p4;
+  }
+  for (int64_t i = tid; i < head + (d.len - tail); i += nth) {
+    const int64_t k = d.off + (i < head ? i : tail + (i - head));
+    wn_adam_update(g[k], scale, m[k], v[k], p[k], alpha, beta1, beta2, eps);
+    wn_ema_update(p[k], a[k], momentum, first, overwrite);
   }
 }
 int wn_launch_adam_ema(float* p, const float* g, float* m, float* v, float* a, const WnTensorDesc* d_table, int n,
@@ -473,6 +538,54 @@
     if (threadIdx.x == 0) wn_absmax_publish_any(absmax_out, fmaxf(fmaxf(wm[0], wm[1]), fmaxf(wm[2], wm[3])));
   }
 }
+__global__ __launch_bounds__(256) void wn_train_prologue_kernel(WnTrainPrologue a, const float* w, const float* bias, int B,
+                                                                int T, int R, int KS, float* y, float* absmax_out) {
+  const int q = R / 4;
+  const int64_t total = (int64_t)B * T * q;
+  float wmax = 0.f;
+  for (int64_t i = (int64_t)blockIdx.x * blockDim.x + threadIdx.x; i < total; i += (int64_t)gridDim.x * blockDim.x) {
+    const int c = (int)(i % q) * 4;
+    const int64_t row = i / q;
+    const int t = (int)(row % T);
+    const float* xr = a.x_full + (row / T) * (int64_t)(T + 1) + t;
+    if (c == 0) {
+      const float yt = xr[1];
+      a.inputs[row] = xr[0];
+      a.y_true[row] = yt;
+      if (a.target) a.target[row] = wn_quantize_one(yt, a.bits);
+    }
+    float a0 = 0.f, a1 = 0.f, a2 = 0.f, a3 = 0.f;
+    for (int tap = 0; tap < KS; ++tap) {
+      const int ts = t - (KS - 1 - tap);
+      const float xv = ts >= 0 ? xr[-(KS - 1 - tap)] : 0.f;
+      const f32x4 wv = *reinterpret_cast<const f32x4*>(w + (int64_t)tap * R + c);
+      a0 = fmaf(wv.x, xv, a0); a1 = fmaf(wv.y, xv, a1); a2 = fmaf(wv.z, xv, a2); a3 = fmaf(wv.w, xv, a3);
+    }
+    const f32x4 bv = *reinterpret_cast<const f32x4*>(bias + c);
+    const f32x4 o = f32x4{a0 + bv.x, a1 + bv.y, a2 + bv.z, a3 + bv.w};
+    *reinterpret_cast<f32x4*>(y + row * R + c) = o;
+    wmax = fmaxf(wmax, fmaxf(fmaxf(fabsf(o.x), fabsf(o.y)), fmaxf(fabsf(o.z), fabsf(o.w))));
+  }
+  if (absmax_out) {
+    __shared__ float wm[4];
+    if (!(wmax < 3.0e38f)) wmax = 3.0e38f;
+    wmax = wn_wave_max(wmax);
+    if ((threadIdx.x & 63) == 0) wm[threadIdx.x >> 6] = wmax;
+    __syncthreads();
+    if (threadIdx.x == 0) wn_absmax_publish_any(absmax_out, fmaxf(fmaxf(wm[0], wm[1]), fmaxf(wm[2], wm[3])));
+  }
+}
+int wn_launch_train_prologue(const WnTrainPrologue& a, const float* w, const float* bias, int B, int T, int R, int KS,
+                             float* y, float* absmax_out, hipStream_t s) {
+  const int64_t total = (int64_t)B * T * (R / 4);
+  if (total <= 0) return WN_OK;
+  if (R % 4 != 0) { wn_set_error("train_prologue: %d channels", R); return WN_E_UNSUPPORTED; }
+  if (a.target && (a.bits < 1 || a.bits > 16)) { wn_set_error("quantize: bits %d unsupported", a.bits); return WN_E_UNSUPPORTED; }
+  hipLaunchKernelGGL(wn_train_prologue_kernel, dim3((unsigned)std::min<int64_t>((total + 255) / 256, 65536)), dim3(256), 0, s, a,
+                     w, bias, B, T, R, KS, y, absmax_out);
+  WN_HIP_CHECK(hipGetLastError());
+  return WN_OK;
+}
 int wn_launch_inconv_fwd(const float* x, const float* w, const float* bias, int B, int T, int R, int KS, float* y,
                          float* absmax_out, hipStream_t s) {
   const int64_t total = (int64_t)B * T * (R / 4);
diff --git a/wavenets_amd/csrc/wn_forward.hip b/wavenets_amd/csrc/wn_forward.hip
--- a/wavenets_amd/csrc/wn_forward.hip
+++ b/wavenets_amd/csrc/wn_forward.hip
@@ -75,19 +75,23 @@
 }
 
 int forward_core(wn_plan* p, const float* params, const float* x, bool prep, const float* cond, int B,
-                 int T, bool training, float* ws, const WsLayout& L, hipStream_t s, const GenRings* rings, LossFuse* lf) {
+                 int T, bool training, float* ws, const WsLayout& L, hipStream_t s, const GenRings* rings, LossFuse* lf,
+                 const WnTrainPrologue* pro) {
   int rc = ensure_device_tables(p);
   if (rc) return rc;
   const int64_t rows = (int64_t)B * T;
   float* fragbase = ws + L.frag;
+  if (pro && !(prep && train_prologue_ok(p) && L.fwd_absmax >= L.absmax)) { wn_set_error("forward: training prologue unavailable"); return WN_E_INVALID; }
   if (prep) {
-    rc = wn_launch_prep_table(p->d_prep, (int)p->prep.size(), params, fragbase, s);
+    rc = wn_launch_prep_table(p->d_prep, (int)p->prep.size(), params, fragbase, s, 16, pro ? ws + L.absmax : nullptr,
+                              pro ? (int)(L.fwd_absmax + 1 - L.absmax) : 0);
     if (rc) return rc;
   }
   wn_exec& exs = wnp::ex(p);
   const bool fold = fold_ok(p);
   const bool fork_prep = prep && fold && p->c.use_skip && wn_debug_get(9) == 0;
   bool prep_forked = false;
+  if (training) exs.gh_zeroed = nullptr;
   auto fold_prep = [&](hipStream_t sp) -> int {
     const bool fp_prof = prep && fold && exs.foldprep_used + 2 <= (int)exs.foldprep_ev.size();
     if (fp_prof) (void)hipEventRecord(exs.foldprep_ev[exs.foldprep_used], sp);
@@ -155,9 +159,12 @@
     }
   }
   float* const fam = ws + L.fwd_absmax;
-  WN_HIP_CHECK(hipMemsetAsync(fam, 0, sizeof(float), s));
+  if (!pro) WN_HIP_CHECK(hipMemsetAsync(fam, 0, sizeof(float), s));
   {
-    if (p->R % 4 == 0 && wn_debug_get(1) != 1) {
+    if (pro) {
+      rc = wn_launch_train_prologue(*pro, params + p->tensors[p->causal.kernel_t].off, params + p->tensors[p->causal.bias_t].off,
+                                    B, T, p->R, p->KS, ws + L.H[0], fam, s);
+    } else if (p->R % 4 == 0 && wn_debug_get(1) != 1) {
       rc = wn_launch_inconv_fwd(x, params + p->tensors[p->causal.kernel_t].off, params + p->tensors[p->causal.bias_t].off, B, T,
                                 p->R, p->KS, ws + L.H[0], fam, s);
     } else {
@@ -195,6 +202,11 @@
     WN_HIP_CHECK(hipStreamWaitEvent(exs.side, exs.ev_ffork, 0));
     rc = fold_prep(exs.side);
     if (rc) return rc;
+    if (training) {
+      rc = wn_launch_fill(ws + L.GH[p->N], 0.f, rows * p->R, exs.side);
+      if (rc) return rc;
+      exs.gh_zeroed = ws + L.GH[p->N];
+    }
     WN_HIP_CHECK(hipEventRecord(exs.ev_fjoin, exs.side));
     prep_forked = true;
   }
@@ -319,6 +331,8 @@
   return WN_OK;
 }
 
+bool train_prologue_ok(const wn_plan* p) { return p->R % 4 == 0 && wn_debug_get(1) != 1 && !p->prep.empty(); }
+
 bool loss_fusable(const wn_plan* p, int64_t rows) {
   if (p->c.head != WN_HEAD_CATEGORICAL || p->Cout != 256 || wn_debug_get(1) == 1 || p->finals.empty()) return false;
   const ConvInfo& c = p->finals.back();
@@ -326,11 +340,10 @@
 }
 
 int loss_stage(wn_plan* p, int B, int T, int global_batch, bool want_grad, float* ws, const WsLayout& L,
-               float* loss_out, float* absmax_out, hipStream_t s, bool fused_done) {
+               float* loss_out, float* absmax_out, hipStream_t s) {
   const int64_t rows = (int64_t)B * T;
   const float gscale = 1.0f / (float)global_batch;
   int rc;
-  if (fused_done) return wn_launch_sum(ws + L.loss_rows, rows, gscale, loss_out, ws + L.sum_scratch, s);
   float* g_logits = want_grad ? ws + L.GF.back() : nullptr;
   if (p->c.head == WN_HEAD_CATEGORICAL) {
     rc = wn_launch_quantize(ws + L.yt, reinterpret_cast<int32_t*>(ws + L.target), rows, p->c.bits, s);
diff --git a/wavenets_amd/csrc/wn_gemm.hip b/wavenets_amd/csrc/wn_gemm.hip
--- a/wavenets_amd/csrc/wn_gemm.hip
+++ b/wavenets_amd/csrc/wn_gemm.hip
@@ -49,7 +49,9 @@
   }
 }
 
-__global__ void wn_prep_table_kernel(const WnPrepDesc* table, const float* params, float* ws) {
+__global__ void wn_prep_table_kernel(const WnPrepDesc* table, const float* params, float* ws, float* zero, int nzero) {
+  if (blockIdx.x == 0 && blockIdx.y == 0)
+    for (int i = threadIdx.x; i < nzero; i += blockDim.x) zero[i] = 0.f;
   WnPrepDesc d = table[blockIdx.y];
   wn_prep_body(d, params, ws, (int64_t)blockIdx.x * blockDim.x + threadIdx.x,
                (int64_t)gridDim.x * blockDim.x);
@@ -61,10 +63,13 @@
 }
 
 int wn_launch_prep_table(const WnPrepDesc* d_table, int n, const float* params, float* ws,
-                         hipStream_t s, int gx) {
-  if (n <= 0) return WN_OK;
+                         hipStream_t s, int gx, float* zero, int nzero) {
+  if (n <= 0) {
+    if (zero && nzero > 0) WN_HIP_CHECK(hipMemsetAsync(zero, 0, (size_t)nzero * sizeof(float), s));
+    return WN_OK;
+  }
   dim3 grid(gx > 0 ? gx : 16, n);
-  hipLaunchKernelGGL(wn_prep_table_kernel, grid, dim3(256), 0, s, d_table, params, ws);
+  hipLaunchKernelGGL(wn_prep_table_kernel, grid, dim3(256), 0, s, d_table, params, ws, zero, zero ? nzero : 0);
   WN_HIP_CHECK(hipGetLastError());
   return WN_OK;
 }
@@ -629,6 +634,37 @@
   return WN_OK;
 }
 
+__global__ __launch_bounds__(256) void wn_reduce_cov_kernel(const float* ws, float* out, const WnCovDesc* table, int n) {
+  int lo = 0, hi = n;
+  while (hi - lo > 1) {
+    const int mid = (lo + hi) >> 1;
+    if (table[mid].blk_first <= (int)blockIdx.x) lo = mid; else hi = mid;
+  }
+  const WnCovDesc d = table[lo];
+  const int64_t i = (int64_t)((int)blockIdx.x - d.blk_first) * 256 + threadIdx.x;
+  if (i >= d.len) return;
+  float acc = 0.f;
+  const float* col = ws + d.slab_off + d.off + i;
+  const int64_t P = d.pitch;
+  int s = 0;
+  for (; s + 16 <= d.nsplit; s += 16) {
+    float v[16];
+#pragma unroll
+    for (int e = 0; e < 16; ++e) v[e] = col[(int64_t)(s + e) * P];
+#pragma unroll
+    for (int e = 0; e < 16; ++e) acc += v[e];
+  }
+  for (; s < d.nsplit; ++s) acc += col[(int64_t)s * P];
+  out[d.off + i] = acc;
+}
+int wn_launch_reduce_cov(const float* ws, float* out, const WnCovDesc* d_table, int n, int64_t nblk, hipStream_t s) {
+  if (n <= 0 || nblk <= 0) return WN_OK;
+  if (nblk >= (int64_t)1 << 30) { wn_set_error("reduce_cov: %lld workgroups", (long long)nblk); return WN_E_UNSUPPORTED; }
+  hipLaunchKernelGGL(wn_reduce_cov_kernel, dim3((unsigned)nblk), dim3(256), 0, s, ws, out, d_table, n);
+  WN_HIP_CHECK(hipGetLastError());
+  return WN_OK;
+}
+
 int wn_wgrad_tile_k() { return 32 * WG_TM; }
 int wn_wgrad_tile_n() { return 32 * WG_TN; }
 
diff --git a/wavenets_amd/csrc/wn_kernels.h b/wavenets_amd/csrc/wn_kernels.h
--- a/wavenets_amd/csrc/wn_kernels.h
+++ b/wavenets_amd/csrc/wn_kernels.h
@@ -16,7 +16,7 @@
   int32_t kind;
 };
 int wn_launch_prep_table(const WnPrepDesc* d_table, int n, const float* params, float* ws,
-                         hipStream_t s, int gx = 16);
+                         hipStream_t s, int gx = 16, float* zero = nullptr, int nzero = 0);
 int wn_launch_prep_one(WnPrepDesc d, const float* params, float* ws, hipStream_t s);
 struct WnVecSumArgs { const float* base; int64_t off0; int64_t stride; int32_t count; int32_t len; float* out; };
 int wn_launch_vecsum(WnVecSumArgs a, hipStream_t s);
@@ -155,6 +155,8 @@
                             int splits_per_b, hipStream_t s, bool exact_fp32 = false);
 int wn_launch_reduce_table(const float* slab, int nsplit, int64_t P, float* out, const WnTensorDesc* d_table,
                            int n, hipStream_t s, const WnTensorDesc* h_table = nullptr);
+struct WnCovDesc { int64_t off, len, slab_off, pitch; int32_t nsplit, blk_first; };
+int wn_launch_reduce_cov(const float* ws, float* out, const WnCovDesc* d_table, int n, int64_t nblk, hipStream_t s);
 struct WnReduceArgs {
   const float* slab; int32_t nsplit; int32_t K; int32_t N;
   float* out; int32_t seg_len; int64_t seg_stride; int32_t accumulate;
@@ -301,6 +303,9 @@
 int wn_inconv_wgrad_supported(int R, int KS);
 int wn_launch_inconv_wgrad(const float* x, const float* g, int B, int T, int R, int KS, int splits_per_b, float* slab,
                            int64_t P, int64_t w_off, int64_t b_off, hipStream_t s);
+struct WnTrainPrologue { const float* x_full; float* inputs; float* y_true; int32_t* target; int bits; };
+int wn_launch_train_prologue(const WnTrainPrologue& a, const float* w, const float* bias, int B, int T, int R, int KS,
+                             float* y, float* absmax_out, hipStream_t s);
 int wn_launch_inconv_fwd(const float* x, const float* w, const float* bias, int B, int T, int R, int KS, float* y,
                          float* absmax_out, hipStream_t s);
 int wn_launch_guard_flag(const float* absmax, float limit, int enabled, float* out, hipStream_t s);
@@ -322,6 +327,8 @@
 int wn_launch_mix_loss(const float* pred, const float* y, int64_t rows, int M, int bits, int kind,
                        float gscale, float* loss_rows, float* g_pred, float* absmax_out, hipStream_t s);
 int wn_launch_sum(const float* v, int64_t n, float scale, float* out, float* scratch, hipStream_t s);
+int wn_launch_loss_tail(const float* v, int64_t n, float scale, float* scratch, bool zero_l2, const float* absmax,
+                        float limit, int enabled, float* loss_out, hipStream_t s);
 int wn_launch_sqdiff_sum(const float* a, const float* b, int64_t n, float scale, float* out, float* scratch, hipStream_t s);
 
 int wn_launch_sample_det(const float* pred, int64_t rows, int C, int M, int bits, float* out, hipStream_t s,
diff --git a/wavenets_amd/csrc/wn_loss.hip b/wavenets_amd/csrc/wn_loss.hip
--- a/wavenets_amd/csrc/wn_loss.hip
+++ b/wavenets_amd/csrc/wn_loss.hip
@@ -228,6 +228,34 @@
   return WN_OK;
 }
 
+__global__ void wn_loss_tail_stage2(const double* scratch, int nb, float scale, int zero_l2, const float* absmax,
+                                    float limit, int enabled, float* loss_out) {
+  __shared__ double sm[256];
+  double acc = 0.0;
+  for (int i = threadIdx.x; i < nb; i += blockDim.x) acc += scratch[i];
+  sm[threadIdx.x] = acc;
+  __syncthreads();
+  for (int o = 128; o > 0; o >>= 1) {
+    if (threadIdx.x < o) sm[threadIdx.x] += sm[threadIdx.x + o];
+    __syncthreads();
+  }
+  if (threadIdx.x == 0) {
+    loss_out[0] = (float)(sm[0] * (double)scale);
+    if (zero_l2) loss_out[1] = 0.f;
+    const float m = absmax ? *absmax : 0.f;
+    loss_out[2] = (enabled && !(m < limit)) ? 1.0f : 0.0f;
+  }
+}
+int wn_launch_loss_tail(const float* v, int64_t n, float scale, float* scratch, bool zero_l2, const float* absmax,
+                        float limit, int enabled, float* loss_out, hipStream_t s) {
+  const int nb = wn_blocks(n, 256, 1024);
+  hipLaunchKernelGGL(wn_sum_stage1, dim3(nb), dim3(256), 0, s, v, n, reinterpret_cast<double*>(scratch));
+  hipLaunchKernelGGL(wn_loss_tail_stage2, dim3(1), dim3(256), 0, s, reinterpret_cast<const double*>(scratch), nb, scale,
+                     zero_l2 ? 1 : 0, absmax, limit, enabled, loss_out);
+  WN_HIP_CHECK(hipGetLastError());
+  return WN_OK;
+}
+
 __global__ void wn_sqdiff_stage1(const float* a, const float* b, int64_t n, double* scratch) {
   __shared__ double sm[256];
   double acc = 0.0;
diff --git a/wavenets_amd/csrc/wn_plan_internal.h b/wavenets_amd/csrc/wn_plan_internal.h
--- a/wavenets_amd/csrc/wn_plan_internal.h
+++ b/wavenets_amd/csrc/wn_plan_internal.h
@@ -102,12 +102,12 @@
   DevTable<WnWgJob> jobs;
   DevTable<WnWgLayer> layers, inner;
   DevTable<WnWgPair> pairs;
-  DevTable<WnTensorDesc> cov;
-  std::vector<WnTensorDesc> h_cov;
+  DevTable<WnCovDesc> cov;
+  int n_cov = 0;
+  int64_t cov_blocks = 0;
   std::vector<WgSpan> spans;
   int n_side = 0;
   bool overlap = false;
-  int cov_head = 0;
   void release() { valid = false; jobs.release(); layers.release(); inner.release(); pairs.release(); cov.release(); }
 };
 
@@ -122,6 +122,7 @@
   hipStream_t side = nullptr;
   hipEvent_t ev_fork = nullptr, ev_join = nullptr;
   hipEvent_t ev_ffork = nullptr, ev_fjoin = nullptr;
+  const float* gh_zeroed = nullptr;
   WnGenBlock* d_gen = nullptr;
   WnGenBlock gen_blk0[3]{};
   int64_t gen_bias_stride = 0;
@@ -360,10 +361,11 @@
 void deep16_ptrs(const wn_plan* p, int b, const float* fragbase, BlockPtrs& k);
 int forward_core(wn_plan* p, const float* params, const float* x, bool prep, const float* cond, int B,
                  int T, bool training, float* ws, const WsLayout& L, hipStream_t s, const GenRings* rings = nullptr,
-                 LossFuse* lf = nullptr);
+                 LossFuse* lf = nullptr, const WnTrainPrologue* pro = nullptr);
+bool train_prologue_ok(const wn_plan* p);
 int shift_split(const float* x_full, int B, int T, float* inputs, float* y_true, hipStream_t s);
 int loss_stage(wn_plan* p, int B, int T, int global_batch, bool want_grad, float* ws, const WsLayout& L,
-               float* loss_out, float* absmax_out, hipStream_t s, bool fused_done = false);
+               float* loss_out, float* absmax_out, hipStream_t s);
 
 }
 
diff --git a/wavenets_amd/csrc/wn_train.hip b/wavenets_amd/csrc/wn_train.hip
--- a/wavenets_amd/csrc/wn_train.hip
+++ b/wavenets_amd/csrc/wn_train.hip
@@ -177,15 +177,28 @@
   if (tp.mtr != 0) span(WgSpan::TR, WgSpan::MFOLD, tp.mtr, pfirst[0], pairs[0].size());
   else if (tp.fold) span(WgSpan::SKIP, WgSpan::MFOLD, 0, 0, !tp.mfused);
   else span(WgSpan::SKIP, WgSpan::BATCH, 0, 0, tp.skipk);
+  std::vector<WnCovDesc> cvd(cov.size());
+  int64_t cov_blocks = 0;
+  for (size_t i = 0; i < cov.size(); ++i) {
+    WnCovDesc& d = cvd[i];
+    d.off = cov[i].off; d.len = cov[i].len;
+    if (tp.in_split && i < 2) { d.slab_off = L.islab; d.pitch = (int64_t)(p->KS + 1) * p->R; d.nsplit = B * L.isplits; }
+    else if (head_own && (int)i >= cov_head) { d.slab_off = L.hslab - L.head_base; d.pitch = L.head_span; d.nsplit = B * L.hsplits; }
+    else { d.slab_off = L.bslab; d.pitch = p->nparams; d.nsplit = B * L.bsplits; }
+    d.blk_first = (int32_t)cov_blocks;
+    cov_blocks += (d.len + 255) / 256;
+    if (cov_blocks >= (int64_t)1 << 30) { wn_set_error("train: coverage table of %lld workgroups", (long long)cov_blocks); return WN_E_UNSUPPORTED; }
+  }
   g.valid = false;
   int rc = g.jobs.upload(jobs, 1);
-  if (!rc) rc = g.cov.upload(cov);
+  if (!rc) rc = g.cov.upload(cvd);
   if (!rc) rc = g.layers.upload(wgl);
   if (!rc) rc = g.inner.upload(wgli);
   if (!rc) rc = g.pairs.upload(all);
   if (rc) return rc;
-  g.h_cov.swap(cov); g.spans.swap(spans);
-  g.n_side = n_side; g.overlap = layerk || pairk; g.cov_head = head_own ? cov_head : (int)g.h_cov.size();
+  g.spans.swap(spans);
+  g.n_cov = (int)cvd.size(); g.cov_blocks = cov_blocks;
+  g.n_side = n_side; g.overlap = layerk || pairk;
   g.B = B; g.T = T; g.bsplits = L.bsplits; g.paths = tp;
   g.valid = true;
   return WN_OK;
@@ -216,15 +229,21 @@
 
   int forward_and_loss() {
     int rc;
-    { const int rcs = shift_split(x_full, B, T, inputs, ws + L.yt, s); if (rcs) return rcs; }
-    if (e.phase_on) (void)hipEventRecord(e.phase_ev[0], s);
-    WN_HIP_CHECK(hipMemsetAsync(am, 0, L.n_absmax * sizeof(float), s));
     LossFuse lf;
     memset(&lf, 0, sizeof(lf));
     const bool fuse = !pred_out && loss_fusable(p, rows);
+    const bool fused_head = train_prologue_ok(p);
+    WnTrainPrologue pro{x_full, inputs, ws + L.yt, fuse ? reinterpret_cast<int32_t*>(ws + L.target) : nullptr, p->c.bits};
+    if (!fused_head) {
+      { const int rcs = shift_split(x_full, B, T, inputs, ws + L.yt, s); if (rcs) return rcs; }
+      WN_HIP_CHECK(hipMemsetAsync(am, 0, L.n_absmax * sizeof(float), s));
+      if (fuse) {
+        rc = wn_launch_quantize(ws + L.yt, reinterpret_cast<int32_t*>(ws + L.target), rows, p->c.bits, s);
+        if (rc) return rc;
+      }
+    }
+    if (e.phase_on) (void)hipEventRecord(e.phase_ev[0], s);
     if (fuse) {
-      rc = wn_launch_quantize(ws + L.yt, reinterpret_cast<int32_t*>(ws + L.target), rows, p->c.bits, s);
-      if (rc) return rc;
       lf.target = reinterpret_cast<const int32_t*>(ws + L.target);
       lf.gscale = 1.0f / (float)global_batch;
       lf.loss_rows = ws + L.loss_rows; lf.g_logits = ws + L.GF.back(); lf.absmax_out = am_GF(nf - 1);
@@ -233,11 +252,17 @@
         lf.seed = e.step_sample_seed; lf.offset = e.step_sample_off;
       }
     }
-    rc = forward_core(p, params, inputs, true, cond, B, T, true, ws, L, s, nullptr, fuse ? &lf : nullptr);
+    rc = forward_core(p, params, inputs, true, cond, B, T, true, ws, L, s, nullptr, fuse ? &lf : nullptr, fused_head ? &pro : nullptr);
     if (rc) return rc;
     if (lf.done && lf.sample_out) e.step_sample = nullptr;
     if (e.phase_on) (void)hipEventRecord(e.phase_ev[1], s);
-    rc = loss_stage(p, B, T, global_batch, true, ws, L, loss_out, am_GF(nf - 1), s, lf.done);
+    const bool l2 = p->c.l2_reg_factor > 0.f;
+    const float guard_limit = WN_RANGE_LIMIT * (e.drop_rate > 0.f ? 1.f - e.drop_rate : 1.f);
+    if (lf.done)
+      rc = wn_launch_loss_tail(ws + L.loss_rows, rows, lf.gscale, ws + L.sum_scratch, !l2, ws + L.fwd_absmax,
+                               guard_limit, wn_debug_get(1) != 1, loss_out, s);
+    else
+      rc = loss_stage(p, B, T, global_batch, true, ws, L, loss_out, am_GF(nf - 1), s);
     if (rc) return rc;
     if (pred_out) {
       if (p->c.head == WN_HEAD_CATEGORICAL) rc = wn_launch_softmax(ws + L.logits, pred_out, rows, p->Cout, s);
@@ -259,19 +284,20 @@
       }
       if (rc) return rc;
     }
-    if (p->c.l2_reg_factor > 0.f) {
+    if (l2) {
       float* norms = ws + L.loss_rows;
       rc = wn_launch_sumsq(params, p->d_kdesc, (int)p->kdesc.size(), norms, s);
       if (rc) return rc;
       rc = wn_launch_sum(norms, (int64_t)p->kdesc.size(), p->c.l2_reg_factor / (float)n_replicas, loss_out + 1, ws + L.sum_scratch, s);
       if (rc) return rc;
-    } else {
+    } else if (!lf.done) {
       rc = wn_launch_fill(loss_out + 1, 0.f, 1, s);
       if (rc) return rc;
     }
-    rc = wn_launch_guard_flag(ws + L.fwd_absmax, WN_RANGE_LIMIT * (e.drop_rate > 0.f ? 1.f - e.drop_rate : 1.f),
-                              wn_debug_get(1) != 1, loss_out + 2, s);
-    if (rc) return rc;
+    if (!lf.done) {
+      rc = wn_launch_guard_flag(ws + L.fwd_absmax, guard_limit, wn_debug_get(1) != 1, loss_out + 2, s);
+      if (rc) return rc;
+    }
     if (e.phase_on) (void)hipEventRecord(e.phase_ev[2], s);
     return WN_OK;
   }
@@ -319,10 +345,11 @@
   int chain_backward() {
     int rc;
     const float* g_skip = (p->c.use_skip && !tp.fold) ? ws + L.g_skipsum : nullptr;
-    if (p->c.use_skip) {
+    if (p->c.use_skip && e.gh_zeroed != ws + L.GH[p->N]) {
       rc = wn_launch_fill(ws + L.GH[p->N], 0.f, rows * p->R, s);
       if (rc) return rc;
     }
+    e.gh_zeroed = nullptr;
     const bool pairk = tp.bwd_pairs();
     for (int b = p->N - 1; b >= 0; --b) {
       BlockPtrs k = block_ptrs(p, b, params, fragbase, B, T);
@@ -495,14 +522,7 @@
     if (tp.fold && (rc = fold_weight_gradients())) return rc;
     if (fork) { WN_HIP_CHECK(hipStreamWaitEvent(s, e.ev_join, 0)); side_join.armed = false; }
     if (cond_batched && (rc = cond_weight_gradients())) return rc;
-    const int cov0 = tp.in_split ? 2 : 0, ncov = (int)g.h_cov.size(), cov1 = g.cov_head;
-    rc = wn_launch_reduce_table(ws + L.bslab, B * L.bsplits, p->nparams, grads, g.cov.d + cov0, cov1 - cov0, s, g.h_cov.data() + cov0);
-    if (rc) return rc;
-    if (tp.in_split && (rc = wn_launch_reduce_table(ws + L.islab, B * L.isplits, (int64_t)(p->KS + 1) * p->R, grads, g.cov.d, 2, s, g.h_cov.data())))
-      return rc;
-    if (cov1 < ncov && (rc = wn_launch_reduce_table(ws + L.hslab - L.head_base, B * L.hsplits, L.head_span, grads, g.cov.d + cov1, ncov - cov1,
-                                                    s, g.h_cov.data() + cov1)))
-      return rc;
+    if ((rc = wn_launch_reduce_cov(ws, grads, g.cov.d, g.n_cov, g.cov_blocks, s))) return rc;
     if (!p->c.use_skip && p->S > 0) {
       for (const BlockInfo& bi : p->blocks) {
         rc = wn_launch_fill(grads + p->tensors[bi.conv_skip.kernel_t].off, 0.f, p->tensors[bi.conv_skip.kernel_t].len, s);
```

Result: no change. 23.33 million (median of 6 runs) (+1.2%).
